# hulop/SfM

Measured on AMD Instinct MI355X. Metric: BA iterations/sec + residual-evals/sec (cams x pts x obs); 1/2/4/8 GPU, higher is better.
Workload: dtype f64; 1 GPU; C3 per GPU: full BA solve (LM + DENSE_SCHUR, Ceres default options); cams=500, points=200000, observations=2000000, points_per_gpu=200000, obs_per_gpu=2000000, views_per_point=10, parallelism=single GPU, reduced_camera_factor=single GPU

## Files before the change

### sfm_amd/csrc/ba_device.h

```cpp
#pragma once
#include <hip/hip_runtime.h>
#include <algorithm>
#include <cstdint>

#include "ba_lm.h"

namespace sfm {

constexpr int kJRec = 20;
constexpr int kJX = 0, kRes = 6, kJC = 8;
constexpr int kEU = 4;
constexpr int kCamR = 36;
constexpr int kUcam = 28;
constexpr int kCamPM = 37;
constexpr int kCamPMMax = 512;
constexpr int kPtV = 10;
constexpr int kPtL = 10;
constexpr int kPtS = 16;
constexpr int kPtG = 16;
constexpr int kCamSR = 32;
constexpr int kNB = 64;
constexpr int kThreads = 256;
constexpr uint32_t kYSentinelWord = 0x7FF4DEADu;
constexpr uint64_t kYSentinel = (uint64_t(kYSentinelWord) << 32) | kYSentinelWord;

struct ReduceJob {
  int slot, nb, op, dst;
};
struct ReduceBatch {
  ReduceJob job[8];
  int n = 0;
  void add(int slot, int nb, int op, int dst) { job[n++] = ReduceJob{slot, nb, op, dst}; }
};

struct DevProblem {
  int32_t C = 0, P = 0;
  int64_t N = 0;
  int32_t* pt_off = nullptr;
  int32_t* order = nullptr;
  int64_t N_pad = 0;
  int32_t* cam_obs = nullptr;
  int32_t* cam_rng = nullptr;
  int32_t* cm_p = nullptr;
  int4* jchunks = nullptr;
  int32_t n_jchunks = 0;
  int32_t xcd_slice_max = 0;
  int32_t* tile_cnt = nullptr;
  int32_t* tile_exp = nullptr;
  int32_t overlap = 0;
  int32_t* jgrp = nullptr;
  int32_t jac_blocks = 1;
  int32_t jac_blocks_rec = 1;
  double* uv_cm = nullptr;
  int32_t* pos = nullptr;
  double* Kc = nullptr;
  double* cam = nullptr;
  double* cam_new = nullptr;
  double* X = nullptr;
  double* X_new = nullptr;
  double* cam0 = nullptr;
  double* X0 = nullptr;
  double* scale_c = nullptr;
  double* scale_p = nullptr;
  double* diag_c = nullptr;
  double* diag_p = nullptr;
  double* camR = nullptr;
  double* camRn = nullptr;
  bool pm_backsub = false;
  double* jrec = nullptr;
  double* eu = nullptr;
  bool eu_cm = false;
  double* ypt = nullptr;
  int32_t* wcam = nullptr;
  double* ptV = nullptr;
  double* ptL = nullptr;
  double* Ucam = nullptr;
  int32_t n = 0, ld = 0, nblk = 0;
  double* S = nullptr;
  double* Spack = nullptr;
  double* invL = nullptr;
  double* ysol = nullptr;
  int32_t* fail = nullptr;
  int32_t* flags = nullptr;
  int32_t* cflags = nullptr;
  unsigned long long* cticket = nullptr;
  int32_t n_cu = 0;
  double min_diag = 1e-6, max_diag = 1e32;

  int64_t n_blk = 0, n_pairs = 0;
  int2* blk = nullptr;
  int32_t* seg = nullptr;
  int32_t* bpts = nullptr;
  int32_t* bperm = nullptr;
  int64_t n_bslots = 0;
  int4* srec = nullptr;
  int32_t schur_wgs = 0;
  double* camS = nullptr;
  double* ptS = nullptr;
  double* ptG = nullptr;
  int32_t schur_pts_sub = 8;
  bool schur_wg_blocks = false;
  double* dpart = nullptr;
  double* jpart = nullptr;
  double* uv_pm = nullptr;
  int32_t* cam_pm = nullptr;
  double* partials = nullptr;
  int32_t max_blocks = 0;
  double* scal = nullptr;
  double* scal_host = nullptr;
  const int32_t* gate = nullptr;
  const double* radius_dev = nullptr;
};

enum PartialSlot {
  kPCost = 0, kPXNormCam, kPXNormPt, kPGradCam, kPGradPt, kPModel, kPNewCost, kPStepPt, kPStepCam, kPBad,
  kPBadCam, kPBadBack, kPModelPt,
  kNumPartialSlots
};

void launch_cam_prep(const DevProblem& d, double* cam, bool count_norm, hipStream_t s);
void launch_cam_prep_accept(const DevProblem& d, bool count_norm, int grid, hipStream_t s);
void launch_jacobian(const DevProblem& d, bool scaled, hipStream_t s, bool write_records = false);
void launch_cam_reduce(const DevProblem& d, hipStream_t s);
void launch_cam_finalize(const DevProblem& d, int mode, bool reuse_diag, bool count_grad, hipStream_t s);
void launch_cam_sum_finalize(const DevProblem& d, int mode, bool count_grad, hipStream_t s);
void launch_point_eval(const DevProblem& d, int mode, bool reuse_diag, hipStream_t s, bool factor = false,
                       double radius = 0.0);
void launch_point_prep(const DevProblem& d, double radius, hipStream_t s);
void launch_obs_prep(const DevProblem& d, hipStream_t s);
void launch_point_factor(const DevProblem& d, double radius, hipStream_t s);
void launch_schur(const DevProblem& d, double radius, bool add_diag, hipStream_t s);
void launch_schur_diag(const DevProblem& d, double radius, bool add_diag, hipStream_t s);
void launch_schur_offdiag(const DevProblem& d, int* tile_cnt, hipStream_t s);
void launch_cam_sum_diag(const DevProblem& d, double radius, bool add_diag, hipStream_t s);
void launch_pad_init(const DevProblem& d, hipStream_t s);
void launch_pack_upper(const DevProblem& d, bool unpack, hipStream_t s);
void launch_gated_copy(const double* src, double* dst, int64_t n, double scale, const int32_t* gate, hipStream_t s);
void launch_cam_update(const DevProblem& d, bool count_norm, hipStream_t s);
inline bool backsub_pm(const DevProblem& d, bool cams_var, bool pts_var) {
  return d.pm_backsub && cams_var && pts_var && d.P > 0 && d.N_pad > 0;
}
bool launch_point_eval_with_cams(const DevProblem& d, int mode, bool count_grad, hipStream_t s);
void launch_point_backsub(const DevProblem& d, hipStream_t s, bool cams_var = true, bool pts_var = true,
                          bool count_norm = false);
inline int obs_xcd_blocks(const DevProblem& d) {
  const int64_t per = d.xcd_slice_max > 0 ? (int64_t(d.xcd_slice_max) + 3) / 4
                                          : ((d.N_pad / 64 + 3) / 4 + 7) / 8;
  return int(8 * std::max<int64_t>(1, per));
}
inline int pt_xcd_blocks(const DevProblem& d) {
  const int64_t per_slice = (int64_t(d.P) + 7) / 8;
  return int(8 * std::max<int64_t>(1, (per_slice + kThreads - 1) / kThreads));
}
void launch_cam_solve(const DevProblem& d, double radius, hipStream_t s);
void launch_reduce(const DevProblem& d, int slot, int nb, int op, int dst, hipStream_t s);
void launch_reduce_batch(const DevProblem& d, const ReduceBatch& b, bool copy_fail, hipStream_t s);
int blocks_for(int64_t n, int threads);

bool launch_cholesky(const DevProblem& d, int epoch, hipStream_t s, bool clear_fail = true, int cam_step = -1,
                     int overlap = 0);
void launch_backsolve(const DevProblem& d, int epoch, hipStream_t s, bool sentinel_set = false);

int launch_cholesky_panel(const DevProblem& d, int k, int pt, int epoch, hipStream_t s);
void launch_panel_update(const DevProblem& d, int k, int j0, int j1, int pt, int nranks, int rank, hipStream_t s);
int panel_update_tiles(int nblk, int pt, int j0, int j1, int nranks, int rank);
constexpr int kPanelPack = 0, kPanelUnpack = 1, kPanelAdd = 2;
void launch_panel_copy(const DevProblem& d, int mode, int pt, int col0, int col1, const int64_t* off, int64_t off1,
                       double* buf, hipStream_t s);
void launch_fail_slot(const DevProblem& d, bool put, double* slot, hipStream_t s);
void launch_spd_fill(double* A, int ld, int n, unsigned seed, hipStream_t s);

}
```

### sfm_amd/csrc/ba_host_layout.h

```cpp
#ifndef SFM_BA_HOST_LAYOUT_H_
#define SFM_BA_HOST_LAYOUT_H_

#include <algorithm>
#include <array>
#include <climits>
#include <cmath>
#include <cstddef>
#include <cstdint>
#include <cstdlib>
#include <vector>

namespace sfm {

constexpr size_t kStageMaxBytes = size_t(1) << 20;
constexpr int64_t kHostCheckMaxObs = 65536;
constexpr int64_t kDeferredUvMinObs = 262144;
constexpr int kSmallSetupMaxC = 256;
constexpr int kSmallSetupMaxChunks = 2048;
constexpr int kSmallSetupMaxPtObs = 64;
constexpr int64_t kSmallSetupMaxObs = 64 * 1024;
constexpr int64_t kSchurXcdMinBlocks = 8192;

namespace hostlayout {

struct StageLayout {
  size_t bytes = 0;
  size_t add(size_t n) {
    const size_t o = bytes;
    bytes += (n + 255) & ~size_t(255);
    return o;
  }
};

inline size_t runs_blob_bound(int C, int64_t N, int P) {
  return 64 * (size_t(C) + 1) + 2 * size_t(N) + 8 * (size_t(P) + 1) + 4 * size_t(C) + 2048;
}

enum class ParamRoute { None, Early, Side, Late };

struct SetupPlan {
  bool host_counts = false;
  bool stage_in = false;
  bool deferred_uv = false;
  size_t o_uv = 0, o_cam = 0, o_pt = 0, o_pc = 0, in_bytes = 0;
  size_t il_base = 0, il_bound = 0;
  size_t o_K = 0, o_c = 0, o_c0 = 0, o_X = 0, o_X0 = 0, pl_bytes = 0;
  size_t pl_base = 0;
  ParamRoute route = ParamRoute::None;
  size_t stage_bytes = 0;
};

inline SetupPlan plan_setup(int64_t N, int C, int P, bool sync_uv) {
  SetupPlan p;
  const bool host_check = N <= kHostCheckMaxObs;
  StageLayout up;
  p.o_uv = up.add(sizeof(double) * 2 * size_t(N));
  p.o_cam = up.add(sizeof(int32_t) * size_t(N));
  p.o_pt = up.add(sizeof(int32_t) * size_t(N));
  p.o_pc = host_check ? up.add(sizeof(int32_t) * (size_t(P) + 1)) : 0;
  p.in_bytes = up.bytes;
  p.stage_in = p.in_bytes <= kStageMaxBytes;
  p.host_counts = host_check && p.stage_in;
  p.deferred_uv = !p.stage_in && N >= kDeferredUvMinObs && !sync_uv;
  p.il_base = p.host_counts ? (p.in_bytes + 255) / 256 * 256 : 0;
  p.il_bound = p.host_counts ? runs_blob_bound(C, N, P) : 0;
  StageLayout pl;
  p.o_K = pl.add(sizeof(double) * 5 * size_t(C));
  p.o_c = pl.add(sizeof(double) * 6 * size_t(C));
  p.o_c0 = pl.add(sizeof(double) * 6 * size_t(C));
  p.o_X = pl.add(sizeof(double) * 3 * size_t(P));
  p.o_X0 = pl.add(sizeof(double) * 3 * size_t(P));
  p.pl_bytes = pl.bytes;
  p.pl_base = (p.il_base + p.il_bound + 255) / 256 * 256;
  if (!(C || P)) p.route = ParamRoute::None;
  else if (p.host_counts && p.pl_base + p.pl_bytes <= 4 * kStageMaxBytes) p.route = ParamRoute::Early;
  else if (p.pl_bytes > kStageMaxBytes) p.route = ParamRoute::Side;
  else p.route = ParamRoute::Late;
  p.stage_bytes = std::max({p.stage_in ? p.il_base + p.il_bound : 0,
                            p.route == ParamRoute::Early ? p.pl_base + p.pl_bytes : 0,
                            sizeof(int32_t) * (size_t(C) + 4)});
  return p;
}

inline bool small_setup_fits(int64_t N, int C, int P, const int32_t* n_obs_of_cam, const int32_t* n_obs_of_pt) {
  if (!(N > 0 && N <= kSmallSetupMaxObs && C > 0 && C <= kSmallSetupMaxC &&
        int64_t(C) * (C + 1) / 2 <= kSchurXcdMinBlocks))
    return false;
  int64_t nch = 0;
  for (int c = 0; c < C; ++c) nch += (n_obs_of_cam[c] + 63) / 64;
  if (nch > kSmallSetupMaxChunks) return false;
  for (int p = 0; p < P; ++p)
    if (n_obs_of_pt[p] > kSmallSetupMaxPtObs) return false;
  return true;
}

struct SchurShape {
  int pts_sub = 8;
  bool wg_blocks = false;
};
inline SchurShape schur_shape(int64_t n_pairs, int64_t n_blk, const char* pts_sub_env, const char* wg_env) {
  SchurShape sh;
  const double avg = n_blk ? double(n_pairs) / double(n_blk) : 0.0;
  if (pts_sub_env) {
    const int v = std::atoi(pts_sub_env);
    sh.pts_sub = v == 64 ? 64 : v == 32 ? 32 : v == 8 ? 8 : 16;
  } else {
    while (sh.pts_sub < 64 && sh.pts_sub < avg / 10.0) sh.pts_sub *= 2;
  }
  sh.wg_blocks = sh.pts_sub == 64 && n_blk <= 4 * 256 && avg >= 256.0;
  if (wg_env) sh.wg_blocks = wg_env[0] == '1' && sh.pts_sub == 64;
  return sh;
}

struct Chunk {
  int32_t cam, pos, cnt, first;
};
static_assert(sizeof(Chunk) == 16, "Chunk must match the device's int4");

inline void check_and_count(int64_t N, const double* obs_uv, const int32_t* cam_idx, const int32_t* pt_idx, int C,
                            int P, bool want_slices, int32_t* cam_cnt, int32_t* pc, std::vector<int32_t>* cam_slice,
                            int64_t* pairs_est) {
  int32_t first[3] = {INT32_MAX, INT32_MAX, INT32_MAX};
  std::fill(cam_cnt, cam_cnt + size_t(C) + 4, 0);
  std::fill(pc, pc + size_t(P) + 1, 0);
  cam_slice->clear();
  *pairs_est = 0;
  const uint64_t* uvb = reinterpret_cast<const uint64_t*>(obs_uv);
  auto nonfinite = [](uint64_t b) { return uint32_t(((b >> 52) & 0x7ff) == 0x7ff); };
  uint32_t bad = 0;
  {
    std::vector<int32_t> cc4(4 * (size_t(C) + 1), 0), pc4(4 * (size_t(P) + 1), 0);
    want_slices = want_slices && P > 0;
    uint32_t sb[8] = {0, 0, 0, 0, 0, 0, 0, 0};
    for (int k = 1; k < 8; ++k) sb[k] = uint32_t((int64_t(k) * P + 7) / 8);
    auto slice_of = [&](uint32_t p) {
      uint32_t v = 0;
      for (int k = 1; k < 8; ++k) v += uint32_t(p >= sb[k]);
      return v;
    };
    std::vector<int32_t> cs4(want_slices ? 4 * 8 * (size_t(C) + 1) : 0, 0);
    int64_t i = 0;
    for (; i + 4 <= N; i += 4) {
      for (int u = 0; u < 4; ++u) {
        const uint32_t c = uint32_t(cam_idx[i + u]), p = uint32_t(pt_idx[i + u]);
        const uint32_t b = uint32_t(c >= uint32_t(C)) | uint32_t(p >= uint32_t(P)) | nonfinite(uvb[2 * (i + u)]) |
                           nonfinite(uvb[2 * (i + u) + 1]);
        bad |= b;
        const uint32_t cc = c < uint32_t(C) ? c : uint32_t(C);
        ++cc4[u * (size_t(C) + 1) + cc];
        ++pc4[u * (size_t(P) + 1) + (p < uint32_t(P) ? p : uint32_t(P))];
        if (want_slices) ++cs4[(u * (size_t(C) + 1) + cc) * 8 + slice_of(p)];
      }
    }
    for (; i < N; ++i) {
      const uint32_t c = uint32_t(cam_idx[i]), p = uint32_t(pt_idx[i]);
      bad |= uint32_t(c >= uint32_t(C)) | uint32_t(p >= uint32_t(P)) | nonfinite(uvb[2 * i]) |
             nonfinite(uvb[2 * i + 1]);
      const uint32_t cc = c < uint32_t(C) ? c : uint32_t(C);
      ++cc4[cc];
      ++pc4[p < uint32_t(P) ? p : uint32_t(P)];
      if (want_slices) ++cs4[size_t(cc) * 8 + slice_of(p)];
    }
    if (want_slices) {
      cam_slice->assign(8 * size_t(C), 0);
      for (size_t e = 0; e < 8 * size_t(C); ++e)
        (*cam_slice)[e] = cs4[e] + cs4[8 * (size_t(C) + 1) + e] + cs4[16 * (size_t(C) + 1) + e] +
                          cs4[24 * (size_t(C) + 1) + e];
    }
    for (int c = 0; c < C; ++c)
      cam_cnt[4 + size_t(c)] =
          cc4[c] + cc4[(size_t(C) + 1) + c] + cc4[2 * (size_t(C) + 1) + c] + cc4[3 * (size_t(C) + 1) + c];
    for (int p = 0; p < P; ++p) {
      pc[p] = pc4[p] + pc4[(size_t(P) + 1) + p] + pc4[2 * (size_t(P) + 1) + p] + pc4[3 * (size_t(P) + 1) + p];
      *pairs_est += int64_t(pc[p]) * (pc[p] - 1) / 2;
    }
  }
  if (bad) {
    for (int64_t i = 0; i < N; ++i) {
      const int32_t c = cam_idx[i], p = pt_idx[i];
      const bool cok = c >= 0 && c < C, pok = p >= 0 && p < P;
      const bool uok = std::isfinite(obs_uv[2 * i]) && std::isfinite(obs_uv[2 * i + 1]);
      if (!cok && first[0] == INT32_MAX) first[0] = int32_t(i);
      if (!pok && first[1] == INT32_MAX) first[1] = int32_t(i);
      if (!uok && first[2] == INT32_MAX) first[2] = int32_t(i);
    }
  }
  cam_cnt[0] = first[0];
  cam_cnt[1] = first[1];
  cam_cnt[2] = first[2];
  cam_cnt[3] = INT32_MAX;
}

struct Runs {
  std::vector<int32_t> cam_off, cam_rng, wcam;
  std::vector<Chunk> chunks;
  int64_t npad = 0;
};
inline void camera_runs(int C, const int32_t* n_obs_of_cam, Runs* r) {
  r->cam_off.assign(size_t(C) + 1, 0);
  r->cam_rng.assign(2 * size_t(C), 0);
  int64_t npad = 0;
  for (int c = 0; c < C; ++c) {
    const int32_t n_c = n_obs_of_cam[c];
    r->cam_off[c + 1] = r->cam_off[c] + n_c;
    r->cam_rng[2 * c] = int32_t(npad);
    r->cam_rng[2 * c + 1] = int32_t(npad + n_c);
    npad += (n_c + 63) / 64 * 64;
  }
  r->npad = npad;
  r->wcam.assign(size_t(npad / 64) + 1, 0);
  for (int c = 0; c < C; ++c)
    for (int64_t w = r->cam_rng[2 * c] / 64;
         w < (int64_t(r->cam_rng[2 * c]) + r->cam_off[c + 1] - r->cam_off[c] + 63) / 64; ++w)
      r->wcam[size_t(w)] = c;
  r->chunks.clear();
  for (int c = 0; c < C; ++c) {
    const int32_t n_c = r->cam_off[c + 1] - r->cam_off[c];
    for (int32_t k = 0; 64 * k < n_c; ++k)
      r->chunks.push_back(Chunk{c, r->cam_rng[2 * c] + 64 * k, std::min<int32_t>(64, n_c - 64 * k),
                                r->cam_off[c] + 64 * k});
  }
}

inline int32_t small_slice_max(int C, const int32_t* n_obs_of_cam, const std::vector<int32_t>& cam_slice) {
  std::array<int32_t, 8> jcnt{};
  for (int c = 0; c < C; ++c) {
    const int32_t n_c = n_obs_of_cam[c];
    int32_t cum = 0;
    int sl = 0;
    for (int32_t k = 0; 64 * k < n_c; ++k) {
      while (sl < 7 && cum + cam_slice[8 * size_t(c) + sl] <= 64 * k) cum += cam_slice[8 * size_t(c) + sl++];
      ++jcnt[size_t(sl)];
    }
  }
  return *std::max_element(jcnt.begin(), jcnt.end());
}

}
}

#endif
```

### sfm_amd/csrc/ba_kernels.hip

```cpp
#include <hip/hip_runtime.h>
#include <cfloat>
#include <cmath>
#include <cstdlib>
#include "ba_device.h"
#include "ba_common.h"

namespace sfm {

namespace {

__global__ __launch_bounds__(kThreads) void k_cam_prep(int C, double* __restrict__ cam,
                                                       double* __restrict__ camR, double* __restrict__ part_xn, const int* __restrict__ gate,
                                                       const double* __restrict__ cam_src, const double* __restrict__ X_src,
                                                       double* __restrict__ X_dst, int64_t n_x) {
  if (gate && *gate == 0) return;
  __shared__ double sh[4];
  const int c = blockIdx.x * blockDim.x + threadIdx.x;
  for (int64_t i = int64_t(blockIdx.x) * blockDim.x + threadIdx.x; i < n_x; i += int64_t(gridDim.x) * blockDim.x)
    X_dst[i] = X_src[i];
  if (int64_t(blockIdx.x) * blockDim.x >= C) return;
  double xn = 0.0;
  if (c < C) {
    const double* cs = cam_src ? cam_src : cam;
    double x6[6];
// ... 14 lines not shown

__device__ __forceinline__ int wave_uniform(int v) { return __builtin_amdgcn_readfirstlane(v); }

__device__ __forceinline__ void jac_flush(const double* wst, double* __restrict__ jrec, int64_t ib, int l) {
  double* dst = jrec + ib * kJRec;
  double2 v[kJRec / 2];
#pragma unroll
  for (int kq = 0; kq < kJRec / 2; ++kq) v[kq] = ld2(wst + 2 * (64 * kq + l));
#pragma unroll
  for (int kq = 0; kq < kJRec / 2; ++kq) st2_nt(dst + 2 * (64 * kq + l), v[kq].x, v[kq].y);
}

__device__ __forceinline__ void wave_lds_sync() {
  __builtin_amdgcn_fence(__ATOMIC_RELEASE, "wavefront");
  __builtin_amdgcn_wave_barrier();
  __builtin_amdgcn_fence(__ATOMIC_ACQUIRE, "wavefront");
}

__device__ __forceinline__ double jac_record(const double* cr, double tc0, double tc1, double tc2, double fx, double sk,
                                             double cx, double fy, double cy, const double* sc, const double* sp,
                                             const double Xp[3], double2 uvo, double rec[kJRec]) {
  const double pc0 = cr[0] * Xp[0] + cr[1] * Xp[1] + cr[2] * Xp[2] + tc0;
  const double pc1 = cr[3] * Xp[0] + cr[4] * Xp[1] + cr[5] * Xp[2] + tc1;
  const double pc2 = cr[6] * Xp[0] + cr[7] * Xp[1] + cr[8] * Xp[2] + tc2;
  const SharedDiv dz = shared_div(pc2);
  const double xp = sdiv(dz, pc0), yp = sdiv(dz, pc1);
  const double r0 = fx * xp + sk * yp + cx - uvo.x;
  const double r1 = fy * yp + cy - uvo.y;
  const double iz = srcp(dz);
  const double a0 = fx * iz, a1 = sk * iz, a2 = -(fx * xp + sk * yp) * iz;
  const double b1 = fy * iz, b2 = -fy * yp * iz;
#pragma unroll
  for (int j = 0; j < 3; ++j) {
    rec[kJX + j] = (a0 * cr[j] + a1 * cr[3 + j] + a2 * cr[6 + j]) * sp[j];
    rec[kJX + 3 + j] = (b1 * cr[3 + j] + b2 * cr[6 + j]) * sp[j];
  }
  rec[kRes] = r0;
  rec[kRes + 1] = r1;
#pragma unroll
  for (int kk = 0; kk < 3; ++kk) {
    const double* D = cr + 9 + 9 * kk;
    const double q0 = D[0] * Xp[0] + D[1] * Xp[1] + D[2] * Xp[2];
    const double q1 = D[3] * Xp[0] + D[4] * Xp[1] + D[5] * Xp[2];
    const double q2 = D[6] * Xp[0] + D[7] * Xp[1] + D[8] * Xp[2];
    rec[kJC + kk] = (a0 * q0 + a1 * q1 + a2 * q2) * sc[kk];
    rec[kJC + 6 + kk] = (b1 * q1 + b2 * q2) * sc[kk];
  }
  rec[kJC + 3] = a0 * sc[3]; rec[kJC + 4] = a1 * sc[4]; rec[kJC + 5] = a2 * sc[5];
  rec[kJC + 9] = 0.0;        rec[kJC + 10] = b1 * sc[4]; rec[kJC + 11] = b2 * sc[5];
  return 0.5 * (r0 * r0 + r1 * r1);
}

template <bool kRec>
__global__ __launch_bounds__(kThreads) void k_jacobian(const int32_t* __restrict__ grp_off,
                                                       const int4* __restrict__ chunks,
                                                       const int32_t* __restrict__ cm_p,
                                                       const double* __restrict__ uv_cm,
                                                       const double* __restrict__ Kc, const double* __restrict__ cam,
                                                       const double* __restrict__ camR, const double* __restrict__ X,
                                                       const double* __restrict__ scale_c,
                                                       const double* __restrict__ scale_p, int scaled,
                                                       double* __restrict__ jrec, double* __restrict__ part_cost,
                                                       double* __restrict__ jpart, const int* __restrict__ gate) {
  if (gate && *gate == 0) return;
  __shared__ double sh[4];
  __shared__ __attribute__((aligned(16))) double stage[kRec ? kThreads * kJRec : 2];
  const int l = threadIdx.x & 63;
  const int wv = wave_uniform(threadIdx.x >> 6);
  double* wst = stage + wv * 64 * kJRec;
  const int grp = blockIdx.x & 7;
  const int nbg = (int(gridDim.x) - 1 - grp) / 8 + 1;
  const int nw = nbg * (kThreads / 64);
  const int wi = (blockIdx.x >> 3) * (kThreads / 64) + wv;
  const int g0 = grp_off[grp], glen = grp_off[grp + 1] - g0;
  int t = g0 + int(int64_t(glen) * wi / nw);
  const int n_chunks = g0 + int(int64_t(glen) * (wi + 1) / nw);
  double cost = 0.0;
  auto chunk_at = [&](int tt) { return chunks[tt < n_chunks ? tt : t]; };
  int p_nxt = 0;
  double2 uv_cur = make_double2(0.0, 0.0);
  double Xc[3] = {0.0, 0.0, 1.0}, spc[3] = {1.0, 1.0, 1.0};
  if (t < n_chunks) {
    const int64_t i = int64_t(chunks[t].y) + l;
    const int p0 = cm_p[i];
    uv_cur = ld2(uv_cm + 2 * i);
    p_nxt = cm_p[int64_t(chunk_at(t + 1).y) + l];
#pragma unroll
    for (int j = 0; j < 3; ++j) Xc[j] = X[3 * size_t(p0) + j];
    if (scaled)
#pragma unroll
      for (int j = 0; j < 3; ++j) spc[j] = scale_p[3 * size_t(p0) + j];
  }
  asm volatile("" : "+v"(Xc[0]), "+v"(Xc[1]), "+v"(Xc[2]), "+v"(spc[0]), "+v"(spc[1]), "+v"(spc[2]), "+v"(uv_cur.x),
               "+v"(uv_cur.y), "+v"(p_nxt));
  double acc[32];
#pragma unroll
  for (int e = 0; e < 32; ++e) acc[e] = 0.0;
  for (; t < n_chunks; ++t) {
    const int4 ch = chunks[t];
    const int c = ch.x, cnt = ch.z;
    const int64_t ib = ch.y;
    double Xn[3], spn[3] = {1.0, 1.0, 1.0};
#pragma unroll
    for (int j = 0; j < 3; ++j) Xn[j] = X[3 * size_t(p_nxt) + j];
    if (scaled)
#pragma unroll
      for (int j = 0; j < 3; ++j) spn[j] = scale_p[3 * size_t(p_nxt) + j];
    const int4 ch_n = chunk_at(t + 1);
    const double2 uv_nxt = ld2(uv_cm + 2 * (int64_t(ch_n.y) + l));
    const int p_nn = cm_p[int64_t(chunk_at(t + 2).y) + l];
    const double* cr = camR + size_t(kCamR) * c;
    const double* k = Kc + 5 * size_t(c);
    double sc[6];
#pragma unroll
    for (int a = 0; a < 6; ++a) sc[a] = scaled ? scale_c[6 * size_t(c) + a] : 1.0;
    {
      double rec[kJRec];
      const double cl = jac_record(cr, cam[6 * c + 3], cam[6 * c + 4], cam[6 * c + 5], k[0], k[1], k[2], k[3], k[4],
                                   sc, spc, Xc, uv_cur, rec);
      cost += (l < cnt) ? cl : 0.0;
      if (kRec) {
        double* mine = wst + l * kJRec;
#pragma unroll
        for (int f = 0; f < kJRec; f += 2) st2(mine + f, rec[f], rec[f + 1]);
      }
      if (jpart) {
        double j0[6], j1[6], r0 = rec[kRes], r1 = rec[kRes + 1];
#pragma unroll
        for (int a = 0; a < 6; ++a) {
          j0[a] = rec[kJC + a];
          j1[a] = rec[kJC + 6 + a];
        }
        if (cnt < 64) {
          const bool real = l < cnt;
#pragma unroll
          for (int a = 0; a < 6; ++a) {
            j0[a] = real ? j0[a] : 0.0;
            j1[a] = real ? j1[a] : 0.0;
          }
          r0 = real ? r0 : 0.0;
          r1 = real ? r1 : 0.0;
        }
        int q = 0;
#pragma unroll
        for (int a = 0; a < 6; ++a)
#pragma unroll
          for (int b = a; b < 6; ++b, ++q) acc[q] += j0[a] * j0[b] + j1[a] * j1[b];
#pragma unroll
        for (int a = 0; a < 6; ++a) acc[21 + a] += j0[a] * r0 + j1[a] * r1;
        double tot = 0.0;
        if (t + 1 >= n_chunks || ch_n.x != c) {
          tot = wave_sum32(acc, l);
#pragma unroll
          for (int e = 0; e < 32; ++e) acc[e] = 0.0;
        }
        if (!(l & 1) && (l >> 1) < 27) jpart[size_t(ib / 64) * 27 + (l >> 1)] = tot;
      }
    }
    if (kRec) {
      wave_lds_sync();
      jac_flush(wst, jrec, ib, l);
      wave_lds_sync();
    }
#pragma unroll
    for (int j = 0; j < 3; ++j) { Xc[j] = Xn[j]; spc[j] = spn[j]; }
    uv_cur = uv_nxt;
    p_nxt = p_nn;
  }
  const double r = block_reduce(cost, sh, false);
  if (threadIdx.x == 0) part_cost[blockIdx.x] = r;
}

__global__ __launch_bounds__(64) void k_cam_sum(const int32_t* __restrict__ cam_rng,
                                                const double* __restrict__ jpart, double* __restrict__ Ucam, const int* __restrict__ gate) {
  if (gate && *gate == 0) return;
  const int c = blockIdx.x, t = threadIdx.x;
  const int w0 = cam_rng[2 * c] / 64, w1 = (cam_rng[2 * c + 1] + 63) / 64;
  double v[32];
#pragma unroll
  for (int e = 0; e < 32; ++e) v[e] = 0.0;
  for (int w = w0 + t; w < w1; w += 64) {
    const double* src = jpart + size_t(w) * 27;
#pragma unroll
    for (int e = 0; e < 27; ++e) v[e] += src[e];
  }
  const double sum = wave_sum32(v, t);
  if (!(t & 1) && (t >> 1) < 27) Ucam[size_t(kUcam) * c + (t >> 1)] = sum;
}

struct CamFold {
  const int32_t* cam_rng;
  const double* jpart;
  double* Ucam;
  double* scale_c;
  double* diag_c;
  double min_diag, max_diag;
  int mode, C;
  double* part_grad;
};
__device__ __forceinline__ double cam_sum_body(int c, int t, const CamFold& f) {
  const int w0 = f.cam_rng[2 * c] / 64, w1 = (f.cam_rng[2 * c + 1] + 63) / 64;
  double v[32];
#pragma unroll
  for (int e = 0; e < 32; ++e) v[e] = 0.0;
  for (int w = w0 + t; w < w1; w += 64) {
    const double* src = f.jpart + size_t(w) * 27;
#pragma unroll
    for (int e = 0; e < 27; ++e) v[e] += src[e];
  }
  const double sum = wave_sum32(v, t);
  if (!(t & 1) && (t >> 1) < 27) f.Ucam[size_t(kUcam) * c + (t >> 1)] = sum;
  const int a = t < 6 ? t : 0;
  const double cn = __shfl(sum, 2 * up6(a, a)), ga = __shfl(sum, 2 * (21 + a));
  double g = 0.0;
  if (t < 6) {
    if (f.mode == 0) {
      f.scale_c[6 * c + a] = 1.0 / (1.0 + sqrt(cn));
    } else {
      f.diag_c[6 * c + a] = fmin(fmax(cn, f.min_diag), f.max_diag);
      g = fabs(ga / f.scale_c[6 * c + a]);
    }
  }
#pragma unroll
  for (int off = 4; off > 0; off >>= 1) g = fmax(g, __shfl_xor(g, off));
  if (t == 0 && f.part_grad) f.part_grad[c] = g;
  return sum;
}

__global__ __launch_bounds__(64) void k_cam_sum_finalize(const CamFold f, const int* __restrict__ gate) {
  if (gate && *gate == 0) return;
  cam_sum_body(blockIdx.x, threadIdx.x, f);
}

__global__ __launch_bounds__(kThreads) void k_cam_finalize(int C, const double* __restrict__ Ucam,
                                                           double* __restrict__ scale_c, double* __restrict__ diag_c,
                                                           double min_diag, double max_diag, int mode, int reuse,
                                                           double* __restrict__ part_grad, const int* __restrict__ gate) {
  if (gate && *gate == 0) return;
  __shared__ double sh[4];
  const int c = blockIdx.x * blockDim.x + threadIdx.x;
  double g = 0.0;
  if (c < C) {
    const double* U = Ucam + size_t(kUcam) * c;
    for (int a = 0; a < 6; ++a) {
      const double cn = U[up6(a, a)];
      if (mode == 0) {
        scale_c[6 * c + a] = 1.0 / (1.0 + sqrt(cn));
      } else {
        if (!reuse) diag_c[6 * c + a] = fmin(fmax(cn, min_diag), max_diag);
        g = fmax(g, fabs(U[21 + a] / scale_c[6 * c + a]));
      }
    }
  }
  const double r = block_reduce(g, sh, true);
  if (threadIdx.x == 0 && part_grad) part_grad[blockIdx.x] = r;
}

struct CamView {
  const double* R; const double* t; const double* K;
  int sR, sT, sK;
};

__device__ __forceinline__ double point_factor_body(int p, const double v[9], const double dg[3], double radius,
                                                    const double x[3], const double sp[3], double* __restrict__ ptL,
                                                    double* __restrict__ ptS, double* __restrict__ ptG) {
  double bad = 0.0;
  double D[3];
  for (int k = 0; k < 3; ++k) { const double d = sqrt(dg[k] / radius); D[k] = d * d; }
  const double V00 = v[0] + D[0], V10 = v[1], V11 = v[2] + D[1], V20 = v[3], V21 = v[4], V22 = v[5] + D[2];
  const double l00 = sqrt(V00);
  const double l10 = V10 / l00, l20 = V20 / l00;
  const double l11 = sqrt(V11 - l10 * l10);
  const double l21 = (V21 - l20 * l10) / l11;
  const double l22 = sqrt(V22 - l20 * l20 - l21 * l21);
  if (!(l00 > 0.0) || !(l11 > 0.0) || !(l22 > 0.0)) bad = 1.0;
  const double z0 = v[6] / l00, z1 = (v[7] - l10 * z0) / l11, z2 = (v[8] - l20 * z0 - l21 * z1) / l22;
  double* L = ptL + size_t(kPtL) * p;
  st2(L, l00, l10); st2(L + 2, l11, l20); st2(L + 4, l21, l22); st2(L + 6, z0, z1); st2(L + 8, z2, 0.0);
  if (ptS) {
    double* o = ptS + size_t(kPtS) * p;
    st2(o, x[0], x[1]); st2(o + 2, x[2], sp[0]); st2(o + 4, sp[1], sp[2]);
    st2(o + 6, l10, l20); st2(o + 8, l21, 1.0 / l00); st2(o + 10, 1.0 / l11, 1.0 / l22);
    st2(o + 12, z0, z1); st2(o + 14, z2, 0.0);
  }
  if (ptG) {
    const double i00 = 1.0 / l00, i11 = 1.0 / l11, i22 = 1.0 / l22;
    const double li10 = -l10 * i00 * i11, li21 = -l21 * i11 * i22, li20 = -(l20 * i00 + l21 * li10) * i22;
    double* o = ptG + size_t(kPtG) * p;
    st2(o, x[0], x[1]); st2(o + 2, x[2], sp[0] * i00); st2(o + 4, sp[0] * li10, sp[0] * li20);
    st2(o + 6, sp[1] * i11, sp[1] * li21); st2(o + 8, sp[2] * i22, 0.0);
  }
  return bad;
}

struct PointFold {
  double radius;
  const double* radius_dev;
  double* ptL;
  double* ptS;
  double* ptG;
  double* part_bad;
};

__device__ __forceinline__ void point_eval_body(int p, const int32_t* __restrict__ pt_off,
                                                const int32_t* __restrict__ cam_pm,
                                                const double* __restrict__ uv_pm, const CamView cv,
                                                const double* __restrict__ X, double* __restrict__ scale_p,
                                                double* __restrict__ diag_p, double* __restrict__ ptV,
                                                double min_diag, double max_diag, int mode, int reuse, double& g,
                                                double& xn, const PointFold& pf, double& bad) {
  double V[6] = {0, 0, 0, 0, 0, 0}, b[3] = {0, 0, 0};
  const double Xp[3] = {X[3 * size_t(p)], X[3 * size_t(p) + 1], X[3 * size_t(p) + 2]};
  double sp[3] = {1.0, 1.0, 1.0};
  if (mode == 1)
    for (int k = 0; k < 3; ++k) sp[k] = scale_p[3 * size_t(p) + k];
  const int q0 = pt_off[p], q1 = pt_off[p + 1];
  int c_n = q0 < q1 ? cam_pm[q0] : 0;
  double2 uv_n = q0 < q1 ? ld2(uv_pm + 2 * size_t(q0)) : make_double2(0.0, 0.0);
  for (int q = q0; q < q1; ++q) {
    const int c = c_n;
    const double2 uvo = uv_n;
    if (q + 1 < q1) {
      c_n = cam_pm[q + 1];
      uv_n = ld2(uv_pm + 2 * size_t(q + 1));
    }
    const double* cr = cv.R + size_t(cv.sR) * c;
    const double* k5 = cv.K + size_t(cv.sK) * c;
    const double* tc = cv.t + size_t(cv.sT) * c;
    const double fx = k5[0], sk = k5[1], cx = k5[2], fy = k5[3], cy = k5[4];
    const double pc0 = cr[0] * Xp[0] + cr[1] * Xp[1] + cr[2] * Xp[2] + tc[0];
    const double pc1 = cr[3] * Xp[0] + cr[4] * Xp[1] + cr[5] * Xp[2] + tc[1];
    const double pc2 = cr[6] * Xp[0] + cr[7] * Xp[1] + cr[8] * Xp[2] + tc[2];
    const SharedDiv dz = shared_div(pc2);
    const double xp = sdiv(dz, pc0), yp = sdiv(dz, pc1);
    const double r0 = fx * xp + sk * yp + cx - uvo.x;
    const double r1 = fy * yp + cy - uvo.y;
    const double iz = srcp(dz);
    const double a0 = fx * iz, a1 = sk * iz, a2 = -(fx * xp + sk * yp) * iz;
    const double b1 = fy * iz, b2 = -fy * yp * iz;
    double u[3], v[3];
#pragma unroll
    for (int j = 0; j < 3; ++j) {
      u[j] = (a0 * cr[j] + a1 * cr[3 + j] + a2 * cr[6 + j]) * sp[j];
      v[j] = (b1 * cr[3 + j] + b2 * cr[6 + j]) * sp[j];
    }
    V[0] += u[0] * u[0] + v[0] * v[0];
    V[1] += u[1] * u[0] + v[1] * v[0]; V[2] += u[1] * u[1] + v[1] * v[1];
    V[3] += u[2] * u[0] + v[2] * v[0]; V[4] += u[2] * u[1] + v[2] * v[1]; V[5] += u[2] * u[2] + v[2] * v[2];
    b[0] += u[0] * r0 + v[0] * r1; b[1] += u[1] * r0 + v[1] * r1; b[2] += u[2] * r0 + v[2] * r1;
  }
  const double cn[3] = {V[0], V[2], V[5]};
  if (mode == 0) {
    for (int k = 0; k < 3; ++k) scale_p[3 * size_t(p) + k] = 1.0 / (1.0 + sqrt(cn[k]));
  } else {
    for (int k = 0; k < 3; ++k) {
      if (!reuse) diag_p[3 * size_t(p) + k] = fmin(fmax(cn[k], min_diag), max_diag);
      g = fmax(g, fabs(b[k] / scale_p[3 * size_t(p) + k]));
      xn += X[3 * size_t(p) + k] * X[3 * size_t(p) + k];
    }
    double* o = ptV + size_t(kPtV) * p;
    st2(o, V[0], V[1]); st2(o + 2, V[2], V[3]); st2(o + 4, V[4], V[5]); st2(o + 6, b[0], b[1]); st2(o + 8, b[2], 0.0);
    if (pf.ptL) {
      double fv[9] = {V[0], V[1], V[2], V[3], V[4], V[5], b[0], b[1], b[2]};
      double fd[3], fx[3] = {Xp[0], Xp[1], Xp[2]}, fs[3] = {sp[0], sp[1], sp[2]};
      for (int k = 0; k < 3; ++k) fd[k] = reuse ? diag_p[3 * size_t(p) + k] : fmin(fmax(cn[k], min_diag), max_diag);
      double radius = pf.radius_dev ? *pf.radius_dev : pf.radius;
      asm volatile("" : "+v"(fv[0]), "+v"(fv[1]), "+v"(fv[2]), "+v"(fv[3]), "+v"(fv[4]), "+v"(fv[5]), "+v"(fv[6]),
                        "+v"(fv[7]), "+v"(fv[8]), "+v"(fd[0]), "+v"(fd[1]), "+v"(fd[2]), "+v"(radius));
      bad = point_factor_body(p, fv, fd, radius, fx, fs, pf.ptL, pf.ptS, pf.ptG);
    }
  }
}

__global__ __launch_bounds__(kThreads) void k_point_eval_rc(int P, const int32_t* __restrict__ pt_off,
                                                            const int32_t* __restrict__ cam_pm,
                                                            const double* __restrict__ uv_pm,
                                                            const double* __restrict__ camR,
                                                            const double* __restrict__ cam,
                                                            const double* __restrict__ Kc,
                                                            const double* __restrict__ X,
                                                            double* __restrict__ scale_p, double* __restrict__ diag_p,
                                                            double* __restrict__ ptV, double min_diag, double max_diag,
                                                            int mode, int reuse, double* __restrict__ part_grad,
                                                            double* __restrict__ part_xn, const int* __restrict__ gate,
                                                            const PointFold pf) {
  if (gate && *gate == 0) return;
  __shared__ double sh[4];
  const int p = blockIdx.x * blockDim.x + threadIdx.x;
  double g = 0.0, xn = 0.0, bad = 0.0;
  const CamView cv{camR, cam + 3, Kc, kCamR, 6, 5};
  if (p < P)
    point_eval_body(p, pt_off, cam_pm, uv_pm, cv, X, scale_p, diag_p, ptV, min_diag, max_diag, mode, reuse, g, xn, pf,
                    bad);
  if (mode == 1) {
    const double rg = block_reduce(g, sh, true);
    if (threadIdx.x == 0) part_grad[blockIdx.x] = rg;
    const double rx = block_reduce(xn, sh, false);
    if (threadIdx.x == 0) part_xn[blockIdx.x] = rx;
    if (pf.ptL) {
      const double rb = block_reduce(bad, sh, true);
      if (threadIdx.x == 0) pf.part_bad[blockIdx.x] = rb;
    }
  }
}

constexpr int kCamE = 17;
template <int kMaxC, int kGroups = 1>
__global__ __launch_bounds__(kThreads * kGroups) void k_point_eval_lds(int P, int C, const int32_t* __restrict__ pt_off,
                                                             const int32_t* __restrict__ cam_pm,
                                                             const double* __restrict__ uv_pm,
                                                             const double* __restrict__ camR,
                                                             const double* __restrict__ cam,
                                                             const double* __restrict__ Kc,
                                                             const double* __restrict__ X,
                                                             double* __restrict__ scale_p, double* __restrict__ diag_p,
                                                             double* __restrict__ ptV, double min_diag, double max_diag,
                                                             int mode, int reuse, double* __restrict__ part_grad,
                                                             double* __restrict__ part_xn, const int* __restrict__ gate,
                                                             const CamFold cf, const PointFold pf) {
  if (gate && *gate == 0) return;
  static_assert(kGroups == 1 || kMaxC > 64, "the camera fold runs with one group per workgroup");
  const int nbp = (P + kThreads - 1) / kThreads;
  if (kGroups == 1 && int(blockIdx.x) >= nbp) {
    const int c = (int(blockIdx.x) - nbp) * (kThreads / 64) + int(threadIdx.x >> 6);
    if (c < cf.C) cam_sum_body(c, threadIdx.x & 63, cf);
    return;
  }
  __shared__ double sh[4 * kGroups];
  __shared__ double cst[kMaxC * kCamE];
  for (int i = threadIdx.x; i < C * kCamE; i += blockDim.x) {
    const int c = i / kCamE, j = i - c * kCamE;
    cst[i] = j < 9 ? camR[size_t(kCamR) * c + j] : j < 12 ? cam[6 * size_t(c) + 3 + (j - 9)] : Kc[5 * size_t(c) + (j - 12)];
  }
  __syncthreads();
  const int grp = int(threadIdx.x) / kThreads, tg = int(threadIdx.x) % kThreads;
  const int vb = int(blockIdx.x) * kGroups + grp;
  const int p = vb * kThreads + tg;
  double g = 0.0, xn = 0.0, bad = 0.0;
  const CamView cv{cst, cst + 9, cst + 12, kCamE, kCamE, kCamE};
  if (p < P)
    point_eval_body(p, pt_off, cam_pm, uv_pm, cv, X, scale_p, diag_p, ptV, min_diag, max_diag, mode, reuse, g, xn, pf,
                    bad);
  if (mode == 1) {
    const int w = int(threadIdx.x) >> 6, l = int(threadIdx.x) & 63;
    __shared__ double shb[4 * kGroups];
    const double wg = wave_max(g), wx = wave_sum(xn);
    if (pf.ptL) {
      const double wb = wave_max(bad);
      if (l == 0) shb[w] = wb;
    }
    if (l == 0) sh[w] = wg;
    __syncthreads();
    double rg = 0.0;
    if (tg == 0) {
      rg = sh[4 * grp];
      for (int i = 1; i < 4; ++i) rg = fmax(rg, sh[4 * grp + i]);
    }
    __syncthreads();
    if (l == 0) sh[w] = wx;
    __syncthreads();
    if (tg == 0 && vb < nbp) {
      double rx = sh[4 * grp];
      for (int i = 1; i < 4; ++i) rx = rx + sh[4 * grp + i];
      part_grad[vb] = rg;
      part_xn[vb] = rx;
      if (pf.ptL) {
        double rb = shb[4 * grp];
        for (int i = 1; i < 4; ++i) rb = fmax(rb, shb[4 * grp + i]);
        pf.part_bad[vb] = rb;
      }
    }
  }
}

__global__ __launch_bounds__(kThreads) void k_point_factor(int P, const double* __restrict__ ptV,
                                                           const double* __restrict__ diag_p, double radius,
                                                           double* __restrict__ ptL, double* __restrict__ part_bad,
                                                           const double* __restrict__ X,
                                                           const double* __restrict__ scale_p,
                                                           double* __restrict__ ptS, const int* __restrict__ gate, const double* __restrict__ radius_dev,
                                                           double* __restrict__ ptG) {
  if (gate && *gate == 0) return;
  if (radius_dev) radius = *radius_dev;
  __shared__ double sh[4];
  const int p = blockIdx.x * blockDim.x + threadIdx.x;
  double bad = 0.0;
  if (p < P) {
    const double* vp = ptV + size_t(kPtV) * p;
    const double v[9] = {vp[0], vp[1], vp[2], vp[3], vp[4], vp[5], vp[6], vp[7], vp[8]};
    const double dg[3] = {diag_p[3 * size_t(p)], diag_p[3 * size_t(p) + 1], diag_p[3 * size_t(p) + 2]};
    double x[3] = {0.0, 0.0, 0.0}, sp[3] = {0.0, 0.0, 0.0};
    if (ptS || ptG)
      for (int k = 0; k < 3; ++k) { x[k] = X[3 * size_t(p) + k]; sp[k] = scale_p[3 * size_t(p) + k]; }
    bad = point_factor_body(p, v, dg, radius, x, sp, ptL, ptS, ptG);
  }
  const double r = block_reduce(bad, sh, true);
  if (threadIdx.x == 0) part_bad[blockIdx.x] = r;
}

struct ObsRC {
  double rec[kJRec];
  double M[6];
  double h0, h1;
};
__device__ __forceinline__ void obs_recompute(int c, int p, double2 uvo, const double* __restrict__ camR,
                                              const double* __restrict__ cam, const double* __restrict__ Kc,
                                              const double* __restrict__ scale_c, const double* __restrict__ ptS,
                                              ObsRC& o) {
  const double* cr = camR + size_t(kCamR) * c;
  const double* k = Kc + 5 * size_t(c);
  const double* tc = cam + 6 * size_t(c) + 3;
  const double* sc = scale_c + 6 * size_t(c);
  const double fx = k[0], sk = k[1], cx = k[2], fy = k[3], cy = k[4];
  const double* rp = ptS + size_t(kPtS) * p;
  double q[16];
#pragma unroll
  for (int f = 0; f < 16; f += 2) {
    const double2 x = ld2(rp + f);
    q[f] = x.x; q[f + 1] = x.y;
  }
  const double Xp[3] = {q[0], q[1], q[2]}, sp[3] = {q[3], q[4], q[5]};
  const double pc0 = cr[0] * Xp[0] + cr[1] * Xp[1] + cr[2] * Xp[2] + tc[0];
  const double pc1 = cr[3] * Xp[0] + cr[4] * Xp[1] + cr[5] * Xp[2] + tc[1];
  const double pc2 = cr[6] * Xp[0] + cr[7] * Xp[1] + cr[8] * Xp[2] + tc[2];
  const double iz = srcp(shared_div(pc2)), xp = pc0 * iz, yp = pc1 * iz;
  double* rec = o.rec;
  rec[kRes] = fx * xp + sk * yp + cx - uvo.x;
  rec[kRes + 1] = fy * yp + cy - uvo.y;
  const double a0 = fx * iz, a1 = sk * iz, a2 = -(fx * xp + sk * yp) * iz;
  const double b1 = fy * iz, b2 = -fy * yp * iz;
#pragma unroll
  for (int j = 0; j < 3; ++j) {
    rec[kJX + j] = (a0 * cr[j] + a1 * cr[3 + j] + a2 * cr[6 + j]) * sp[j];
    rec[kJX + 3 + j] = (b1 * cr[3 + j] + b2 * cr[6 + j]) * sp[j];
  }
#pragma unroll
  for (int kk = 0; kk < 3; ++kk) {
    const double* D = cr + 9 + 9 * kk;
    const double q0 = D[0] * Xp[0] + D[1] * Xp[1] + D[2] * Xp[2];
    const double q1 = D[3] * Xp[0] + D[4] * Xp[1] + D[5] * Xp[2];
    const double q2 = D[6] * Xp[0] + D[7] * Xp[1] + D[8] * Xp[2];
    rec[kJC + kk] = (a0 * q0 + a1 * q1 + a2 * q2) * sc[kk];
    rec[kJC + 6 + kk] = (b1 * q1 + b2 * q2) * sc[kk];
  }
  rec[kJC + 3] = a0 * sc[3]; rec[kJC + 4] = a1 * sc[4]; rec[kJC + 5] = a2 * sc[5];
  rec[kJC + 9] = 0.0;        rec[kJC + 10] = b1 * sc[4]; rec[kJC + 11] = b2 * sc[5];
  const double l10 = q[6], l20 = q[7], l21 = q[8], i00 = q[9], i11 = q[10], i22 = q[11];
  const double* e = rec + kJX;
  o.M[0] = e[0] * i00; o.M[1] = (e[1] - l10 * o.M[0]) * i11; o.M[2] = (e[2] - l20 * o.M[0] - l21 * o.M[1]) * i22;
  o.M[3] = e[3] * i00; o.M[4] = (e[4] - l10 * o.M[3]) * i11; o.M[5] = (e[5] - l20 * o.M[3] - l21 * o.M[4]) * i22;
  o.h0 = o.M[0] * q[12] + o.M[1] * q[13] + o.M[2] * q[14];
  o.h1 = o.M[3] * q[12] + o.M[4] * q[13] + o.M[5] * q[14];
}

struct XcdChunks {
  int t, end, stride;
};
__device__ __forceinline__ XcdChunks xcd_chunks(const int32_t* __restrict__ grp_off, int wv) {
  const int grp = blockIdx.x & 7;
  const int nbg = (int(gridDim.x) - 1 - grp) / 8 + 1;
  const int wi = (blockIdx.x >> 3) * (kThreads / 64) + wv;
  return XcdChunks{grp_off[grp] + wi, grp_off[grp + 1], nbg * (kThreads / 64)};
}

__global__ __launch_bounds__(kThreads) void k_obs_prep_rc(const int32_t* __restrict__ grp_off,
                                                          const int4* __restrict__ chunks,
                                                          const int32_t* __restrict__ cm_p,
                                                          const double* __restrict__ uv_cm,
                                                          const int32_t* __restrict__ cam_obs,
                                                          const double* __restrict__ camR,
                                                          const double* __restrict__ cam,
                                                          const double* __restrict__ Kc,
                                                          const double* __restrict__ scale_c,
                                                          const double* __restrict__ ptS,
                                                          double* __restrict__ dpart, const int* __restrict__ gate) {
  if (gate && *gate == 0) return;
  const int l = threadIdx.x & 63, wv = threadIdx.x >> 6;
  const XcdChunks xc = xcd_chunks(grp_off, wave_uniform(wv));
  if (xc.t >= xc.end) return;
  const int4 ch = chunks[xc.t];
  const int64_t i0 = __builtin_amdgcn_readfirstlane(ch.y);
  const int64_t i = i0 + l;
  const int c = __builtin_amdgcn_readfirstlane(ch.x);
  ObsRC o;
  obs_recompute(c, cm_p[i], ld2(uv_cm + 2 * i), camR, cam, Kc, scale_c, ptS, o);
  const double* jc = o.rec + kJC;
  double F[18];
#pragma unroll
  for (int u = 0; u < 6; ++u) {
    F[3 * u] = jc[u] * o.M[0] + jc[6 + u] * o.M[3];
    F[3 * u + 1] = jc[u] * o.M[1] + jc[6 + u] * o.M[4];
    F[3 * u + 2] = jc[u] * o.M[2] + jc[6 + u] * o.M[5];
  }
  double r0 = o.rec[kRes] - o.h0, r1 = o.rec[kRes + 1] - o.h1;
  if (__builtin_amdgcn_readfirstlane(ch.z) < 64) {
    const bool real = cam_obs[i] >= 0;
#pragma unroll
    for (int e = 0; e < 18; ++e) F[e] = real ? F[e] : 0.0;
    r0 = real ? r0 : 0.0;
    r1 = real ? r1 : 0.0;
  }
  double v[32];
  int q = 0;
#pragma unroll
  for (int u = 0; u < 6; ++u)
#pragma unroll
    for (int w = u; w < 6; ++w, ++q)
      v[q] = F[3 * u] * F[3 * w] + F[3 * u + 1] * F[3 * w + 1] + F[3 * u + 2] * F[3 * w + 2];
#pragma unroll
  for (int u = 0; u < 6; ++u) v[21 + u] = jc[u] * r0 + jc[6 + u] * r1;
#pragma unroll
  for (int e = 27; e < 32; ++e) v[e] = 0.0;
  const double tot = wave_sum32(v, l);
  if (!(l & 1) && (l >> 1) < 27) dpart[size_t(i0 / 64) * 27 + (l >> 1)] = tot;
}

__global__ __launch_bounds__(kThreads) void k_backsub_a_rc(const int32_t* __restrict__ grp_off,
                                                           const int4* __restrict__ chunks,
                                                           const int32_t* __restrict__ cm_p,
                                                           const double* __restrict__ uv_cm,
                                                           const int32_t* __restrict__ cam_obs,
                                                           const double* __restrict__ camR,
                                                           const double* __restrict__ cam,
                                                           const double* __restrict__ Kc,
                                                           const double* __restrict__ scale_c,
                                                           const double* __restrict__ ptS,
                                                           const double* __restrict__ ysol, double* __restrict__ eu,
                                                           int eu_cm, double* __restrict__ part_model, const int* __restrict__ gate) {
  if (gate && *gate == 0) return;
  __shared__ double sh[4];
  const int l = threadIdx.x & 63, wv = threadIdx.x >> 6;
  double model = 0.0;
  const XcdChunks xc = xcd_chunks(grp_off, wave_uniform(wv));
  for (int t = xc.t; t < xc.end; t += xc.stride) {
    const int4 ch = chunks[t];
    const int64_t i = int64_t(__builtin_amdgcn_readfirstlane(ch.y)) + l;
    const int c = __builtin_amdgcn_readfirstlane(ch.x);
    ObsRC o;
    obs_recompute(c, cm_p[i], ld2(uv_cm + 2 * i), camR, cam, Kc, scale_c, ptS, o);
    const double* y = ysol + 6 * size_t(c);
    const double* J = o.rec + kJC;
    double e0 = 0.0, e1 = 0.0;
#pragma unroll
    for (int k = 0; k < 6; ++k) { e0 += J[k] * y[k]; e1 += J[6 + k] * y[k]; }
    const int qo = cam_obs[i];
    if (qo >= 0) {
      model += e0 * o.rec[kRes] + e1 * o.rec[kRes + 1] - 0.5 * (e0 * e0 + e1 * e1);
      const double* M = o.M;
      double* dst = eu + 4 * (eu_cm ? size_t(i) : size_t(qo));
      st2(dst, M[0] * e0 + M[3] * e1, M[1] * e0 + M[4] * e1);
      st2(dst + 2, M[2] * e0 + M[5] * e1, 0.0);
    }
  }
  const double r = block_reduce(model, sh, false);
  if (threadIdx.x == 0) part_model[blockIdx.x] = r;
}

template <bool kRegs = false>
__device__ __forceinline__ void schur_diag_body(int c, int C, int t, const int32_t* __restrict__ cam_rng,
                                                const double* __restrict__ dpart, const double* __restrict__ Ucam,
                                                const double* __restrict__ diag_c, double radius, int add_diag,
                                                double* __restrict__ S, int ld, int n, int init,
                                                int* __restrict__ fail, unsigned long long* __restrict__ ysol,
                                                int n_y, double uq = 0.0, double dgu = 0.0) {
  for (int j = 6 * c; j < 6 * c + 6; ++j) {
    for (int i = n + 1 + t; i < ld; i += 64) S[size_t(j) * ld + i] = 0.0;
    if (t == 0 && j < n_y) ysol[j] = kYSentinel;
  }
  if (c == C - 1) {
    for (int j = n; j < ld; ++j) {
      for (int i = (j > n ? j : n + 1) + t; i < ld; i += 64) S[size_t(j) * ld + i] = (i == j) ? 1.0 : 0.0;
      if (t == 0 && j < n_y) ysol[j] = kYSentinel;
    }
    if (t == 0) {
      S[size_t(n) * ld + n] = 1.0;
      *fail = 0;
    }
  }
  const int w0 = cam_rng[2 * c] / 64, w1 = (cam_rng[2 * c + 1] + 63) / 64;
  double v[32];
#pragma unroll
  for (int e = 0; e < 32; ++e) v[e] = 0.0;
  for (int w = w0 + t; w < w1; w += 64) {
    const double* src = dpart + size_t(w) * 27;
#pragma unroll
    for (int e = 0; e < 27; ++e) v[e] += src[e];
  }
  const double sum = wave_sum32(v, t);
  const int tu = t < 36 ? t / 6 : 0, tv = t < 36 ? t % 6 : 0;
  const int src = t < 36 ? up6(tu, tv) : (t < 42 ? 21 + (t - 36) : 0);
  const double tot = __shfl(sum, 2 * src);
  if (t < 36) {
    const int u = tu, vv = tv, q = src;
    double* sp = S + size_t(6 * c + u) * ld + 6 * size_t(c) + vv;
    double val = (init ? 0.0 : *sp) - tot;
    if (add_diag) {
      val += kRegs ? uq : Ucam[size_t(kUcam) * c + q];
      if (u == vv) { const double dd = sqrt((kRegs ? dgu : diag_c[6 * size_t(c) + u]) / radius); val += dd * dd; }
    }
    *sp = val;
  } else if (t < 42) {
    S[size_t(6 * c + (t - 36)) * ld + n] = tot;
  }
}

struct DiagFold {
  const int32_t* cam_rng;
  const double* dpart;
  const double* Ucam;
  const double* diag_c;
  double radius;
  const double* radius_dev;
  int add_diag, C, n, n_y;
  int* fail;
  unsigned long long* ysol;
};

constexpr int kCamS = 50;

__device__ __forceinline__ void stage_cam(double* cs, int c, const double* __restrict__ camR,
                                          const double* __restrict__ cam, const double* __restrict__ Kc,
                                          const double* __restrict__ scale_c, int l) {
  if (l < 36) cs[l] = camR[size_t(kCamR) * c + l];
  else if (l < 39) cs[l] = cam[6 * size_t(c) + 3 + (l - 36)];
  else if (l < 44) cs[l] = Kc[5 * size_t(c) + (l - 39)];
  else if (l < 50) cs[l] = scale_c[6 * size_t(c) + (l - 44)];
}

__device__ __forceinline__ void pair_side_m(const double* cs, const double Xp[3], const double sp[3],
                                            const double Lp[6], double M[6], double ab[5]) {
  const double* cr = cs;
  const double fx = cs[39], sk = cs[40], fy = cs[42];
  const double pc0 = cr[0] * Xp[0] + cr[1] * Xp[1] + cr[2] * Xp[2] + cs[36];
  const double pc1 = cr[3] * Xp[0] + cr[4] * Xp[1] + cr[5] * Xp[2] + cs[37];
  const double pc2 = cr[6] * Xp[0] + cr[7] * Xp[1] + cr[8] * Xp[2] + cs[38];
  const double iz = srcp(shared_div(pc2)), xp = pc0 * iz, yp = pc1 * iz;
  const double a0 = fx * iz, a1 = sk * iz, a2 = -(fx * xp + sk * yp) * iz;
  const double b1 = fy * iz, b2 = -fy * yp * iz;
  ab[0] = a0; ab[1] = a1; ab[2] = a2; ab[3] = b1; ab[4] = b2;
  double e[6];
#pragma unroll
  for (int j = 0; j < 3; ++j) {
    e[j] = (a0 * cr[j] + a1 * cr[3 + j] + a2 * cr[6 + j]) * sp[j];
    e[3 + j] = (b1 * cr[3 + j] + b2 * cr[6 + j]) * sp[j];
  }
// ... 534 lines not shown
    p_nx = iB1;
    asm volatile("" ::: "memory");
    pairs_rot_finish<kSub>(cs1, cs2, acc, own, cc, S, ld, nullptr, l, sl);
    wave_lds_sync();
    tA = tB; tB = tC; tC += W;
    rA = rB; rB = rC;
    cur ^= 1;
  }
}

__global__ __launch_bounds__(64) void k_schur_diag_sum(const int32_t* __restrict__ cam_rng,
                                                       const double* __restrict__ dpart,
                                                       const double* __restrict__ Ucam,
                                                       const double* __restrict__ diag_c, double radius,
                                                       int add_diag, double* __restrict__ S, int ld, int n,
                                                       int init, const int* __restrict__ gate, const double* __restrict__ radius_dev,
                                                       int* __restrict__ fail, unsigned long long* __restrict__ ysol, int n_y) {
  if (gate && *gate == 0) return;
  if (radius_dev) radius = *radius_dev;
  schur_diag_body(blockIdx.x, gridDim.x, threadIdx.x, cam_rng, dpart, Ucam, diag_c, radius, add_diag, S, ld, n, init,
                  fail, ysol, n_y);
}

__global__ __launch_bounds__(64) void k_cam_sum_diag(const CamFold f, const DiagFold df, double* __restrict__ S, int ld,
                                                     const int* __restrict__ gate) {
  if (gate && *gate == 0) return;
  const int c = blockIdx.x, t = threadIdx.x;
  const double sum = cam_sum_body(c, t, f);
  const int tu = t < 36 ? t / 6 : 0, tv = t < 36 ? t % 6 : 0;
  double uq = __shfl(sum, 2 * up6(tu, tv));
  double dgu = fmin(fmax(__shfl(sum, 2 * up6(tu, tu)), f.min_diag), f.max_diag);
  double radius = df.radius_dev ? *df.radius_dev : df.radius;
  asm volatile("" : "+v"(uq), "+v"(dgu), "+v"(radius));
  schur_diag_body<true>(c, df.C, t, df.cam_rng, df.dpart, nullptr, nullptr, radius, df.add_diag, S, ld, df.n, 1,
                        df.fail, df.ysol, df.n_y, uq, dgu);
}

__device__ __forceinline__ size_t packed_row(int i, int n) { return size_t(i) * (n + 1) - size_t(i) * (i - 1) / 2; }

__global__ void k_pack_upper(const double* __restrict__ S, int ld, int n, double* __restrict__ P, const int* __restrict__ gate) {
  if (gate && *gate == 0) return;
  const int i = blockIdx.x;
  const double* row = S + size_t(i) * ld;
  double* dst = P + packed_row(i, n) - i;
  for (int j = i + threadIdx.x; j <= n; j += blockDim.x) dst[j] = row[j];
}

__global__ void k_unpack_upper(const double* __restrict__ P, int ld, int n, double* __restrict__ S, const int* __restrict__ gate) {
  if (gate && *gate == 0) return;
  const int i = blockIdx.x;
  double* row = S + size_t(i) * ld;
  const double* src = P + packed_row(i, n) - i;
  for (int j = i + threadIdx.x; j <= n; j += blockDim.x) row[j] = src[j];
}

__global__ void k_gated_copy(const double* src, double* dst, int64_t n, double scale, const int* __restrict__ gate) {
  if (gate && *gate == 0) return;
  for (int64_t i = blockIdx.x * int64_t(blockDim.x) + threadIdx.x; i < n; i += int64_t(gridDim.x) * blockDim.x)
    dst[i] = src[i] * scale;
}

__global__ void k_pad_init(double* __restrict__ S, int ld, int n, int* __restrict__ fail,
                           unsigned long long* __restrict__ ysol, int n_y, const int* __restrict__ gate) {
  if (gate && *gate == 0) return;
  const int j = blockIdx.x;
  if (j == 0 && threadIdx.x == 0) *fail = 0;
  if (threadIdx.x == 0 && j < n_y) ysol[j] = kYSentinel;
  for (int i = (j > n ? j : n + 1) + threadIdx.x; i < ld; i += blockDim.x) S[size_t(j) * ld + i] = (i == j) ? 1.0 : 0.0;
  if (j == n && threadIdx.x == 0) S[size_t(n) * ld + n] = 1.0;
}

__device__ __forceinline__ void cam_pm_pack(int c, const double* __restrict__ camR, const double* __restrict__ cam,
                                            const double* __restrict__ Kc, const double* __restrict__ ysol,
                                            const double* __restrict__ scale_c, double* __restrict__ o) {
  const double* cr = camR + size_t(kCamR) * c;
  double R[9], sy[6];
  for (int i = 0; i < 9; ++i) R[i] = cr[i];
  for (int k = 0; k < 6; ++k) sy[k] = scale_c[6 * c + k] * ysol[6 * c + k];
  bool first_order = true;
#pragma unroll 1
  for (int k = 0; k < 3; ++k)
#pragma unroll
    for (int i = 0; i < 9; ++i) first_order = first_order & (cr[9 + 9 * k + i] == skew_basis_entry(k, i));
  double om[3] = {sy[0], sy[1], sy[2]};
  if (!first_order) {
    om[0] = om[1] = om[2] = 0.0;
    for (int k = 0; k < 3; ++k) {
      const double* D = cr + 9 + 9 * k;
      double W[9];
      for (int i = 0; i < 3; ++i)
        for (int j = 0; j < 3; ++j) W[3 * i + j] = D[3 * i] * R[3 * j] + D[3 * i + 1] * R[3 * j + 1] + D[3 * i + 2] * R[3 * j + 2];
      om[0] += 0.5 * (W[7] - W[5]) * sy[k];
      om[1] += 0.5 * (W[2] - W[6]) * sy[k];
      om[2] += 0.5 * (W[3] - W[1]) * sy[k];
    }
  }
  for (int i = 0; i < 9; ++i) o[i] = R[i];
  for (int i = 0; i < 3; ++i) o[9 + i] = cam[6 * c + 3 + i];
  for (int i = 0; i < 5; ++i) o[12 + i] = Kc[5 * size_t(c) + i];
  for (int i = 0; i < 3; ++i) { o[17 + i] = om[i]; o[20 + i] = sy[3 + i]; }
  o[35] = first_order ? 1.0 : 0.0;
  o[36] = 0.0;
}

__global__ __launch_bounds__(kThreads) void k_cam_update(int C, const double* __restrict__ cam,
                                                         const double* __restrict__ ysol,
                                                         const double* __restrict__ scale_c,
                                                         double* __restrict__ cam_new, double* __restrict__ camRn,
                                                         double* __restrict__ part_step, double* __restrict__ part_bad, const int* __restrict__ gate) {
  if (gate && *gate == 0) return;
  __shared__ double sh[4];
  const int c = blockIdx.x * blockDim.x + threadIdx.x;
  double st = 0.0, bad = 0.0;
  if (c < C) cam_update_one(c, cam, ysol, scale_c, cam_new, camRn, st, bad);
  const double rs = block_reduce(st, sh, false);
  if (threadIdx.x == 0 && part_step) part_step[blockIdx.x] = rs;
  const double rb = block_reduce(bad, sh, true);
  if (threadIdx.x == 0) part_bad[blockIdx.x] = rb;
}

__global__ __launch_bounds__(kThreads) void k_cam_solve(int C, const double* __restrict__ Ucam,
                                                        const double* __restrict__ diag_c, double radius,
                                                        double* __restrict__ ysol, int* __restrict__ fail, const int* __restrict__ gate, const double* __restrict__ radius_dev) {
  if (gate && *gate == 0) return;
  if (radius_dev) radius = *radius_dev;
  const int c = blockIdx.x * blockDim.x + threadIdx.x;
  if (c >= C) return;
  const double* U = Ucam + size_t(kUcam) * c;
  double L[21], y[6];
  bool ok = true;
#pragma unroll
  for (int j = 0; j < 6; ++j) {
    double s = U[up6(j, j)] + diag_c[6 * c + j] / radius;
#pragma unroll
    for (int k = 0; k < j; ++k) s -= L[up6(k, j)] * L[up6(k, j)];
    ok = ok && s > 0.0 && isfinite(s);
    const double ljj = sqrt(s);
    L[up6(j, j)] = ljj;
#pragma unroll
    for (int i = j + 1; i < 6; ++i) {
      double a = U[up6(j, i)];
#pragma unroll
      for (int k = 0; k < j; ++k) a -= L[up6(k, i)] * L[up6(k, j)];
      L[up6(j, i)] = a / ljj;
    }
  }
#pragma unroll
  for (int i = 0; i < 6; ++i) {
    double s = U[21 + i];
#pragma unroll
    for (int k = 0; k < i; ++k) s -= L[up6(k, i)] * y[k];
    y[i] = s / L[up6(i, i)];
  }
#pragma unroll
  for (int i = 5; i >= 0; --i) {
    double s = y[i];
#pragma unroll
    for (int k = i + 1; k < 6; ++k) s -= L[up6(i, k)] * y[k];
    y[i] = s / L[up6(i, i)];
  }
#pragma unroll
  for (int i = 0; i < 6; ++i) ysol[6 * c + i] = y[i];
  if (!ok) atomicOr(fail, 1);
}


__global__ __launch_bounds__(kThreads) void k_backsub_b(int P, const int32_t* __restrict__ pt_off,
                                                        const double* __restrict__ eu,
                                                        const int32_t* __restrict__ eu_pos,
                                                        const double* __restrict__ ptL,
                                                        const double* __restrict__ ptV,
                                                        const double* __restrict__ scale_p,
                                                        const double* __restrict__ X, double* __restrict__ X_new,
                                                        double* __restrict__ ypt, double* __restrict__ part_step,
                                                        double* __restrict__ part_bad,
                                                        double* __restrict__ part_model, const int* __restrict__ gate) {
  if (gate && *gate == 0) return;
  __shared__ double sh[4];
  const int x = blockIdx.x & 7;
  const int pb = int((int64_t(x) * P + 7) / 8), pe = int((int64_t(x + 1) * P + 7) / 8);
  const int p = pb + (blockIdx.x >> 3) * blockDim.x + threadIdx.x;
  double st = 0.0, bad = 0.0, model = 0.0;
  if (p < pe) {
    const double* L = ptL + size_t(kPtL) * p;
    const double l00 = L[0], l10 = L[1], l11 = L[2], l20 = L[3], l21 = L[4], l22 = L[5];
    double w0 = L[6], w1 = L[7], w2 = L[8];
    double s0 = 0.0, s1 = 0.0, s2 = 0.0;
    const int q0 = pt_off[p], q1 = pt_off[p + 1];
    int q = q0;
    for (; q + 4 <= q1; q += 4) {
      int ps[4];
#pragma unroll
      for (int j = 0; j < 4; ++j) ps[j] = eu_pos ? eu_pos[q + j] : q + j;
      double2 a[4];
      double b[4];
#pragma unroll
      for (int j = 0; j < 4; ++j) {
        const double* u = eu + 4 * size_t(ps[j]);
        a[j] = ld2(u);
        b[j] = u[2];
      }
#pragma unroll
      for (int j = 0; j < 4; ++j) {
        w0 -= a[j].x;
        w1 -= a[j].y;
        w2 -= b[j];
        s0 += a[j].x; s1 += a[j].y; s2 += b[j];
      }
    }
    for (; q < q1; ++q) {
      const double* u = eu + 4 * (eu_pos ? size_t(eu_pos[q]) : size_t(q));
      const double2 u01 = ld2(u);
      const double u2 = u[2];
      w0 -= u01.x;
      w1 -= u01.y;
      w2 -= u2;
      s0 += u01.x; s1 += u01.y; s2 += u2;
    }
    const double y2 = w2 / l22;
    const double y1 = (w1 - l21 * y2) / l11;
    const double y0 = (w0 - l10 * y1 - l20 * y2) / l00;
    if (!isfinite(y0) || !isfinite(y1) || !isfinite(y2)) bad = 1.0;
    {
      const double* v = ptV + size_t(kPtV) * p;
      const double h0 = l00 * s0, h1 = l10 * s0 + l11 * s1, h2 = l20 * s0 + l21 * s1 + l22 * s2;
      const double yVy = v[0] * y0 * y0 + v[2] * y1 * y1 + v[5] * y2 * y2 +
                         2.0 * (v[1] * y0 * y1 + v[3] * y0 * y2 + v[4] * y1 * y2);
      model = y0 * (v[6] - h0) + y1 * (v[7] - h1) + y2 * (v[8] - h2) - 0.5 * yVy;
    }
    const double yp[3] = {y0, y1, y2};
    for (int k = 0; k < 3; ++k) {
      const double x = X[3 * size_t(p) + k];
      const double xn = x + scale_p[3 * size_t(p) + k] * (-yp[k]);
      const double d = x - xn;
      st += d * d;
      X_new[3 * size_t(p) + k] = xn;
      ypt[3 * size_t(p) + k] = yp[k];
    }
  }
  double r = block_reduce(st, sh, false);
  if (threadIdx.x == 0) part_step[blockIdx.x] = r;
  r = block_reduce(bad, sh, true);
  if (threadIdx.x == 0) part_bad[blockIdx.x] = r;
  r = block_reduce(model, sh, false);
  if (threadIdx.x == 0) part_model[blockIdx.x] = r;
}

__global__ __launch_bounds__(kThreads) void k_backsub_c(const int32_t* __restrict__ grp_off,
                                                        const int4* __restrict__ chunks,
                                                        const int32_t* __restrict__ cam_obs,
                                                        const int32_t* __restrict__ cm_p,
                                                        const double* __restrict__ uv_cm,
                                                        const double* __restrict__ Kc,
                                                        const double* __restrict__ X_new,
                                                        const double* __restrict__ camRn,
                                                        double* __restrict__ part_cost, const int* __restrict__ gate) {
  if (gate && *gate == 0) return;
  __shared__ double sh[4];
  const int l = threadIdx.x & 63, wv = threadIdx.x >> 6;
  const XcdChunks xc = xcd_chunks(grp_off, wave_uniform(wv));
  double ncost = 0.0;
  if (xc.t < xc.end) {
    const int4 ch = chunks[xc.t];
    const int64_t i = int64_t(__builtin_amdgcn_readfirstlane(ch.y)) + l;
    const int c = __builtin_amdgcn_readfirstlane(ch.x);
    const bool real = cam_obs[i] >= 0;
    const int p = cm_p[i];
    const double* Rn = camRn + 12 * size_t(c);
    const double Xn0 = X_new[3 * size_t(p)], Xn1 = X_new[3 * size_t(p) + 1], Xn2 = X_new[3 * size_t(p) + 2];
    double pc[3];
#pragma unroll
    for (int k = 0; k < 3; ++k) pc[k] = Rn[3 * k] * Xn0 + Rn[3 * k + 1] * Xn1 + Rn[3 * k + 2] * Xn2 + Rn[9 + k];
    const SharedDiv dz = shared_div(pc[2]);
    const double xp = sdiv(dz, pc[0]), ypj = sdiv(dz, pc[1]);
    const double* k5 = Kc + 5 * size_t(c);
    const double2 uvo = ld2(uv_cm + 2 * i);
    const double rn0 = k5[0] * xp + k5[1] * ypj + k5[2] - uvo.x;
    const double rn1 = k5[3] * ypj + k5[4] - uvo.y;
    if (real) ncost = 0.5 * (rn0 * rn0 + rn1 * rn1);
  }
  const double r = block_reduce(ncost, sh, false);
  if (threadIdx.x == 0) part_cost[blockIdx.x] = r;
}

struct CamStepFold {
  const double* cam; const double* ysol; const double* scale_c; const double* camR; const double* Kc;
  double* cam_new; double* camRn; double* part_step; double* part_bad;
};

__device__ __forceinline__ void cam_step_record(int c, const CamStepFold& cu, double* o, bool store, double& st,
                                                double& bad) {
  double xn[6], rn[12];
  cam_update_vals(c, cu.cam, cu.ysol, cu.scale_c, xn, rn, st, bad);
  if (store) {
    for (int k = 0; k < 6; ++k) cu.cam_new[6 * c + k] = xn[k];
    for (int i = 0; i < 12; ++i) cu.camRn[12 * size_t(c) + i] = rn[i];
  }
  for (int i = 0; i < 12; ++i) o[23 + i] = rn[i];
  cam_pm_pack(c, cu.camR, cu.cam, cu.Kc, cu.ysol, cu.scale_c, o);
}

template <int kGroups>
__global__ __launch_bounds__(kThreads * kGroups) void k_backsub_pm(
    int P, int C, const int32_t* __restrict__ pt_off, const int32_t* __restrict__ cam_pm,
    const double* __restrict__ uv_pm, const double* __restrict__ ptL,
    const double* __restrict__ ptV, const double* __restrict__ scale_p, const double* __restrict__ X,
    double* __restrict__ X_new, double* __restrict__ ypt, double* __restrict__ part_model,
    double* __restrict__ part_model_pt, double* __restrict__ part_step, double* __restrict__ part_bad,
    double* __restrict__ part_cost, const int* __restrict__ gate, const CamStepFold cu) {
  if (gate && *gate == 0) return;
  static_assert(kThreads * kGroups >= kCamPMMax, "one thread per camera record");
  __shared__ double sh[4 * kGroups];
  __shared__ double cst[kCamPMMax * kCamPM];
  const int nbp = (P + kThreads - 1) / kThreads;
  const int grp = int(threadIdx.x) / kThreads, tg = int(threadIdx.x) % kThreads;
  const int vb = int(blockIdx.x) * kGroups + grp;
  const int p = vb * kThreads + tg;
  {
    const int c = int(threadIdx.x);
    double cst_ = 0.0, cbad = 0.0;
    if (c < C) cam_step_record(c, cu, cst + kCamPM * c, blockIdx.x == 0, cst_, cbad);
    if (blockIdx.x == 0) {
      const int w = int(threadIdx.x) >> 6, l = int(threadIdx.x) & 63;
      const int nbc = (C + kThreads - 1) / kThreads;
      const double ws = wave_sum(cst_), wb = wave_max(cbad);
      if (l == 0) sh[w] = ws;
      __syncthreads();
      if (tg == 0 && grp < nbc && cu.part_step) {
        double r = sh[4 * grp];
        for (int i = 1; i < 4; ++i) r = r + sh[4 * grp + i];
        cu.part_step[grp] = r;
      }
      __syncthreads();
      if (l == 0) sh[w] = wb;
      __syncthreads();
      if (tg == 0 && grp < nbc) {
        double r = sh[4 * grp];
        for (int i = 1; i < 4; ++i) r = fmax(r, sh[4 * grp + i]);
        cu.part_bad[grp] = r;
      }
    }
  }
  __syncthreads();
  double model = 0.0, model_pt = 0.0, st = 0.0, bad = 0.0, ncost = 0.0;
  if (p < P) {
    const double Xp[3] = {X[3 * size_t(p)], X[3 * size_t(p) + 1], X[3 * size_t(p) + 2]};
    const double sp[3] = {scale_p[3 * size_t(p)], scale_p[3 * size_t(p) + 1], scale_p[3 * size_t(p) + 2]};
    const int q0 = pt_off[p], q1 = pt_off[p + 1];
    int c_n = q0 < q1 ? cam_pm[q0] : 0;
    double2 uv_n = q0 < q1 ? ld2(uv_pm + 2 * size_t(q0)) : make_double2(0.0, 0.0);
    double h0 = 0.0, h1 = 0.0, h2 = 0.0;
    for (int q = q0; q < q1; ++q) {
      const double* k = cst + kCamPM * c_n;
      const double2 uvo = uv_n;
      if (q + 1 < q1) {
        c_n = cam_pm[q + 1];
        uv_n = ld2(uv_pm + 2 * size_t(q + 1));
      }
      const double y0 = k[0] * Xp[0] + k[1] * Xp[1] + k[2] * Xp[2];
      const double y1 = k[3] * Xp[0] + k[4] * Xp[1] + k[5] * Xp[2];
      const double y2 = k[6] * Xp[0] + k[7] * Xp[1] + k[8] * Xp[2];
      const double pc0 = y0 + k[9], pc1 = y1 + k[10], pc2 = y2 + k[11];
      const double fx = k[12], sk = k[13], cx = k[14], fy = k[15], cy = k[16];
      const double iz = srcp(shared_div(pc2)), xp = pc0 * iz, yp = pc1 * iz;
      const double r0 = fx * xp + sk * yp + cx - uvo.x;
      const double r1 = fy * yp + cy - uvo.y;
      const double a0 = fx * iz, a1 = sk * iz, a2 = -(fx * xp + sk * yp) * iz;
      const double b1 = fy * iz, b2 = -fy * yp * iz;
      const bool fo = k[35] != 0.0;
      const double t0 = fo ? Xp[0] : y0, t1 = fo ? Xp[1] : y1, t2 = fo ? Xp[2] : y2;
      const double d0 = k[18] * t2 - k[19] * t1 + k[20];
      const double d1 = k[19] * t0 - k[17] * t2 + k[21];
      const double d2 = k[17] * t1 - k[18] * t0 + k[22];
      const double e0 = a0 * d0 + a1 * d1 + a2 * d2, e1 = b1 * d1 + b2 * d2;
      model += e0 * r0 + e1 * r1 - 0.5 * (e0 * e0 + e1 * e1);
      h0 += ((a0 * k[0] + a1 * k[3] + a2 * k[6]) * e0 + (b1 * k[3] + b2 * k[6]) * e1) * sp[0];
      h1 += ((a0 * k[1] + a1 * k[4] + a2 * k[7]) * e0 + (b1 * k[4] + b2 * k[7]) * e1) * sp[1];
      h2 += ((a0 * k[2] + a1 * k[5] + a2 * k[8]) * e0 + (b1 * k[5] + b2 * k[8]) * e1) * sp[2];
    }
    const double* L = ptL + size_t(kPtL) * p;
    const double l00 = L[0], l10 = L[1], l11 = L[2], l20 = L[3], l21 = L[4], l22 = L[5];
    const double s0 = h0 / l00, s1 = (h1 - l10 * s0) / l11, s2 = (h2 - l20 * s0 - l21 * s1) / l22;
    const double w0 = L[6] - s0, w1 = L[7] - s1, w2 = L[8] - s2;
    const double yp2 = w2 / l22;
    const double yp1 = (w1 - l21 * yp2) / l11;
    const double yp0 = (w0 - l10 * yp1 - l20 * yp2) / l00;
    if (!isfinite(yp0) || !isfinite(yp1) || !isfinite(yp2)) bad = 1.0;
    {
      const double* v = ptV + size_t(kPtV) * p;
      const double yVy = v[0] * yp0 * yp0 + v[2] * yp1 * yp1 + v[5] * yp2 * yp2 +
                         2.0 * (v[1] * yp0 * yp1 + v[3] * yp0 * yp2 + v[4] * yp1 * yp2);
      model_pt = yp0 * (v[6] - h0) + yp1 * (v[7] - h1) + yp2 * (v[8] - h2) - 0.5 * yVy;
    }
    const double ys[3] = {yp0, yp1, yp2};
    double Xn[3];
#pragma unroll
    for (int j = 0; j < 3; ++j) {
      Xn[j] = Xp[j] + sp[j] * (-ys[j]);
      const double dd = Xp[j] - Xn[j];
      st += dd * dd;
      X_new[3 * size_t(p) + j] = Xn[j];
      ypt[3 * size_t(p) + j] = ys[j];
    }
    c_n = q0 < q1 ? cam_pm[q0] : 0;
    uv_n = q0 < q1 ? ld2(uv_pm + 2 * size_t(q0)) : make_double2(0.0, 0.0);
    for (int q = q0; q < q1; ++q) {
      const double* k = cst + kCamPM * c_n;
      const double2 uvo = uv_n;
      if (q + 1 < q1) {
        c_n = cam_pm[q + 1];
        uv_n = ld2(uv_pm + 2 * size_t(q + 1));
      }
      const double* Rn = k + 23;
      double pc[3];
#pragma unroll
      for (int j = 0; j < 3; ++j) pc[j] = Rn[3 * j] * Xn[0] + Rn[3 * j + 1] * Xn[1] + Rn[3 * j + 2] * Xn[2] + Rn[9 + j];
      const SharedDiv dz = shared_div(pc[2]);
      const double xp = sdiv(dz, pc[0]), ypj = sdiv(dz, pc[1]);
      const double rn0 = k[12] * xp + k[13] * ypj + k[14] - uvo.x;
      const double rn1 = k[15] * ypj + k[16] - uvo.y;
      ncost += 0.5 * (rn0 * rn0 + rn1 * rn1);
    }
  }
  const int w = int(threadIdx.x) >> 6, l = int(threadIdx.x) & 63;
  auto group_reduce = [&](double v, bool is_max, double* __restrict__ part) {
    v = is_max ? wave_max(v) : wave_sum(v);
    __syncthreads();
    if (l == 0) sh[w] = v;
    __syncthreads();
    if (tg == 0 && vb < nbp) {
      double r = sh[4 * grp];
      for (int i = 1; i < 4; ++i) r = is_max ? fmax(r, sh[4 * grp + i]) : r + sh[4 * grp + i];
      part[vb] = r;
    }
  };
  group_reduce(model, false, part_model);
  group_reduce(model_pt, false, part_model_pt);
  group_reduce(st, false, part_step);
  group_reduce(bad, true, part_bad);
  group_reduce(ncost, false, part_cost);
}

__global__ __launch_bounds__(1024) void k_reduce_batch(const double* __restrict__ partials, int64_t max_blocks,
                                                       ReduceBatch b, double* __restrict__ scal,
                                                       const int* __restrict__ fail, const int* __restrict__ gate) {
  if (gate && *gate == 0) return;
  __shared__ double sh[16];
  reduce_batch_job(partials, max_blocks, b.job[blockIdx.x], scal, blockIdx.x == 0 ? fail : nullptr, sh);
}

__global__ __launch_bounds__(1024) void k_reduce(const double* __restrict__ src, int nb, int op,
                                                 double* __restrict__ dst) {
  __shared__ double sh[16];
  double v = 0.0;
  for (int i = threadIdx.x; i < nb; i += 1024) v = op ? fmax(v, src[i]) : v + src[i];
  v = op ? wave_max(v) : wave_sum(v);
  const int w = threadIdx.x >> 6, l = threadIdx.x & 63;
  if (l == 0) sh[w] = v;
  __syncthreads();
  if (threadIdx.x == 0) {
    double r = sh[0];
    for (int i = 1; i < 16; ++i) r = op ? fmax(r, sh[i]) : r + sh[i];
    *dst = r;
  }
}

}

int blocks_for(int64_t n, int threads) { return int((n + threads - 1) / threads); }

static inline double* slot(const DevProblem& d, int s) { return d.partials + size_t(s) * d.max_blocks; }

void launch_cam_prep(const DevProblem& d, double* cam, bool count_norm, hipStream_t s) {
  k_cam_prep<<<blocks_for(d.C, kThreads), kThreads, 0, s>>>(d.C, cam, d.camR, count_norm ? slot(d, kPXNormCam) : nullptr, d.gate,
                                                            nullptr, nullptr, nullptr, 0);
}
void launch_cam_prep_accept(const DevProblem& d, bool count_norm, int grid, hipStream_t s) {
  k_cam_prep<<<std::max(grid, blocks_for(d.C, kThreads)), kThreads, 0, s>>>(
      d.C, d.cam, d.camR, count_norm ? slot(d, kPXNormCam) : nullptr, d.gate, d.cam_new, d.X_new, d.X, 3 * int64_t(d.P));
}
void launch_jacobian(const DevProblem& d, bool scaled, hipStream_t s, bool write_records) {
  if (write_records)
    k_jacobian<true><<<d.jac_blocks_rec, kThreads, 0, s>>>(d.jgrp, d.jchunks, d.cm_p, d.uv_cm, d.Kc, d.cam, d.camR,
                                                           d.X, d.scale_c, d.scale_p, scaled ? 1 : 0, d.jrec,
                                                           slot(d, kPCost), d.jpart, d.gate);
  else
    k_jacobian<false><<<d.jac_blocks, kThreads, 0, s>>>(d.jgrp, d.jchunks, d.cm_p, d.uv_cm, d.Kc, d.cam, d.camR, d.X,
                                                        d.scale_c, d.scale_p, scaled ? 1 : 0, d.jrec, slot(d, kPCost),
                                                        d.jpart, d.gate);
}
void launch_cam_reduce(const DevProblem& d, hipStream_t s) {
  if (d.C) k_cam_sum<<<d.C, 64, 0, s>>>(d.cam_rng, d.jpart, d.Ucam, d.gate);
}
static CamFold cam_fold(const DevProblem& d, int mode, bool count_grad) {
  return CamFold{d.cam_rng, d.jpart, d.Ucam, d.scale_c, d.diag_c, d.min_diag, d.max_diag, mode, d.C,
                 count_grad ? slot(d, kPGradCam) : nullptr};
}
void launch_cam_sum_finalize(const DevProblem& d, int mode, bool count_grad, hipStream_t s) {
  if (d.C) k_cam_sum_finalize<<<d.C, 64, 0, s>>>(cam_fold(d, mode, count_grad), d.gate);
}
bool launch_point_eval_with_cams(const DevProblem& d, int mode, bool count_grad, hipStream_t s) {
  if (d.P == 0 || d.C == 0 || d.C > 64) return false;
  const int nb = blocks_for(d.P, kThreads) + (d.C + kThreads / 64 - 1) / (kThreads / 64);
  k_point_eval_lds<64><<<nb, kThreads, 0, s>>>(d.P, d.C, d.pt_off, d.cam_pm, d.uv_pm, d.camR, d.cam, d.Kc, d.X,
                                               d.scale_p, d.diag_p, d.ptV, d.min_diag, d.max_diag, mode, 0,
                                               slot(d, kPGradPt), slot(d, kPXNormPt), d.gate,
                                               cam_fold(d, mode, count_grad), PointFold{});
  return true;
}
void launch_cam_finalize(const DevProblem& d, int mode, bool reuse_diag, bool count_grad, hipStream_t s) {
  k_cam_finalize<<<blocks_for(d.C, kThreads), kThreads, 0, s>>>(d.C, d.Ucam, d.scale_c, d.diag_c, d.min_diag, d.max_diag, mode,
                                                               reuse_diag ? 1 : 0,
                                                               count_grad ? slot(d, kPGradCam) : nullptr, d.gate);
}
static bool env_flag_k(const char* name) {
  const char* v = std::getenv(name);
  return v && v[0] == '1';
}
void launch_point_eval(const DevProblem& d, int mode, bool reuse_diag, hipStream_t s, bool factor, double radius) {
  if (d.P == 0) return;
  const int nb = blocks_for(d.P, kThreads);
  const PointFold pf = factor && mode == 1 ? PointFold{radius, d.radius_dev, d.ptL, d.ptS, d.ptG, slot(d, kPBad)}
                                           : PointFold{};
#define SFM_PE_LDS(M_)                                                                                              \
  k_point_eval_lds<M_><<<nb, kThreads, 0, s>>>(d.P, d.C, d.pt_off, d.cam_pm, d.uv_pm, d.camR, d.cam, d.Kc, d.X,      \
                                               d.scale_p, d.diag_p, d.ptV, d.min_diag, d.max_diag, mode,           \
                                               reuse_diag ? 1 : 0, slot(d, kPGradPt), slot(d, kPXNormPt), d.gate,    \
                                               CamFold{}, pf)
  if (d.C <= 64) SFM_PE_LDS(64);
  else if (d.C <= 512 && !env_flag_k("SFM_PE_GROUPS1"))
    k_point_eval_lds<512, 2><<<blocks_for(d.P, 2 * kThreads), 2 * kThreads, 0, s>>>(
        d.P, d.C, d.pt_off, d.cam_pm, d.uv_pm, d.camR, d.cam, d.Kc, d.X, d.scale_p, d.diag_p, d.ptV, d.min_diag,
        d.max_diag, mode, reuse_diag ? 1 : 0, slot(d, kPGradPt), slot(d, kPXNormPt), d.gate, CamFold{}, pf);
  else if (d.C <= 512) SFM_PE_LDS(512);
  else
    k_point_eval_rc<<<nb, kThreads, 0, s>>>(d.P, d.pt_off, d.cam_pm, d.uv_pm, d.camR, d.cam, d.Kc, d.X, d.scale_p,
                                            d.diag_p, d.ptV, d.min_diag, d.max_diag, mode, reuse_diag ? 1 : 0,
                                            slot(d, kPGradPt), slot(d, kPXNormPt), d.gate, pf);
#undef SFM_PE_LDS
}
void launch_point_factor(const DevProblem& d, double radius, hipStream_t s) {
  if (d.P) k_point_factor<<<blocks_for(d.P, kThreads), kThreads, 0, s>>>(d.P, d.ptV, d.diag_p, radius, d.ptL,
                                                                         slot(d, kPBad), d.X, d.scale_p, d.ptS, d.gate, d.radius_dev,
                                                                         d.ptG);
}
void launch_point_prep(const DevProblem& d, double radius, hipStream_t s) {
  launch_point_factor(d, radius, s);
  launch_obs_prep(d, s);
}
void launch_obs_prep(const DevProblem& d, hipStream_t s) {
  if (d.N_pad)
    k_obs_prep_rc<<<obs_xcd_blocks(d), kThreads, 0, s>>>(d.jgrp, d.jchunks, d.cm_p, d.uv_cm, d.cam_obs, d.camR, d.cam,
                                                         d.Kc, d.scale_c, d.ptS, d.dpart, d.gate);
}
void launch_schur(const DevProblem& d, double radius, bool add_diag, hipStream_t s) {
  if (d.schur_wg_blocks && d.n_blk && d.C) {
    const DiagFold f{d.cam_rng, d.dpart, d.Ucam, d.diag_c, radius, d.radius_dev, add_diag ? 1 : 0, d.C, d.n,
                     (d.n + kNB - 1) / kNB * kNB, d.fail, reinterpret_cast<unsigned long long*>(d.ysol)};
    k_schur_pts<64, kThreads / 64><<<int(d.n_bslots), kThreads, 0, s>>>(d.n_bslots, d.blk, d.seg, d.bpts, d.ptS,
                                                                       d.camR, d.cam, d.Kc, d.scale_c, d.S, d.ld,
                                                                       d.bperm, d.gate, nullptr, d.nblk, f);
    return;
  }
  launch_schur_diag(d, radius, add_diag, s);
  launch_schur_offdiag(d, nullptr, s);
}
void launch_cam_sum_diag(const DevProblem& d, double radius, bool add_diag, hipStream_t s) {
  if (!d.C) return;
  const DiagFold f{d.cam_rng, d.dpart, d.Ucam, d.diag_c, radius, d.radius_dev, add_diag ? 1 : 0, d.C, d.n,
                   (d.n + kNB - 1) / kNB * kNB, d.fail, reinterpret_cast<unsigned long long*>(d.ysol)};
  k_cam_sum_diag<<<d.C, 64, 0, s>>>(cam_fold(d, 1, true), f, d.S, d.ld, d.gate);
}
void launch_schur_diag(const DevProblem& d, double radius, bool add_diag, hipStream_t s) {
  if (d.C)
    k_schur_diag_sum<<<d.C, 64, 0, s>>>(d.cam_rng, d.dpart, d.Ucam, d.diag_c, radius, add_diag ? 1 : 0, d.S, d.ld,
                                        d.n, 1, d.gate, d.radius_dev, d.fail,
                                        reinterpret_cast<unsigned long long*>(d.ysol), (d.n + kNB - 1) / kNB * kNB);
}
void launch_schur_offdiag(const DevProblem& d, int* tile_cnt, hipStream_t s) {
  if (!d.n_blk) return;
  const int64_t n_slots = tile_cnt ? d.n_blk : d.n_bslots;
  const int32_t* bperm = tile_cnt ? nullptr : d.bperm;
  const int sub = d.schur_pts_sub, per = 64 / sub * (kThreads / 64);
  const int nb = int((n_slots + per - 1) / per);
#define SFM_PTS(S_)                                                                                           \
  k_schur_pts<S_><<<nb, kThreads, 0, s>>>(n_slots, d.blk, d.seg, d.bpts, d.ptS, d.camR, d.cam, d.Kc, d.scale_c, \
                                          d.S, d.ld, bperm, d.gate, tile_cnt, d.nblk, DiagFold{})
  if (d.schur_wg_blocks) {
    k_schur_pts<64, kThreads / 64><<<int(n_slots), kThreads, 0, s>>>(n_slots, d.blk, d.seg, d.bpts, d.ptS,
                                                                    d.camR, d.cam, d.Kc, d.scale_c, d.S, d.ld,
                                                                    bperm, d.gate, tile_cnt, d.nblk, DiagFold{});
    return;
  }
  if (d.ptG && d.srec && !tile_cnt) {
    const int64_t wg_groups = n_slots / per;
    const int grid = d.schur_wgs > 0 ? d.schur_wgs
                                     : int(std::max<int64_t>(8, std::min<int64_t>(8 * std::max(1, d.n_cu), wg_groups)));
    const int n_tick = int(n_slots / (8 * per)) * (kThreads / 64);
    const int nbc = (d.C + per - 1) / per;
#define SFM_ROTP(S_)                                                                                               \
  k_cam_stage_rot<S_><<<nbc, kThreads, 0, s>>>(d.C, d.camR, d.cam, d.Kc, d.scale_c, d.camS, d.gate);               \
  k_schur_pairs_rot_pw<S_><<<grid, kThreads, 0, s>>>(d.srec, n_tick, d.bpts, d.ptG, d.camS, d.S, d.ld, d.gate)
    if (sub == 8) { SFM_ROTP(8); }
    else if (sub == 16) { SFM_ROTP(16); }
    else if (sub == 32) { SFM_ROTP(32); }
    else { SFM_ROTP(64); }
#undef SFM_ROTP
    return;
  }
  if (d.ptG) {
#define SFM_ROT(S_)                                                                                           \
  k_schur_pairs_rot<S_><<<nb, kThreads, 0, s>>>(n_slots, d.blk, d.seg, d.bpts, d.ptG, d.camR, d.cam, d.Kc, d.scale_c, \
                                                d.S, d.ld, bperm, d.gate, tile_cnt, d.nblk)
    if (sub == 8) SFM_ROT(8);
    else if (sub == 16) SFM_ROT(16);
    else if (sub == 32) SFM_ROT(32);
    else SFM_ROT(64);
#undef SFM_ROT
    return;
  }
  if (sub == 8) SFM_PTS(8);
  else if (sub == 16) SFM_PTS(16);
  else if (sub == 32) SFM_PTS(32);
  else SFM_PTS(64);
#undef SFM_PTS
}
void launch_pack_upper(const DevProblem& d, bool unpack, hipStream_t s) {
  if (d.n == 0) return;
  if (unpack) k_unpack_upper<<<d.n, 256, 0, s>>>(d.Spack, d.ld, d.n, d.S, d.gate);
  else k_pack_upper<<<d.n, 256, 0, s>>>(d.S, d.ld, d.n, d.Spack, d.gate);
}
void launch_gated_copy(const double* src, double* dst, int64_t n, double scale, const int32_t* gate, hipStream_t s) {
  if (n <= 0) return;
  const int grid = int(std::min<int64_t>(1024, (n + 255) / 256));
  k_gated_copy<<<grid, 256, 0, s>>>(src, dst, n, scale, gate);
}
void launch_pad_init(const DevProblem& d, hipStream_t s) {
  const int n_y = (d.n + kNB - 1) / kNB * kNB;
  k_pad_init<<<d.ld, 64, 0, s>>>(d.S, d.ld, d.n, d.fail, reinterpret_cast<unsigned long long*>(d.ysol), n_y, d.gate);
}
void launch_cam_update(const DevProblem& d, bool count_norm, hipStream_t s) {
  k_cam_update<<<blocks_for(d.C, kThreads), kThreads, 0, s>>>(d.C, d.cam, d.ysol, d.scale_c, d.cam_new, d.camRn,
                                                             count_norm ? slot(d, kPStepCam) : nullptr,
                                                             slot(d, kPBadCam), d.gate);
}
void launch_cam_solve(const DevProblem& d, double radius, hipStream_t s) {
  (void)hipMemsetAsync(d.fail, 0, sizeof(int), s);
  if (d.C) k_cam_solve<<<blocks_for(d.C, kThreads), kThreads, 0, s>>>(d.C, d.Ucam, d.diag_c, radius, d.ysol, d.fail, d.gate, d.radius_dev);
}
void launch_point_backsub(const DevProblem& d, hipStream_t s, bool cams_var, bool pts_var, bool count_norm) {
  if (backsub_pm(d, cams_var, pts_var)) {
    constexpr int kG = 4;
    k_backsub_pm<kG><<<blocks_for(d.P, kG * kThreads), kG * kThreads, 0, s>>>(
        d.P, d.C, d.pt_off, d.cam_pm, d.uv_pm, d.ptL, d.ptV, d.scale_p, d.X, d.X_new, d.ypt,
        slot(d, kPModel), slot(d, kPModelPt), slot(d, kPStepPt), slot(d, kPBadBack), slot(d, kPNewCost), d.gate,
        CamStepFold{d.cam, d.ysol, d.scale_c, d.camR, d.Kc, d.cam_new, d.camRn,
                    count_norm ? slot(d, kPStepCam) : nullptr, slot(d, kPBadCam)});
    return;
  }
  if (d.N_pad && cams_var)
    k_backsub_a_rc<<<obs_xcd_blocks(d), kThreads, 0, s>>>(d.jgrp, d.jchunks, d.cm_p, d.uv_cm, d.cam_obs, d.camR,
                                                          d.cam, d.Kc, d.scale_c, d.ptS, d.ysol, d.eu, d.eu_cm ? 1 : 0,
                                                          slot(d, kPModel), d.gate);
  else if (d.N_pad) {
    (void)hipMemsetAsync(d.eu, 0, sizeof(double) * 4 * size_t(d.eu_cm ? d.N_pad : d.N), s);
    (void)hipMemsetAsync(slot(d, kPModel), 0, sizeof(double) * size_t(obs_xcd_blocks(d)), s);
  }
  if (d.P && pts_var) {
    k_backsub_b<<<pt_xcd_blocks(d), kThreads, 0, s>>>(d.P, d.pt_off, d.eu, d.eu_cm ? d.pos : nullptr,
                                                               d.ptL, d.ptV, d.scale_p,
                                                               d.X, d.X_new, d.ypt, slot(d, kPStepPt),
                                                               slot(d, kPBadBack), slot(d, kPModelPt), d.gate);
  } else if (d.P) {
    const size_t nbP = size_t(pt_xcd_blocks(d));
    (void)hipMemsetAsync(d.ypt, 0, sizeof(double) * 3 * size_t(d.P), s);
    (void)hipMemcpyAsync(d.X_new, d.X, sizeof(double) * 3 * size_t(d.P), hipMemcpyDeviceToDevice, s);
    (void)hipMemsetAsync(slot(d, kPStepPt), 0, sizeof(double) * nbP, s);
    (void)hipMemsetAsync(slot(d, kPBadBack), 0, sizeof(double) * nbP, s);
    (void)hipMemsetAsync(slot(d, kPModelPt), 0, sizeof(double) * nbP, s);
  }
  if (d.N_pad)
    k_backsub_c<<<obs_xcd_blocks(d), kThreads, 0, s>>>(d.jgrp, d.jchunks, d.cam_obs, d.cm_p, d.uv_cm, d.Kc, d.X_new,
                                                       d.camRn, slot(d, kPNewCost), d.gate);
}
void launch_reduce(const DevProblem& d, int sl, int nb, int op, int dst, hipStream_t s) {
  k_reduce<<<1, 1024, 0, s>>>(slot(d, sl), nb, op, d.scal + dst);
}
void launch_reduce_batch(const DevProblem& d, const ReduceBatch& b, bool copy_fail, hipStream_t s) {
  if (b.n > 0)
    k_reduce_batch<<<b.n, 1024, 0, s>>>(d.partials, d.max_blocks, b, d.scal, copy_fail ? d.fail : nullptr, d.gate);
}

}
```

### sfm_amd/csrc/ba_problem.hip

```cpp
#include <hip/hip_runtime.h>

#include <algorithm>
#include <atomic>
#include <climits>
#include <cstdlib>
#include <cstring>
#include <string>
#include <thread>
#include <vector>

#include "sfm_trace.h"
#include "ba_device.h"
#include "ba_setup.h"
#include "ba_common.h"
#include "ba_host_layout.h"
#include "ba_handle.h"
#include "../../include/sfm_amd.h"

using namespace sfm;
using hostlayout::ParamRoute;

namespace {

struct Setup {
  sfm_ba_handle* const h;
  DevProblem& d;
  const hipStream_t s;
  const int64_t N;
  const int C, P;
  const double* const obs_uv;
  const int32_t *const cam_idx, *const pt_idx;
  const double* const X;
  const hostlayout::SetupPlan plan;
  HostTimer timer;
  int rc = 0;

  std::vector<double> Kc, cam;
  std::vector<int32_t> cam_cnt;
  std::vector<int32_t> cam_slice;
  int64_t pairs_est = 0;
  hostlayout::Runs runs;
  bool small = false;

  uint8_t* in_blob = nullptr;
  double* in_uv = nullptr;
  int32_t *in_cam = nullptr, *in_pt = nullptr, *cnt_p = nullptr, *cnt_c = nullptr;
  int32_t* err = nullptr;
  uint64_t *k64a = nullptr, *k64b = nullptr;
  uint32_t *k32a = nullptr, *k32b = nullptr;
  int32_t *iota = nullptr, *pt_s = nullptr, *cm_order = nullptr, *perm = nullptr, *d_cam_off = nullptr;
  int4* ch_in = nullptr;
  void* sort_tmp = nullptr;
  size_t sort_bytes = 0;
  int32_t* small_fill = nullptr;
  int64_t* poff = nullptr;
  const int32_t* pair_order = nullptr;
  int64_t n_pairs = 0;
  int bperm_per = 0;
  int64_t* grp_host = nullptr;
  int32_t* uv_err_host = nullptr;

  std::atomic<int> uv_state{0};
  std::atomic<int> param_state{0};
  struct Joiner {
    std::thread t;
    void join() {
      if (t.joinable()) t.join();
    }
    ~Joiner() { join(); }
  } worker;

  Setup(sfm_ba_handle* h_, int64_t n_obs, const double* uv, const int32_t* ci, const int32_t* pi, int n_cams,
        int n_pts, const double* X_)
      : h(h_), d(h_->d), s(h_->stream), N(n_obs), C(n_cams), P(n_pts), obs_uv(uv), cam_idx(ci), pt_idx(pi), X(X_),
        plan(hostlayout::plan_setup(n_obs, n_cams, n_pts, n_obs >= kDeferredUvMinObs && env_flag("SFM_SYNC_UV"))),
        cam_cnt(size_t(n_cams) + 4) {}

  template <typename T>
  bool alloc(T*& p, size_t count) { return (rc = dalloc(h, &p, count)) == 0; }
  template <typename T>
  bool tmp(T*& p, size_t count) { return (rc = dalloc_tmp(h, &p, count)) == 0; }
};

struct ProblemGuard {
  Setup& c;
  bool committed = false;
  ~ProblemGuard() {
    if (committed) return;
    c.worker.join();
    free_problem(c.h);
  }
};

void bind_params(Setup& c, uint8_t* blob) {
  c.d.Kc = reinterpret_cast<double*>(blob + c.plan.o_K);
  c.d.cam = reinterpret_cast<double*>(blob + c.plan.o_c);
  c.d.cam0 = reinterpret_cast<double*>(blob + c.plan.o_c0);
  c.d.X = reinterpret_cast<double*>(blob + c.plan.o_X);
  c.d.X0 = reinterpret_cast<double*>(blob + c.plan.o_X0);
}
int alloc_params(Setup& c) {
  uint8_t* pb = nullptr;
  if (!c.alloc(pb, c.plan.pl_bytes)) return c.rc;
  bind_params(c, pb);
  return 0;
}
void fill_param_stage(const Setup& c, uint8_t* ps) {
  std::memcpy(ps + c.plan.o_K, c.Kc.data(), sizeof(double) * c.Kc.size());
  std::memcpy(ps + c.plan.o_c, c.cam.data(), sizeof(double) * c.cam.size());
  std::memcpy(ps + c.plan.o_c0, c.cam.data(), sizeof(double) * c.cam.size());
  if (c.P) {
    std::memcpy(ps + c.plan.o_X, c.X, sizeof(double) * 3 * size_t(c.P));
    std::memcpy(ps + c.plan.o_X0, c.X, sizeof(double) * 3 * size_t(c.P));
  }
}
int ensure_side_stream(sfm_ba_handle* h) {
  if (h->ustream) return 0;
  HIPCHK(hipStreamCreateWithFlags(&h->ustream, hipStreamNonBlocking));
  HIPCHK(hipEventCreateWithFlags(&h->uev, hipEventDisableTiming));
  return 0;
}
bool side_params_copies(Setup& c) {
  const DevProblem& d = c.d;
  hipStream_t u = c.h->ustream;
  const size_t cam_b = sizeof(double) * c.cam.size(), X_b = sizeof(double) * 3 * size_t(c.P);
  return hipMemcpyAsync(d.Kc, c.Kc.data(), sizeof(double) * c.Kc.size(), hipMemcpyHostToDevice, u) == hipSuccess &&
         hipMemcpyAsync(d.cam, c.cam.data(), cam_b, hipMemcpyHostToDevice, u) == hipSuccess &&
         hipMemcpyAsync(d.cam0, d.cam, cam_b, hipMemcpyDeviceToDevice, u) == hipSuccess &&
         (!c.P || (hipMemcpyAsync(d.X, c.X, X_b, hipMemcpyHostToDevice, u) == hipSuccess &&
                   hipMemcpyAsync(d.X0, d.X, X_b, hipMemcpyDeviceToDevice, u) == hipSuccess)) &&
         hipEventRecord(c.h->uev, u) == hipSuccess;
}
int enqueue_side_params(Setup& c) { return side_params_copies(c) ? 0 : fail(SFM_EIO, "parameter upload failed"); }


int open_uploads(Setup& c, const double* K9, const double* rot, const double* t) {
  if (int rc = stage_reserve(c.h, c.plan.stage_bytes)) return rc;
  if (!c.tmp(c.in_blob, c.plan.in_bytes)) return c.rc;
  c.in_uv = reinterpret_cast<double*>(c.in_blob + c.plan.o_uv);
  c.in_cam = reinterpret_cast<int32_t*>(c.in_blob + c.plan.o_cam);
  c.in_pt = reinterpret_cast<int32_t*>(c.in_blob + c.plan.o_pt);
  c.Kc.resize(5 * size_t(c.C));
  c.cam.resize(6 * size_t(c.C));
  for (int i = 0; i < c.C; ++i) {
    const double* k = K9 + 9 * size_t(i);
    double* o = &c.Kc[5 * size_t(i)];
    o[0] = k[0]; o[1] = k[1]; o[2] = k[2]; o[3] = k[4]; o[4] = k[5];
    for (int j = 0; j < 3; ++j) { c.cam[6 * i + j] = rot[3 * i + j]; c.cam[6 * i + 3 + j] = t[3 * i + j]; }
  }
  if (c.plan.route == ParamRoute::Side) {
    if (int rc = alloc_params(c)) return rc;
    return ensure_side_stream(c.h);
  }
  return 0;
}

int start_uv_worker(Setup& c) {
  sfm_ba_handle* h = c.h;
  if (int rc = ensure_side_stream(h)) return rc;
  if (!h->uev_uv) HIPCHK(hipEventCreateWithFlags(&h->uev_uv, hipEventDisableTiming));
  Setup* cp = &c;
  auto uv_job = [cp]() {
    Setup& c = *cp;
    bool ok = hipSetDevice(c.h->device) == hipSuccess;
    if (c.plan.route == ParamRoute::Side)
      c.param_state.store(ok && side_params_copies(c) ? 1 : 2, std::memory_order_release);
    ok = ok && hipMemcpyAsync(c.in_uv, c.obs_uv, sizeof(double) * 2 * size_t(c.N), hipMemcpyHostToDevice,
                              c.h->ustream) == hipSuccess &&
         hipEventRecord(c.h->uev_uv, c.h->ustream) == hipSuccess;
    c.uv_state.store(ok ? 1 : 2, std::memory_order_release);
  };
  try {
    c.worker.t = std::thread(uv_job);
  } catch (...) {
    uv_job();
  }
  return 0;
}
int wait_uv(Setup& c) {
  c.worker.join();
  if (c.uv_state.load(std::memory_order_acquire) != 1) return fail(SFM_EIO, "observation upload failed");
  if (hipStreamWaitEvent(c.s, c.h->uev_uv, 0) != hipSuccess) return fail(SFM_EIO, "observation upload wait failed");
  return 0;
}

int upload_inputs(Setup& c) {
  const hostlayout::SetupPlan& pl = c.plan;
  uint8_t* stg = c.h->stage;
  hipStream_t s = c.s;
  const int64_t N = c.N;
  if (pl.host_counts) {
    hostlayout::check_and_count(N, c.obs_uv, c.cam_idx, c.pt_idx, c.C, c.P, c.C <= kSmallSetupMaxC, c.cam_cnt.data(),
                                reinterpret_cast<int32_t*>(stg + pl.o_pc), &c.cam_slice, &c.pairs_est);
    c.cnt_p = reinterpret_cast<int32_t*>(c.in_blob + pl.o_pc);
    c.timer.mark("host checks + counts");
  } else {
    if (!(c.tmp(c.err, 4 + size_t(c.C) + 1) && c.tmp(c.cnt_p, size_t(c.P) + 1))) return c.rc;
    c.cnt_c = c.err + 4;
  }
  if (pl.stage_in && (N || pl.host_counts)) {
    if (N) {
      std::memcpy(stg + pl.o_uv, c.obs_uv, sizeof(double) * 2 * size_t(N));
      std::memcpy(stg + pl.o_cam, c.cam_idx, sizeof(int32_t) * size_t(N));
      std::memcpy(stg + pl.o_pt, c.pt_idx, sizeof(int32_t) * size_t(N));
    }
    HIPCHK(hipMemcpyAsync(c.in_blob, stg, pl.in_bytes, hipMemcpyHostToDevice, s));
    c.timer.mark("stage copy + upload");
  } else if (N) {
    HIPCHK(hipMemcpyAsync(c.in_cam, c.cam_idx, sizeof(int32_t) * size_t(N), hipMemcpyHostToDevice, s));
    HIPCHK(hipMemcpyAsync(c.in_pt, c.pt_idx, sizeof(int32_t) * size_t(N), hipMemcpyHostToDevice, s));
    if (pl.deferred_uv) return start_uv_worker(c);
    HIPCHK(hipMemcpyAsync(c.in_uv, c.obs_uv, sizeof(double) * 2 * size_t(N), hipMemcpyHostToDevice, s));
  }
  return 0;
}

int validate_on_device(Setup& c) {
  const bool deferred_uv = c.plan.deferred_uv;
  uint8_t* stg = c.h->stage;
  hipStream_t s = c.s;
  Fill32Set fs;
  fs.add(c.err, 4 * sizeof(int32_t), uint32_t(INT32_MAX));
  fs.add(c.cnt_c, sizeof(int32_t) * (size_t(c.C) + 1), 0);
  fs.add(c.cnt_p, sizeof(int32_t) * (size_t(c.P) + 1), 0);
  launch_fill32(fs, s);
  launch_validate(c.N, deferred_uv ? nullptr : c.in_uv, c.in_cam, c.in_pt, c.C, c.P, c.err, c.cnt_c,
                  deferred_uv ? nullptr : c.cnt_p, s);
  HIPCHK(hipMemcpyAsync(stg, c.err, sizeof(int32_t) * (size_t(c.C) + 4), hipMemcpyDeviceToHost, s));
  HIPCHK(hipStreamSynchronize(s));
  std::memcpy(c.cam_cnt.data(), stg, sizeof(int32_t) * (size_t(c.C) + 4));
  if (deferred_uv && std::min(c.cam_cnt[0], c.cam_cnt[1]) != INT32_MAX) {
    if (int rc = wait_uv(c)) return rc;
    launch_validate(c.N, c.in_uv, c.in_cam, c.in_pt, c.C, c.P, c.err, c.cnt_c, c.cnt_p, s);
    HIPCHK(hipMemcpyAsync(stg, c.err, sizeof(int32_t) * 4, hipMemcpyDeviceToHost, s));
    HIPCHK(hipStreamSynchronize(s));
    std::memcpy(c.cam_cnt.data(), stg, sizeof(int32_t) * 4);
  }
  return 0;
}
int report_first_bad_observation(const Setup& c) {
  const int32_t e0 = c.cam_cnt[0], e1 = c.cam_cnt[1], e2 = c.cam_cnt[2];
  const int32_t first = std::min({e0, e1, e2});
  if (first == INT32_MAX) return 0;
  const char* what = first == e0 ? "cam_idx out of range at " : first == e1 ? "pt_idx out of range at "
                                                                               : "non-finite observation at ";
  return fail(SFM_EINVAL, what + std::to_string(first));
}

void camera_runs(Setup& c) {
  DevProblem& d = c.d;
  hostlayout::camera_runs(c.C, c.cam_cnt.data() + 4, &c.runs);
  d.N_pad = c.runs.npad;
  d.n_jchunks = int32_t(c.runs.chunks.size());
  d.jac_blocks_rec = 8 * std::max(1, std::min((d.n_jchunks / 8 + 3) / 4, 128));
  d.jac_blocks = 8 * std::max(1, std::min((d.n_jchunks / 8 + 3) / 4, 256));
  if (const char* jw = std::getenv("SFM_JAC_WG_PER_XCD")) {
    const int v = std::atoi(jw);
    if (v > 0) d.jac_blocks = 8 * std::max(1, std::min((d.n_jchunks / 8 + 3) / 4, v));
  }
  const char* ss = std::getenv("SFM_SMALL_SETUP");
  c.small = c.plan.host_counts && !(ss && ss[0] == '0') &&
            hostlayout::small_setup_fits(c.N, c.C, c.P, c.cam_cnt.data() + 4,
                                         reinterpret_cast<const int32_t*>(c.h->stage + c.plan.o_pc));
  c.timer.mark("camera runs (host)");
}

int alloc_layouts(Setup& c) {
  DevProblem& d = c.d;
  const size_t N = size_t(c.N), npad = size_t(d.N_pad);
  const int64_t nch = d.n_jchunks;
  const int64_t nmax = std::max<int64_t>({c.N, nch, 1});
  c.sort_bytes = std::max({setup_sort_bytes(c.N, 64), setup_sort_bytes(nmax, 32), setup_sort_bytes(c.P + 1, 1),
                           setup_sort_bytes(c.N + 1, 2), size_t(256)});
  uint8_t* tb = nullptr;
  const bool ok = (c.small || c.alloc(d.pt_off, size_t(c.P) + 1)) &&
                  c.alloc(d.order, N) && c.alloc(d.uv_pm, 2 * N) && c.alloc(d.cam_pm, N) && c.alloc(d.cam_obs, npad) &&
                  c.alloc(d.cm_p, npad) && c.alloc(d.jchunks, size_t(std::max(1, d.n_jchunks))) &&
                  c.alloc(d.jgrp, size_t(9)) && c.alloc(d.uv_cm, 2 * npad) && c.alloc(d.pos, N) &&
                  c.tmp(c.k64a, N) && c.tmp(c.k64b, N) && c.tmp(c.k32a, size_t(nmax)) && c.tmp(c.k32b, size_t(nmax)) &&
                  c.tmp(c.iota, size_t(nmax)) && c.tmp(c.pt_s, N) && c.tmp(c.cm_order, N) &&
                  c.tmp(c.perm, size_t(std::max<int64_t>(1, nch))) && c.tmp(tb, c.sort_bytes);
  c.sort_tmp = tb;
  return ok ? 0 : c.rc;
}

int upload_runs_blob(Setup& c) {
  DevProblem& d = c.d;
  const hostlayout::SetupPlan& pl = c.plan;
  const hostlayout::Runs& r = c.runs;
  const bool small = c.small;
  StageLayout il;
  const size_t o_rng = il.add(sizeof(int32_t) * r.cam_rng.size()), o_w = il.add(sizeof(int32_t) * r.wcam.size()),
               o_off = il.add(sizeof(int32_t) * r.cam_off.size()),
               o_ch = il.add(sizeof(hostlayout::Chunk) * r.chunks.size());
  const size_t o_poff = small ? il.add(sizeof(int32_t) * (size_t(c.P) + 1)) : 0,
               o_fill = small ? il.add(sizeof(int32_t) * (size_t(c.P) + size_t(c.C))) : 0;
  if (pl.il_base && il.bytes > pl.il_bound) return fail(SFM_EIO, "internal: camera-run blob above its bound");
  if (int rc = stage_reserve(c.h, pl.il_base + il.bytes)) return rc;
  if (pl.route == ParamRoute::Early && pl.il_base + il.bytes > pl.pl_base)
    return fail(SFM_EIO, "internal: stage layout overlap");
  uint8_t* stg = c.h->stage;
  uint8_t* ib = nullptr;
  if (!c.alloc(ib, il.bytes)) return c.rc;
  uint8_t* sb = stg + pl.il_base;
  std::memcpy(sb + o_rng, r.cam_rng.data(), sizeof(int32_t) * r.cam_rng.size());
  std::memcpy(sb + o_w, r.wcam.data(), sizeof(int32_t) * r.wcam.size());
  std::memcpy(sb + o_off, r.cam_off.data(), sizeof(int32_t) * r.cam_off.size());
  if (!r.chunks.empty()) std::memcpy(sb + o_ch, r.chunks.data(), sizeof(hostlayout::Chunk) * r.chunks.size());
  if (small) {
    const int32_t* pc = reinterpret_cast<const int32_t*>(stg + pl.o_pc);
    int32_t* po = reinterpret_cast<int32_t*>(sb + o_poff);
    po[0] = 0;
    for (int p = 0; p < c.P; ++p) po[p + 1] = po[p] + pc[p];
    std::memset(sb + o_fill, 0, sizeof(int32_t) * (size_t(c.P) + size_t(c.C)));
  }
  if (pl.deferred_uv) {
    void* sbd = nullptr;
    HIPCHK(hipHostGetDevicePointer(&sbd, sb, 0));
    launch_copy_from_host(ib, sbd, (il.bytes + 15) / 16 * 16, c.s);
  } else {
    HIPCHK(hipMemcpyAsync(ib, sb, il.bytes, hipMemcpyHostToDevice, c.s));
  }
  if (small) {
    d.pt_off = reinterpret_cast<int32_t*>(ib + o_poff);
    c.small_fill = reinterpret_cast<int32_t*>(ib + o_fill);
  }
  d.cam_rng = reinterpret_cast<int32_t*>(ib + o_rng);
  d.wcam = reinterpret_cast<int32_t*>(ib + o_w);
  c.d_cam_off = reinterpret_cast<int32_t*>(ib + o_off);
  c.ch_in = reinterpret_cast<int4*>(ib + o_ch);
  return 0;
}

int upload_params_early(Setup& c) {
  if (int rc = alloc_params(c)) return rc;
  uint8_t* ps = c.h->stage + c.plan.pl_base;
  fill_param_stage(c, ps);
  HIPCHK(hipMemcpyAsync(c.d.Kc, ps, c.plan.pl_bytes, hipMemcpyHostToDevice, c.s));
  return 0;
}

int layout_small(Setup& c) {
  DevProblem& d = c.d;
  hipStream_t s = c.s;
  int32_t* small_cnt = nullptr;
  d.n_blk = int64_t(c.C) * (c.C + 1) / 2;
  if (!(c.alloc(d.seg, size_t(d.n_blk) + 1) && c.tmp(small_cnt, std::max<size_t>(1, size_t(d.n_blk))))) return c.rc;
  c.timer.mark("allocs + camera-run blob");
  launch_small_pm(c.N, c.in_pt, c.in_cam, c.in_uv, d.pt_off, c.small_fill, reinterpret_cast<int32_t*>(c.k32a), d.order,
                  d.uv_pm, d.cam_pm, c.pt_s, s);
  launch_small_cm(c.N, c.C, d.cam_pm, c.d_cam_off, c.cm_order, s);
  launch_fill_cm(d.N_pad, d.wcam, d.cam_rng, c.d_cam_off, c.cm_order, c.pt_s, d.uv_pm, d.cm_p, d.uv_cm, d.cam_obs,
                 d.pos, s);
  launch_small_chunks(d.n_jchunks, c.ch_in, c.cm_order, c.pt_s, c.P, d.jchunks, d.jgrp, s);
  launch_small_pairs_count(c.C, d.n_blk, c.d_cam_off, c.cm_order, d.cam_pm, c.pt_s, d.pt_off, small_cnt, d.seg, s);
  c.n_pairs = std::max<int64_t>(1, 2 * c.pairs_est);
  d.xcd_slice_max = hostlayout::small_slice_max(c.C, c.cam_cnt.data() + 4, c.cam_slice);
  c.timer.mark("layout launches");
  return 0;
}

int layout_sorted(Setup& c) {
  DevProblem& d = c.d;
  hipStream_t s = c.s;
  const int64_t N = c.N;
  const int C = c.C, P = c.P, nch = d.n_jchunks;
  const bool deferred_uv = c.plan.deferred_uv;
  c.timer.mark("allocs + camera-run blob");
  launch_pm_keys(N, c.in_cam, c.in_pt, C, c.k64a, c.iota, s);
  HIPCHK(sort_pairs64(c.sort_tmp, c.sort_bytes, c.k64a, c.k64b, c.iota, d.order, N,
                      uint64_t(std::max(1, P)) * uint64_t(std::max(1, C)) - 1, s));
  launch_gather_pm(N, d.order, deferred_uv ? nullptr : c.in_uv, c.in_cam, c.in_pt, d.uv_pm, d.cam_pm, c.pt_s, c.k32a,
                   c.iota, s);
  if (deferred_uv) launch_pt_off(P, c.k64b, N, C, d.pt_off, s);
  else HIPCHK(exclusive_sum32(c.sort_tmp, c.sort_bytes, c.cnt_p, d.pt_off, int64_t(P) + 1, s));
  HIPCHK(sort_pairs32(c.sort_tmp, c.sort_bytes, c.k32a, c.k32b, c.iota, c.cm_order, N, uint64_t(std::max(1, C)) - 1,
                      s));
  launch_fill_cm(d.N_pad, d.wcam, d.cam_rng, c.d_cam_off, c.cm_order, c.pt_s, deferred_uv ? nullptr : d.uv_pm, d.cm_p,
                 d.uv_cm, d.cam_obs, d.pos, s);
  launch_chunk_keys(nch, c.ch_in, c.cm_order, c.pt_s, P, c.k32a, c.iota, s);
  HIPCHK(sort_pairs32(c.sort_tmp, c.sort_bytes, c.k32a, c.k32b, c.iota, c.perm, nch, 7, s));
  launch_chunk_gather(nch, c.perm, c.ch_in, c.k32b, d.jchunks, d.jgrp, s);
  int64_t* pcnt = nullptr;
  if (!(c.tmp(pcnt, size_t(N) + 1) && c.tmp(c.poff, size_t(N) + 1))) return c.rc;
  c.pair_order = env_flag("SFM_PAIRS_CM") ? c.cm_order : nullptr;
  launch_pair_count(N, c.pair_order, d.cam_pm, c.pt_s, d.pt_off, pcnt, s);
  HIPCHK(exclusive_sum64(c.sort_tmp, c.sort_bytes, pcnt, c.poff, N + 1, s));
  return 0;
}

int enqueue_total_readback(Setup& c) {
  uint8_t* stg = c.h->stage;
  if (!c.plan.deferred_uv) {
    HIPCHK(hipMemcpyAsync(stg, c.poff + c.N, sizeof(int64_t), hipMemcpyDeviceToHost, c.s));
    HIPCHK(hipMemcpyAsync(stg + 8, c.d.jgrp, 9 * sizeof(int32_t), hipMemcpyDeviceToHost, c.s));
    c.timer.mark("layout launches");
    return 0;
  }
  c.timer.mark("layout launches");
  void* stg_d = nullptr;
  HIPCHK(hipHostGetDevicePointer(&stg_d, stg, 0));
  uint8_t* sd = static_cast<uint8_t*>(stg_d);
  HostCopySet cs;
  cs.add(sd, c.poff + c.N, sizeof(int64_t));
  cs.add(sd + 8, c.d.jgrp, 9 * sizeof(int32_t));
  launch_copy_to_host(cs, c.s);
  return 0;
}
int read_pair_total(Setup& c) {
  const uint8_t* stg = c.h->stage;
  HIPCHK(hipStreamSynchronize(c.s));
  std::memcpy(&c.n_pairs, stg, sizeof(int64_t));
  int32_t g[9];
  std::memcpy(g, stg + 8, sizeof(g));
  c.d.xcd_slice_max = 0;
  for (int i = 0; i < 8; ++i) c.d.xcd_slice_max = std::max(c.d.xcd_slice_max, g[i + 1] - g[i]);
  c.timer.mark("layouts (device)");
  return 0;
}

int alloc_pair_lists(Setup& c) {
  DevProblem& d = c.d;
  if (c.n_pairs >= int64_t(INT32_MAX)) return fail(SFM_EINVAL, "too many Schur pairs for 32-bit offsets");
  d.n_blk = int64_t(c.C) * (c.C + 1) / 2;
  d.n_pairs = c.plan.host_counts && !c.cam_slice.empty() ? c.pairs_est : c.n_pairs;
  const hostlayout::SchurShape sh =
      hostlayout::schur_shape(d.n_pairs, d.n_blk, std::getenv("SFM_SCHUR_PTS_SUB"), std::getenv("SFM_SCHUR_WG"));
  d.schur_pts_sub = sh.pts_sub;
  d.schur_wg_blocks = sh.wg_blocks;
  if (!d.scal_host && hipHostMalloc(&d.scal_host, sizeof(double) * (kNumScalars + 1 + 17)) != hipSuccess) {
    d.scal_host = nullptr;
    return fail(SFM_ENOMEM, "hipHostMalloc failed");
  }
  c.grp_host = reinterpret_cast<int64_t*>(d.scal_host + kNumScalars + 1);
  c.uv_err_host = reinterpret_cast<int32_t*>(c.grp_host + 16);
  const bool ok = c.alloc(d.blk, std::max<size_t>(1, size_t(d.n_blk))) &&
                  (c.small || c.alloc(d.seg, size_t(d.n_blk) + 1)) &&
                  c.alloc(d.bpts, std::max<size_t>(1, size_t(c.n_pairs)));
  return ok ? 0 : c.rc;
}

void pair_lists_small(Setup& c) {
  DevProblem& d = c.d;
  launch_small_pairs_fill(c.C, d.n_blk, c.d_cam_off, c.cm_order, d.cam_pm, c.pt_s, d.pt_off, d.seg, d.bpts, c.s);
  launch_blk(c.C, d.blk, c.s);
  d.bperm = nullptr;
  d.srec = nullptr;
  d.n_bslots = d.n_blk;
}

int pair_lists_sorted(Setup& c) {
  DevProblem& d = c.d;
  hipStream_t s = c.s;
  const int64_t n_pairs = c.n_pairs;
  uint32_t *bk_a = nullptr, *bk_b = nullptr;
  int32_t* bv = nullptr;
  const int64_t nk = std::max<int64_t>({n_pairs, d.n_blk, 1});
  if (!(c.tmp(bk_a, size_t(nk)) && c.tmp(bk_b, size_t(nk)) && c.tmp(bv, size_t(nk)))) return c.rc;
  const size_t need = std::max(setup_sort_bytes(n_pairs, 32), setup_sort_bytes(d.n_blk, 32));
  if (need > c.sort_bytes) {
    uint8_t* tb = nullptr;
    if (!c.tmp(tb, need)) return c.rc;
    c.sort_tmp = tb;
    c.sort_bytes = need;
  }
  launch_pair_fill(c.N, c.pair_order, d.cam_pm, c.pt_s, d.pt_off, c.poff, c.C, bk_a, bv, s);
  HIPCHK(sort_pairs32(c.sort_tmp, c.sort_bytes, bk_a, bk_b, bv, d.bpts, n_pairs,
                      uint64_t(std::max<int64_t>(1, d.n_blk)) - 1, s));
  launch_seg(d.n_blk, bk_b, n_pairs, d.seg, s);
  launch_blk(c.C, d.blk, s);
  d.bperm = nullptr;
  d.srec = nullptr;
  d.n_bslots = d.n_blk;
  if (d.n_blk > kSchurXcdMinBlocks) {
    const int per = 64 / d.schur_pts_sub * (kThreads / 64);
    int32_t *sorted = nullptr, *row_x = nullptr;
    int64_t* grp = nullptr;
    if (!(c.tmp(sorted, size_t(d.n_blk)) && c.tmp(row_x, size_t(c.C)) && c.tmp(grp, 16) &&
          c.alloc(d.bperm, size_t(bperm_slots_bound(d.n_blk, per))) &&
          c.alloc(d.srec, size_t(bperm_slots_bound(d.n_blk, per)))))
      return c.rc;
    HIPCHK(launch_bperm(c.C, d.n_blk, n_pairs, d.seg, d.blk, per, bk_a, bk_b, bv, sorted, row_x, grp, c.sort_tmp,
                        c.sort_bytes, d.bperm, d.srec, s));
    HIPCHK(hipMemcpyAsync(c.grp_host, grp, sizeof(int64_t) * 16, hipMemcpyDeviceToHost, s));
    c.bperm_per = per;
  }
  return 0;
}

int alloc_solver_arrays(Setup& c) {
  sfm_ba_handle* h = c.h;
  DevProblem& d = c.d;
  const size_t C = size_t(c.C), P = size_t(c.P), N = size_t(c.N), npad = size_t(d.N_pad);
  d.n = 6 * c.C;
  d.ld = ((d.n + 1 + kNB - 1) / kNB) * kNB;
  d.nblk = d.ld / kNB;
  d.max_blocks = std::max({1, c.C, blocks_for(c.N, 256), blocks_for(c.P, 256), d.jac_blocks, d.jac_blocks_rec,
                           blocks_for(d.N_pad, 256), obs_xcd_blocks(d), pt_xcd_blocks(d)});
  if (c.plan.route == ParamRoute::Late || c.plan.route == ParamRoute::None)
    if (int rc = alloc_params(c)) return rc;
  d.pm_backsub = d.n_blk > kSchurXcdMinBlocks && c.C <= kCamPMMax;
  const char* ec = std::getenv("SFM_EU_CM");
  d.eu_cm = !(ec && ec[0] == '0');
  d.ptG = nullptr;
  d.camS = nullptr;
  h->force_pack = env_flag("SFM_FORCE_PACK");
  const char* ov = std::getenv("SFM_OVERLAP");
  d.overlap = (ov ? std::atoi(ov) : 0) > 0 && d.nblk > 2 && !sharded(h) ? 1 : 0;
  const size_t tiles = size_t(d.nblk) * d.nblk;
  bool ok = c.alloc(d.cam_new, 6 * C) && c.alloc(d.X_new, 3 * P) && c.alloc(d.scale_c, 6 * C) &&
            c.alloc(d.scale_p, 3 * P) && c.alloc(d.diag_c, 6 * C) && c.alloc(d.diag_p, 3 * P) &&
            c.alloc(d.camR, size_t(kCamR) * C) && c.alloc(d.camRn, 12 * C) &&
            c.alloc(d.eu, size_t(kEU) * (d.eu_cm ? npad : N)) && c.alloc(d.ypt, 3 * P) &&
            c.alloc(d.ptV, size_t(kPtV) * P) && c.alloc(d.ptL, size_t(kPtL) * P) &&
            c.alloc(d.ptS, size_t(kPtS) * std::max<size_t>(1, P)) &&
            (d.n_blk <= kSchurXcdMinBlocks || c.alloc(d.ptG, size_t(kPtG) * std::max<size_t>(1, P))) &&
            (d.n_blk <= kSchurXcdMinBlocks || c.alloc(d.camS, size_t(kCamSR) * std::max<size_t>(1, C))) &&
            c.alloc(d.Ucam, size_t(kUcam) * C) && c.alloc(d.jpart, 27 * std::max<size_t>(1, npad / 64)) &&
            c.alloc(d.dpart, 27 * std::max<size_t>(1, npad / 64)) && c.alloc(d.S, size_t(d.ld) * d.ld) &&
            (!(sharded(h) || h->force_pack) || c.alloc(d.Spack, packed_size(d.n))) &&
            c.alloc(d.invL, size_t(d.nblk) * kNB * kNB) && c.alloc(d.flags, size_t(d.nblk)) &&
            c.alloc(d.cflags, 2 * tiles) &&
            c.alloc(d.cticket, 5);
  if (!ok) return c.rc;
  const char* sw = std::getenv("SFM_SCHUR_WGS");
  d.schur_wgs = sw ? std::min(1 << 16, std::max(0, std::atoi(sw)) + 7) / 8 * 8 : 0;
  if (d.overlap) {
    if (!(c.alloc(d.tile_cnt, tiles) && c.alloc(d.tile_exp, tiles))) return c.rc;
    std::vector<int32_t> te(tiles, 0);
    for (int c1 = 0; c1 < c.C; ++c1)
      for (int c2 = c1; c2 < c.C; ++c2)
        for (int I = 6 * c2 / kNB; I <= (6 * c2 + 5) / kNB; ++I)
          for (int J = 6 * c1 / kNB; J <= (6 * c1 + 5) / kNB; ++J) ++te[size_t(I) * d.nblk + J];
    HIPCHK(hipMemcpy(d.tile_exp, te.data(), sizeof(int32_t) * te.size(), hipMemcpyHostToDevice));
  }
  ok = c.alloc(d.ysol, size_t(d.ld)) && c.alloc(d.fail, size_t(1)) &&
       c.alloc(d.partials, size_t(kNumPartialSlots) * d.max_blocks) &&
       c.alloc(d.scal, size_t(kNumScalars) + 1);
  return ok ? 0 : c.rc;
}

int layout_deferred_uv(Setup& c) {
  sfm_ba_handle* h = c.h;
  DevProblem& d = c.d;
  c.worker.join();
  if (c.uv_state.load(std::memory_order_acquire) != 1) return fail(SFM_EIO, "observation upload failed");
  c.timer.mark("uv upload (worker)");
  hipStream_t u = h->ustream;
  launch_uv_layout(c.N, d.N_pad, d.order, d.wcam, d.cam_rng, c.d_cam_off, c.cm_order, c.in_uv, d.uv_pm, d.uv_cm, c.err,
                   u);
  void* ue_d = nullptr;
  HIPCHK(hipHostGetDevicePointer(&ue_d, c.uv_err_host, 0));
  HostCopySet cs;
  cs.add(ue_d, c.err + 2, sizeof(int32_t));
  launch_copy_to_host(cs, u);
  HIPCHK(hipEventRecord(h->uev_uv, u));
  return 0;
}

int finish_params(Setup& c) {
  switch (c.plan.route) {
    case ParamRoute::None:
    case ParamRoute::Early:
      return 0;
    case ParamRoute::Side:
      if (c.plan.deferred_uv && c.param_state.load(std::memory_order_acquire) != 1)
        return fail(SFM_EIO, "parameter upload failed");
      HIPCHK(hipStreamWaitEvent(c.s, c.h->uev, 0));
      return 0;
    case ParamRoute::Late: {
      if (int rc = stage_reserve(c.h, c.plan.pl_bytes)) return rc;
      fill_param_stage(c, c.h->stage);
      HIPCHK(hipMemcpyAsync(c.d.Kc, c.h->stage, c.plan.pl_bytes, hipMemcpyHostToDevice, c.s));
      return 0;
    }
  }
  return 0;
}

int finish(Setup& c) {
  sfm_ba_handle* h = c.h;
  DevProblem& d = c.d;
  hipStream_t s = c.s;
  {
    Fill32Set fs;
    fs.add(d.S, sizeof(double) * size_t(d.ld) * d.ld, 0);
    fs.add(d.invL, sizeof(double) * size_t(d.nblk) * kNB * kNB, 0);
    fs.add(d.flags, sizeof(int32_t) * size_t(d.nblk), 0);
    fs.add(d.cflags, sizeof(int32_t) * 2 * size_t(d.nblk) * d.nblk, 0);
    fs.add(d.cticket, 5 * sizeof(unsigned long long), 0);
    fs.add(d.partials, sizeof(double) * size_t(kNumPartialSlots) * d.max_blocks, 0);
    launch_fill32(fs, s);
  }
  h->chol_epoch = 0;
  h->bs_epoch = 0;
  d.n_cu = h->n_cu;
  c.timer.mark("pairs + params launches");
  static const bool sync_setup = env_flag("SFM_SYNC_SETUP");
  const bool deferred_uv = c.plan.deferred_uv;
  if (deferred_uv) HIPCHK(hipStreamWaitEvent(s, h->uev_uv, 0));
  if (c.small && c.plan.route == ParamRoute::Early && !c.bperm_per && !sync_setup) return 0;
  HIPCHK(hipStreamSynchronize(s));
  if (deferred_uv && *c.uv_err_host != INT32_MAX)
    return fail(SFM_EINVAL, "non-finite observation at " + std::to_string(*c.uv_err_host));
  if (c.bperm_per) {
    int64_t m_max = 1;
    for (int x = 0; x < 8; ++x) m_max = std::max<int64_t>(m_max, (c.grp_host[8 + x] + c.bperm_per - 1) / c.bperm_per);
    d.n_bslots = m_max * 8 * c.bperm_per;
  }
  retire_tmps(h);
  c.timer.mark("pair lists + uploads (device)");
  return 0;
}

int run_setup(Setup& c, const double* K9, const double* rot, const double* t) {
  const hostlayout::SetupPlan& plan = c.plan;
  const bool side = plan.route == ParamRoute::Side;
  int rc = 0;
  if ((rc = open_uploads(c, K9, rot, t))) return rc;
  if ((rc = upload_inputs(c))) return rc;
  if (!plan.host_counts && (rc = validate_on_device(c))) return rc;
  c.timer.mark("upload + validate");
  if ((rc = report_first_bad_observation(c))) return rc;
  camera_runs(c);
  if ((rc = alloc_layouts(c))) return rc;
  if ((rc = upload_runs_blob(c))) return rc;
  if (plan.route == ParamRoute::Early && (rc = upload_params_early(c))) return rc;
  if (c.small) {
    if ((rc = layout_small(c))) return rc;
  } else {
    if ((rc = layout_sorted(c))) return rc;
    if ((rc = enqueue_total_readback(c))) return rc;
    if (side && !plan.deferred_uv) {
      if ((rc = enqueue_side_params(c))) return rc;
      c.timer.mark("parameter upload (side stream)");
    }
    if ((rc = read_pair_total(c))) return rc;
  }
  if ((rc = alloc_pair_lists(c))) return rc;
  if (c.small) pair_lists_small(c);
  else if ((rc = pair_lists_sorted(c))) return rc;
  if ((rc = alloc_solver_arrays(c))) return rc;
  release_pool(c.h);
  if (plan.deferred_uv && (rc = layout_deferred_uv(c))) return rc;
  if (side && c.small && (rc = enqueue_side_params(c))) return rc;
  if ((rc = finish_params(c))) return rc;
  return finish(c);
}

}

int sfm_ba_set_problem(sfm_ba_handle* h, int64_t n_obs, const double* obs_uv, const int32_t* cam_idx,
                       const int32_t* pt_idx, int32_t n_cams, const double* K9, const double* rot, const double* t,
                       int32_t n_pts, const double* X) {
  SFM_TRACE("sfm_ba_set_problem");
  if (!h) return fail(SFM_EINVAL, "handle is NULL");
  if (n_obs < 0 || n_cams < 0 || n_pts < 0) return fail(SFM_EINVAL, "negative size");
  if (n_obs > 0 && (!obs_uv || !cam_idx || !pt_idx)) return fail(SFM_EINVAL, "observation arrays are NULL");
  if (n_cams > 0 && (!K9 || !rot || !t)) return fail(SFM_EINVAL, "camera arrays are NULL");
  if (n_pts > 0 && !X) return fail(SFM_EINVAL, "point array is NULL");
  if (n_obs > int64_t(INT32_MAX) - 64 * int64_t(n_cams))
    return fail(SFM_EINVAL, "more than 2^31-1 observations per shard");
  Setup c(h, n_obs, obs_uv, cam_idx, pt_idx, n_cams, n_pts, X);
  HIPCHK(hipSetDevice(h->device));
  HIPCHK(hipStreamSynchronize(h->stream));
  free_problem(h);
  c.timer.mark("sync + free");
  h->d.C = n_cams;
  h->d.P = n_pts;
  h->d.N = n_obs;
  ProblemGuard guard{c};
  if (int rc = run_setup(c, K9, rot, t)) return rc;
  guard.committed = true;
  h->has_problem = true;
  return 0;
}
```

### sfm_amd/csrc/ba_setup.h

```cpp
#pragma once
#include <hip/hip_runtime.h>
#include <cstddef>
#include <cstdint>

#include "ba_host_layout.h"

namespace sfm {

size_t setup_sort_bytes(int64_t n, int which);
hipError_t sort_pairs64(void* tmp, size_t bytes, const uint64_t* kin, uint64_t* kout, const int32_t* vin,
                        int32_t* vout, int64_t n, uint64_t max_key, hipStream_t s);
hipError_t sort_pairs32(void* tmp, size_t bytes, const uint32_t* kin, uint32_t* kout, const int32_t* vin,
                        int32_t* vout, int64_t n, uint64_t max_key, hipStream_t s);
hipError_t exclusive_sum32(void* tmp, size_t bytes, const int32_t* in, int32_t* out, int64_t n, hipStream_t s);
hipError_t exclusive_sum64(void* tmp, size_t bytes, const int64_t* in, int64_t* out, int64_t n, hipStream_t s);

struct Fill32Set {
  struct Job { uint32_t* p; int64_t n; uint32_t v; } job[8];
  int n = 0;
  void add(void* p, size_t bytes, uint32_t v) { job[n++] = Job{static_cast<uint32_t*>(p), int64_t(bytes / 4), v}; }
};
void launch_fill32(const Fill32Set& fs, hipStream_t s);
struct HostCopySet {
  int n = 0;
  int32_t* dst[4];
  const int32_t* src[4];
  int words[4];
  void add(void* d, const void* s, size_t bytes) {
    dst[n] = static_cast<int32_t*>(d);
    src[n] = static_cast<const int32_t*>(s);
    words[n] = int(bytes / 4);
    ++n;
  }
};
void launch_copy_to_host(const HostCopySet& cs, hipStream_t s);
void launch_copy_from_host(void* dst, const void* src_host_mapped, size_t bytes, hipStream_t s);

void launch_validate(int64_t N, const double* uv, const int32_t* cam, const int32_t* pt, int C, int P, int32_t* err,
                     int32_t* cam_cnt, int32_t* pt_cnt, hipStream_t s);
void launch_pm_keys(int64_t N, const int32_t* cam, const int32_t* pt, int C, uint64_t* keys, int32_t* iota,
                    hipStream_t s);
void launch_gather_pm(int64_t N, const int32_t* order, const double* uv, const int32_t* cam, const int32_t* pt,
                      double* uv_pm, int32_t* cam_pm, int32_t* pt_s, uint32_t* cam_key, int32_t* iota, hipStream_t s);
void launch_fill_cm(int64_t N_pad, const int32_t* wcam, const int32_t* cam_rng, const int32_t* cam_off,
                    const int32_t* cm_order, const int32_t* pt_s, const double* uv_pm, int32_t* cm_p, double* uv_cm,
                    int32_t* cam_obs, int32_t* pos, hipStream_t s);
void launch_uv_layout(int64_t N, int64_t N_pad, const int32_t* order, const int32_t* wcam, const int32_t* cam_rng,
                      const int32_t* cam_off, const int32_t* cm_order, const double* uv, double* uv_pm, double* uv_cm,
                      int32_t* err, hipStream_t s);
void launch_pt_off(int P, const uint64_t* sorted_keys, int64_t N, int C, int32_t* pt_off, hipStream_t s);
void launch_chunk_keys(int n, const int4* ch, const int32_t* cm_order, const int32_t* pt_s, int P, uint32_t* key,
                       int32_t* iota, hipStream_t s);
void launch_chunk_gather(int n, const int32_t* perm, const int4* ch, const uint32_t* key, int4* out, int32_t* grp,
                         hipStream_t s);
void launch_pair_count(int64_t N, const int32_t* cm_order, const int32_t* cam_pm, const int32_t* pt_s,
                       const int32_t* pt_off, int64_t* cnt, hipStream_t s);
void launch_pair_fill(int64_t N, const int32_t* cm_order, const int32_t* cam_pm, const int32_t* pt_s,
                      const int32_t* pt_off, const int64_t* off, int C, uint32_t* key, int32_t* val, hipStream_t s);
void launch_seg(int64_t n_blk, const uint32_t* key, int64_t n_pairs, int32_t* seg, hipStream_t s);
void launch_blk(int C, int2* blk, hipStream_t s);
void launch_small_pm(int64_t N, const int32_t* pt, const int32_t* cam, const double* uv, const int32_t* pt_off,
                     int32_t* fill, int32_t* tmp, int32_t* order, double* uv_pm, int32_t* cam_pm, int32_t* pt_s,
                     hipStream_t s);
void launch_small_cm(int64_t N, int C, const int32_t* cam_pm, const int32_t* cam_off, int32_t* cm_order,
                     hipStream_t s);
void launch_small_chunks(int n, const int4* ch, const int32_t* cm_order, const int32_t* pt_s, int P, int4* out,
                         int32_t* grp, hipStream_t s);
void launch_small_pairs_count(int C, int64_t n_blk, const int32_t* cam_off, const int32_t* cm_order,
                              const int32_t* cam_pm, const int32_t* pt_s, const int32_t* pt_off, int32_t* cnt,
                              int32_t* seg, hipStream_t s);
void launch_small_pairs_fill(int C, int64_t n_blk, const int32_t* cam_off, const int32_t* cm_order,
                             const int32_t* cam_pm, const int32_t* pt_s, const int32_t* pt_off, const int32_t* seg,
                             int32_t* bpts, hipStream_t s);
int64_t bperm_slots_bound(int64_t n_blk, int per);
hipError_t launch_bperm(int C, int64_t n_blk, int64_t n_pairs, const int32_t* seg, const int2* blk, int per,
                        uint32_t* key_a, uint32_t* key_b, int32_t* iota, int32_t* sorted, int32_t* row_x,
                        int64_t* grp, void* sort_tmp, size_t sort_bytes, int32_t* bperm, int4* srec, hipStream_t s);

}
```

### sfm_amd/csrc/ba_setup.hip

```cpp
#include <hip/hip_runtime.h>
#include <algorithm>
#include <hipcub/hipcub.hpp>
#include <climits>
#include <cmath>
#include "ba_setup.h"

namespace sfm {
namespace {

constexpr int kT = 256;
inline int nblocks(int64_t n) { return int(std::max<int64_t>(1, (n + kT - 1) / kT)); }

constexpr int kLdsCams = 8192;
__global__ __launch_bounds__(kT) void k_validate(int64_t N, const double* __restrict__ uv,
                                                 const int32_t* __restrict__ cam, const int32_t* __restrict__ pt, int C,
                                                 int P, int32_t* __restrict__ err, int32_t* __restrict__ cam_cnt,
                                                 int32_t* __restrict__ pt_cnt) {
  __shared__ int32_t hist[kLdsCams];
  const bool lds = C <= kLdsCams;
  if (lds)
    for (int c = threadIdx.x; c < C; c += kT) hist[c] = 0;
  __syncthreads();
  for (int64_t i = int64_t(blockIdx.x) * kT + threadIdx.x; i < N; i += int64_t(gridDim.x) * kT) {
    const int c = cam[i], p = pt[i];
    const bool cok = c >= 0 && c < C, pok = p >= 0 && p < P;
    if (!cok) atomicMin(err + 0, int32_t(i));
    if (!pok) atomicMin(err + 1, int32_t(i));
    if (uv) {
      const double2 u = reinterpret_cast<const double2*>(uv)[i];
      if (!(isfinite(u.x) && isfinite(u.y))) atomicMin(err + 2, int32_t(i));
    }
    if (cok && pok) {
      if (lds) atomicAdd(hist + c, 1);
      else atomicAdd(cam_cnt + c, 1);
      if (pt_cnt) atomicAdd(pt_cnt + p, 1);
    }
  }
  __syncthreads();
  if (lds)
    for (int c = threadIdx.x; c < C; c += kT)
      if (hist[c]) atomicAdd(cam_cnt + c, hist[c]);
}

__global__ __launch_bounds__(kT) void k_pm_keys(int64_t N, const int32_t* __restrict__ cam,
                                                const int32_t* __restrict__ pt, int C, uint64_t* __restrict__ keys,
                                                int32_t* __restrict__ iota) {
  const int64_t i = int64_t(blockIdx.x) * kT + threadIdx.x;
  if (i >= N) return;
  keys[i] = uint64_t(pt[i]) * uint64_t(C) + uint64_t(cam[i]);
  iota[i] = int32_t(i);
}

__global__ __launch_bounds__(kT) void k_gather_pm(int64_t N, const int32_t* __restrict__ order,
                                                  const double* __restrict__ uv, const int32_t* __restrict__ cam,
                                                  const int32_t* __restrict__ pt, double* __restrict__ uv_pm,
                                                  int32_t* __restrict__ cam_pm, int32_t* __restrict__ pt_s,
                                                  uint32_t* __restrict__ cam_key, int32_t* __restrict__ iota) {
  const int64_t q = int64_t(blockIdx.x) * kT + threadIdx.x;
  if (q >= N) return;
  const int64_t i = order[q];
  if (uv) reinterpret_cast<double2*>(uv_pm)[q] = reinterpret_cast<const double2*>(uv)[i];
  const int c = cam[i];
  cam_pm[q] = c;
  pt_s[q] = pt[i];
  cam_key[q] = uint32_t(c);
  iota[q] = int32_t(q);
}

__global__ __launch_bounds__(kT) void k_fill_cm(int64_t N_pad, const int32_t* __restrict__ wcam,
                                                const int32_t* __restrict__ cam_rng,
                                                const int32_t* __restrict__ cam_off,
                                                const int32_t* __restrict__ cm_order,
                                                const int32_t* __restrict__ pt_s, const double* __restrict__ uv_pm,
                                                int32_t* __restrict__ cm_p, double* __restrict__ uv_cm,
                                                int32_t* __restrict__ cam_obs, int32_t* __restrict__ pos) {
  const int64_t i = int64_t(blockIdx.x) * kT + threadIdx.x;
  if (i >= N_pad) return;
  const int c = wcam[i >> 6];
  const int32_t j = int32_t(i - cam_rng[2 * c]);
  const int32_t n_c = cam_off[c + 1] - cam_off[c];
  const int32_t q = cm_order[cam_off[c] + min(j, n_c - 1)];
  cm_p[i] = pt_s[q];
  if (uv_pm) reinterpret_cast<double2*>(uv_cm)[i] = reinterpret_cast<const double2*>(uv_pm)[q];
  cam_obs[i] = j < n_c ? q : -1;
  if (j < n_c) pos[q] = int32_t(i);
}

__global__ __launch_bounds__(kT) void k_uv_layout(int64_t N, int64_t N_pad, const int32_t* __restrict__ order,
                                                  const int32_t* __restrict__ wcam,
                                                  const int32_t* __restrict__ cam_rng,
                                                  const int32_t* __restrict__ cam_off,
                                                  const int32_t* __restrict__ cm_order, const double* __restrict__ uv,
                                                  double* __restrict__ uv_pm, double* __restrict__ uv_cm,
                                                  int32_t* __restrict__ err) {
  const int64_t i = int64_t(blockIdx.x) * kT + threadIdx.x;
  if (i < N) {
    const int32_t o = order[i];
    const double2 u = reinterpret_cast<const double2*>(uv)[o];
    reinterpret_cast<double2*>(uv_pm)[i] = u;
    if (!(isfinite(u.x) && isfinite(u.y))) atomicMin(err + 2, o);
  }
  if (i < N_pad) {
    const int c = wcam[i >> 6];
    const int32_t j = int32_t(i - cam_rng[2 * c]);
    const int32_t n_c = cam_off[c + 1] - cam_off[c];
    const int32_t q = cm_order[cam_off[c] + min(j, n_c - 1)];
    reinterpret_cast<double2*>(uv_cm)[i] = reinterpret_cast<const double2*>(uv)[order[q]];
  }
}

__global__ __launch_bounds__(kT) void k_chunk_keys(int n, const int4* __restrict__ ch,
                                                   const int32_t* __restrict__ cm_order,
                                                   const int32_t* __restrict__ pt_s, int P, uint32_t* __restrict__ key,
                                                   int32_t* __restrict__ iota) {
  const int t = blockIdx.x * kT + threadIdx.x;
  if (t >= n) return;
  const int p0 = pt_s[cm_order[ch[t].w]];
  key[t] = uint32_t(int64_t(p0) * 8 / max(1, P));
  iota[t] = t;
}

__global__ __launch_bounds__(kT) void k_chunk_gather(int n, const int32_t* __restrict__ perm,
                                                     const int4* __restrict__ ch, const uint32_t* __restrict__ key,
                                                     int4* __restrict__ out, int32_t* __restrict__ grp) {
  const int t = blockIdx.x * kT + threadIdx.x;
  if (t < n) {
    const int4 v = ch[perm[t]];
    out[t] = make_int4(v.x, v.y, v.z, 0);
  }
  if (t <= 8) {
    int lo = 0, hi = n;
    while (lo < hi) {
      const int mid = (lo + hi) >> 1;
      if (int(key[mid]) < t) lo = mid + 1; else hi = mid;
    }
    grp[t] = lo;
  }
}

__global__ __launch_bounds__(kT) void k_pair_count(int64_t N, const int32_t* __restrict__ cm_order,
                                                   const int32_t* __restrict__ cam_pm,
                                                   const int32_t* __restrict__ pt_s,
                                                   const int32_t* __restrict__ pt_off, int64_t* __restrict__ cnt) {
  const int64_t i = int64_t(blockIdx.x) * kT + threadIdx.x;
  if (i > N) return;
  if (i == N) { cnt[N] = 0; return; }
  const int32_t o1 = cm_order ? cm_order[i] : int32_t(i);
  const int c1 = cam_pm[o1], p = pt_s[o1];
  int64_t k = 0;
  for (int32_t o2 = pt_off[p]; o2 < pt_off[p + 1]; ++o2) k += (cam_pm[o2] >= c1 && o2 != o1) ? 1 : 0;
  cnt[i] = k;
}

__device__ __forceinline__ int64_t row_start(int c1, int C) { return int64_t(c1) * C - int64_t(c1) * (c1 - 1) / 2; }

__global__ __launch_bounds__(kT) void k_pair_fill(int64_t N, const int32_t* __restrict__ cm_order,
                                                  const int32_t* __restrict__ cam_pm, const int32_t* __restrict__ pt_s,
                                                  const int32_t* __restrict__ pt_off, const int64_t* __restrict__ off,
                                                  int C, uint32_t* __restrict__ key, int32_t* __restrict__ val) {
  const int64_t i = int64_t(blockIdx.x) * kT + threadIdx.x;
  if (i >= N) return;
  const int32_t o1 = cm_order ? cm_order[i] : int32_t(i);
  const int c1 = cam_pm[o1], p = pt_s[o1];
  const int64_t rs = row_start(c1, C) - c1;
  int64_t k = off[i];
  for (int32_t o2 = pt_off[p]; o2 < pt_off[p + 1]; ++o2) {
    const int c2 = cam_pm[o2];
    if (c2 >= c1 && o2 != o1) {
      key[k] = uint32_t(rs + c2);
      val[k] = p;
      ++k;
    }
  }
}

__global__ __launch_bounds__(kT) void k_pt_off(int P, const uint64_t* __restrict__ key, int64_t N, int C,
                                               int32_t* __restrict__ pt_off) {
  const int64_t p = int64_t(blockIdx.x) * kT + threadIdx.x;
  if (p > P) return;
  const uint64_t t = uint64_t(p) * uint64_t(C);
  int64_t lo = 0, hi = N;
  while (lo < hi) {
    const int64_t mid = (lo + hi) >> 1;
    if (key[mid] < t) lo = mid + 1; else hi = mid;
  }
  pt_off[p] = int32_t(lo);
}

__global__ __launch_bounds__(kT) void k_seg(int64_t n_blk, const uint32_t* __restrict__ key, int64_t n_pairs,
                                            int32_t* __restrict__ seg) {
  const int64_t b = int64_t(blockIdx.x) * kT + threadIdx.x;
  if (b > n_blk) return;
  int64_t lo = 0, hi = n_pairs;
  while (lo < hi) {
    const int64_t mid = (lo + hi) >> 1;
    if (int64_t(key[mid]) < b) lo = mid + 1; else hi = mid;
  }
  seg[b] = int32_t(lo);
}

__global__ __launch_bounds__(kT) void k_blk(int C, int2* __restrict__ blk) {
  const int c1 = blockIdx.y;
  const int64_t rs = row_start(c1, C) - c1;
  for (int c2 = c1 + int(blockIdx.x) * kT + int(threadIdx.x); c2 < C; c2 += int(gridDim.x) * kT)
    blk[rs + c2] = make_int2(c1, c2);
}

__global__ __launch_bounds__(kT) void k_bperm_rows(int C, const int32_t* __restrict__ seg, int64_t n_pairs,
                                                   int64_t n_blk, int32_t* __restrict__ row_x,
                                                   int64_t* __restrict__ grp) {
  __shared__ int64_t sc[kT];
  __shared__ int64_t carry;
  __shared__ unsigned long long gfirst[8], gsize[8];
  const int t = threadIdx.x;
  if (t < 8) {
    gfirst[t] = ~0ull;
    gsize[t] = 0;
  }
  if (t == 0) carry = 0;
  __syncthreads();
  const int64_t total = n_pairs > 0 ? n_pairs : n_blk;
  for (int base = 0; base < C; base += kT) {
    const int c1 = base + t;
    int64_t first = 0, nb = 0, w = 0;
    if (c1 < C) {
      first = row_start(c1, C);
      nb = C - c1;
      w = n_pairs > 0 ? int64_t(seg[first + nb]) - seg[first] : nb;
    }
    sc[t] = w;
    __syncthreads();
    for (int o = 1; o < kT; o <<= 1) {
      const int64_t v = t >= o ? sc[t - o] : 0;
      __syncthreads();
      sc[t] += v;
      __syncthreads();
    }
    const int64_t before = carry + sc[t] - w;
    if (c1 < C) {
      const int x = int(min<int64_t>(7, (8 * (before + w / 2)) / max<int64_t>(1, total)));
      row_x[c1] = x;
      atomicMin(&gfirst[x], (unsigned long long)first);
      atomicAdd(&gsize[x], (unsigned long long)nb);
    }
    __syncthreads();
    if (t == kT - 1) carry += sc[kT - 1];
    __syncthreads();
  }
  if (t < 8) {
    grp[t] = gsize[t] ? int64_t(gfirst[t]) : 0;
    grp[8 + t] = int64_t(gsize[t]);
  }
}

__global__ __launch_bounds__(kT) void k_bperm_keys(int64_t n_blk, const int2* __restrict__ blk,
                                                   const int32_t* __restrict__ seg, int cbits,
                                                   uint32_t* __restrict__ key, int32_t* __restrict__ iota) {
  const int64_t b = int64_t(blockIdx.x) * kT + threadIdx.x;
  if (b >= n_blk) return;
  const uint32_t cmax = (1u << cbits) - 1u;
  const uint32_t cnt = min(uint32_t(seg[b + 1] - seg[b]), cmax);
  key[b] = (uint32_t(blk[b].x) << cbits) | (cmax - cnt);
  iota[b] = int32_t(b);
}

__global__ __launch_bounds__(kT) void k_bperm_fill(int64_t n_blk, const int32_t* __restrict__ sorted,
                                                   const int2* __restrict__ blk, const int32_t* __restrict__ row_x,
                                                   const int64_t* __restrict__ grp, int per,
                                                   const int32_t* __restrict__ seg, int32_t* __restrict__ bperm,
                                                   int4* __restrict__ srec) {
  const int64_t p = int64_t(blockIdx.x) * kT + threadIdx.x;
  if (p >= n_blk) return;
  const int32_t b = sorted[p];
  const int2 cc = blk[b];
  const int x = row_x[cc.x];
  const int64_t i = p - grp[x];
  const int64_t k = ((i / per) * 8 + x) * per + i % per;
  bperm[k] = b;
  srec[k] = make_int4(cc.x, cc.y, seg[b], seg[b + 1]);
}

__global__ __launch_bounds__(kT) void k_copy_from_host(uint4* __restrict__ dst, const uint4* __restrict__ src,
                                                       int64_t n16) {
  for (int64_t i = int64_t(blockIdx.x) * kT + threadIdx.x; i < n16; i += int64_t(gridDim.x) * kT) dst[i] = src[i];
}

__global__ __launch_bounds__(kT) void k_fill32(Fill32Set fs) {
  const Fill32Set::Job f = fs.job[blockIdx.y];
  const int64_t n4 = (reinterpret_cast<uintptr_t>(f.p) & 15) ? 0 : f.n / 4;
  const uint4 v4 = make_uint4(f.v, f.v, f.v, f.v);
  const int64_t t0 = int64_t(blockIdx.x) * kT + threadIdx.x, st = int64_t(gridDim.x) * kT;
  for (int64_t i = t0; i < n4; i += st) reinterpret_cast<uint4*>(f.p)[i] = v4;
  for (int64_t i = 4 * n4 + t0; i < f.n; i += st) f.p[i] = f.v;
}


__global__ __launch_bounds__(kT) void k_small_pm_scatter(int64_t N, const int32_t* __restrict__ pt,
                                                         const int32_t* __restrict__ pt_off,
                                                         int32_t* __restrict__ fill, int32_t* __restrict__ tmp) {
  const int64_t i = int64_t(blockIdx.x) * kT + threadIdx.x;
  if (i >= N) return;
  const int p = pt[i];
  tmp[pt_off[p] + atomicAdd(fill + p, 1)] = int32_t(i);
}
__global__ __launch_bounds__(kT) void k_small_pm_rank(int64_t N, const int32_t* __restrict__ pt_off,
                                                      const int32_t* __restrict__ tmp,
                                                      const int32_t* __restrict__ cam, const int32_t* __restrict__ pt,
                                                      const double* __restrict__ uv, int32_t* __restrict__ order,
                                                      double* __restrict__ uv_pm, int32_t* __restrict__ cam_pm,
                                                      int32_t* __restrict__ pt_s) {
  const int64_t s = int64_t(blockIdx.x) * kT + threadIdx.x;
  if (s >= N) return;
  const int32_t i = tmp[s];
  const int p = pt[i], c = cam[i];
  const int q0 = pt_off[p], q1 = pt_off[p + 1];
  int rank = 0;
  for (int q = q0; q < q1; ++q) {
    const int32_t j = tmp[q];
    const int cj = cam[j];
    rank += (cj < c || (cj == c && j < i)) ? 1 : 0;
  }
  const int dst = q0 + rank;
  order[dst] = i;
  reinterpret_cast<double2*>(uv_pm)[dst] = reinterpret_cast<const double2*>(uv)[i];
  cam_pm[dst] = c;
  pt_s[dst] = p;
}
constexpr int kSmallCmMaxSteps = int(kSmallSetupMaxObs / 1024);
__global__ __launch_bounds__(1024) void k_small_cm_compact(int64_t N, const int32_t* __restrict__ cam_pm,
                                                           const int32_t* __restrict__ cam_off,
                                                           int32_t* __restrict__ cm_order) {
  __shared__ int cnt[kSmallCmMaxSteps * 16];
  const int c = blockIdx.x, t = threadIdx.x, l = t & 63, w = t >> 6;
  const uint64_t lt = (l == 0) ? 0ull : (~0ull >> (64 - l));
  const int K = int((N + 1023) / 1024);
  uint64_t hits = 0;
#pragma unroll 8
  for (int k = 0; k < K; ++k) {
    const int64_t q = int64_t(k) * 1024 + t;
    if (q < N && cam_pm[q] == c) hits |= 1ull << k;
  }
  for (int k = 0; k < K; ++k) {
    const uint64_t m = __builtin_amdgcn_ballot_w64((hits >> k) & 1);
    if (l == 0) cnt[16 * k + w] = __popcll(m);
  }
  __syncthreads();
  __shared__ int wsum[16];
  const int ne = 16 * K;
  const int v = t < ne ? cnt[t] : 0;
  int incl = v;
#pragma unroll
  for (int off = 1; off < 64; off <<= 1) {
    const int o = __shfl_up(incl, off);
    if (l >= off) incl += o;
  }
  if (l == 63) wsum[w] = incl;
  __syncthreads();
  int wbase = 0;
  for (int u = 0; u < w; ++u) wbase += wsum[u];
  if (t < ne) cnt[t] = wbase + incl - v;
  __syncthreads();
  const int base = cam_off[c];
  for (int k = 0; k < K; ++k) {
    const uint64_t m = __builtin_amdgcn_ballot_w64((hits >> k) & 1);
    if ((hits >> k) & 1) cm_order[base + cnt[16 * k + w] + __popcll(m & lt)] = int32_t(int64_t(k) * 1024 + t);
  }
}
constexpr int kSmallChunks = 2048;
__global__ __launch_bounds__(1024) void k_small_chunks(int n, const int4* __restrict__ ch,
                                                       const int32_t* __restrict__ cm_order,
                                                       const int32_t* __restrict__ pt_s, int P, int4* __restrict__ out,
                                                       int32_t* __restrict__ grp) {
  __shared__ unsigned char key[kSmallChunks];
  for (int t = threadIdx.x; t < n; t += 1024)
    key[t] = (unsigned char)(int64_t(pt_s[cm_order[ch[t].w]]) * 8 / max(1, P));
  __syncthreads();
  if (threadIdx.x >= 64) return;
  const int l = threadIdx.x;
  const uint64_t lt = (l == 0) ? 0ull : (~0ull >> (64 - l));
  int cnt[8] = {0, 0, 0, 0, 0, 0, 0, 0};
  for (int b = 0; b < n; b += 64) {
    const int t = b + l, k = t < n ? int(key[t]) : -1;
#pragma unroll
    for (int g = 0; g < 8; ++g) cnt[g] += __popcll(__builtin_amdgcn_ballot_w64(k == g));
  }
  int start[9];
  start[0] = 0;
#pragma unroll
  for (int g = 0; g < 8; ++g) start[g + 1] = start[g] + cnt[g];
  if (l <= 8) {
    int v = 0;
#pragma unroll
    for (int g = 0; g <= 8; ++g) v = l == g ? start[g] : v;
    grp[l] = v;
  }
  for (int b = 0; b < n; b += 64) {
    const int t = b + l, k = t < n ? int(key[t]) : -1;
    int dst = 0;
#pragma unroll
    for (int g = 0; g < 8; ++g) {
      const uint64_t m = __builtin_amdgcn_ballot_w64(k == g);
      if (k == g) dst = start[g] + __popcll(m & lt);
      start[g] += __popcll(m);
    }
    if (t < n) {
      const int4 v = ch[t];
      out[dst] = make_int4(v.x, v.y, v.z, 0);
    }
  }
}
__device__ __forceinline__ int2 small_block(int64_t b, int C) {
  int c1 = 0;
  while (c1 + 1 < C && int64_t(c1 + 1) * C - int64_t(c1 + 1) * c1 / 2 <= b) ++c1;
  const int64_t rs = int64_t(c1) * C - int64_t(c1) * (c1 - 1) / 2 - c1;
  return make_int2(c1, int(b - rs));
}
__device__ __forceinline__ int small_pairs_of(int i, int c1, int c2, const int32_t* __restrict__ cm_order,
                                              const int32_t* __restrict__ cam_pm, const int32_t* __restrict__ pt_s,
                                              const int32_t* __restrict__ pt_off, int& p) {
  const int32_t o1 = cm_order[i];
  p = pt_s[o1];
  const int q0 = pt_off[p], q1 = pt_off[p + 1];
  int k = 0;
  for (int q = q0; q < q1; q += 4) {
    int cj[4];
#pragma unroll
    for (int j = 0; j < 4; ++j) cj[j] = cam_pm[min(q + j, q1 - 1)];
#pragma unroll
    for (int j = 0; j < 4; ++j) k += (q + j < q1 && cj[j] == c2) ? 1 : 0;
  }
  return k - (c2 == c1 ? 1 : 0);
}
__global__ __launch_bounds__(kT) void k_small_pair_count(int C, const int32_t* __restrict__ cam_off,
                                                         const int32_t* __restrict__ cm_order,
                                                         const int32_t* __restrict__ cam_pm,
                                                         const int32_t* __restrict__ pt_s,
                                                         const int32_t* __restrict__ pt_off, int32_t* __restrict__ cnt) {
  __shared__ int sh[kT / 64];
  const int2 cc = small_block(blockIdx.x, C);
  int k = 0, p;
  for (int i = cam_off[cc.x] + threadIdx.x; i < cam_off[cc.x + 1]; i += kT)
    k += small_pairs_of(i, cc.x, cc.y, cm_order, cam_pm, pt_s, pt_off, p);
  for (int off = 32; off > 0; off >>= 1) k += __shfl_xor(k, off);
  if ((threadIdx.x & 63) == 0) sh[threadIdx.x >> 6] = k;
  __syncthreads();
  if (threadIdx.x == 0) cnt[blockIdx.x] = sh[0] + sh[1] + sh[2] + sh[3];
}
__global__ __launch_bounds__(1024) void k_small_scan(int64_t n, const int32_t* __restrict__ cnt,
                                                     int32_t* __restrict__ seg) {
  __shared__ int32_t part[1024];
  const int t = threadIdx.x;
  const int64_t per = (n + 1023) / 1024, a = std::min<int64_t>(n, t * per), e = std::min<int64_t>(n, a + per);
  int32_t sum = 0;
  for (int64_t i = a; i < e; ++i) sum += cnt[i];
  part[t] = sum;
  __syncthreads();
  for (int off = 1; off < 1024; off <<= 1) {
    const int32_t v = t >= off ? part[t - off] : 0;
    __syncthreads();
    part[t] += v;
    __syncthreads();
  }
  int32_t run = part[t] - sum;
  for (int64_t i = a; i < e; ++i) {
    seg[i] = run;
    run += cnt[i];
  }
  if (t == 1023) seg[n] = part[t];
}
__global__ __launch_bounds__(kT) void k_small_pair_fill(int C, const int32_t* __restrict__ cam_off,
                                                        const int32_t* __restrict__ cm_order,
                                                        const int32_t* __restrict__ cam_pm,
                                                        const int32_t* __restrict__ pt_s,
                                                        const int32_t* __restrict__ pt_off,
                                                        const int32_t* __restrict__ seg, int32_t* __restrict__ bpts) {
  __shared__ int sc[kT];
  const int2 cc = small_block(blockIdx.x, C);
  const int t = threadIdx.x, i0 = cam_off[cc.x], i1 = cam_off[cc.x + 1];
  int run = seg[blockIdx.x];
  for (int b = i0; b < i1; b += kT) {
    const int i = b + t;
    int p = 0;
    const int k = i < i1 ? small_pairs_of(i, cc.x, cc.y, cm_order, cam_pm, pt_s, pt_off, p) : 0;
    sc[t] = k;
    __syncthreads();
    for (int off = 1; off < kT; off <<= 1) {
      const int v = t >= off ? sc[t - off] : 0;
      __syncthreads();
      sc[t] += v;
      __syncthreads();
    }
    for (int j = 0; j < k; ++j) bpts[run + sc[t] - k + j] = p;
    run += sc[kT - 1];
    __syncthreads();
  }
}

int bits_for(uint64_t max_key) {
  int b = 1;
  while (b < 64 && (max_key >> b) != 0) ++b;
  return b;
}

}

size_t setup_sort_bytes(int64_t n, int which) {
  size_t bytes = 0;
  if (n <= 0) return 0;
  if (which == 64)
    (void)hipcub::DeviceRadixSort::SortPairs(nullptr, bytes, (const uint64_t*)nullptr, (uint64_t*)nullptr,
                                             (const int32_t*)nullptr, (int32_t*)nullptr, int(n));
  else if (which == 32)
    (void)hipcub::DeviceRadixSort::SortPairs(nullptr, bytes, (const uint32_t*)nullptr, (uint32_t*)nullptr,
                                             (const int32_t*)nullptr, (int32_t*)nullptr, int(n));
  else if (which == 1)
    (void)hipcub::DeviceScan::ExclusiveSum(nullptr, bytes, (const int32_t*)nullptr, (int32_t*)nullptr, int(n));
  else
    (void)hipcub::DeviceScan::ExclusiveSum(nullptr, bytes, (const int64_t*)nullptr, (int64_t*)nullptr, int(n));
  return bytes;
}

hipError_t sort_pairs64(void* tmp, size_t bytes, const uint64_t* kin, uint64_t* kout, const int32_t* vin,
                        int32_t* vout, int64_t n, uint64_t max_key, hipStream_t s) {
  if (n <= 0) return hipSuccess;
  return hipcub::DeviceRadixSort::SortPairs(tmp, bytes, kin, kout, vin, vout, int(n), 0, bits_for(max_key), s);
}
hipError_t sort_pairs32(void* tmp, size_t bytes, const uint32_t* kin, uint32_t* kout, const int32_t* vin,
                        int32_t* vout, int64_t n, uint64_t max_key, hipStream_t s) {
  if (n <= 0) return hipSuccess;
  return hipcub::DeviceRadixSort::SortPairs(tmp, bytes, kin, kout, vin, vout, int(n), 0, bits_for(max_key), s);
}
hipError_t exclusive_sum32(void* tmp, size_t bytes, const int32_t* in, int32_t* out, int64_t n, hipStream_t s) {
  if (n <= 0) return hipSuccess;
  return hipcub::DeviceScan::ExclusiveSum(tmp, bytes, in, out, int(n), s);
}
hipError_t exclusive_sum64(void* tmp, size_t bytes, const int64_t* in, int64_t* out, int64_t n, hipStream_t s) {
  if (n <= 0) return hipSuccess;
  return hipcub::DeviceScan::ExclusiveSum(tmp, bytes, in, out, int(n), s);
}

void launch_validate(int64_t N, const double* uv, const int32_t* cam, const int32_t* pt, int C, int P, int32_t* err,
                     int32_t* cam_cnt, int32_t* pt_cnt, hipStream_t s) {
  if (N <= 0) return;
  k_validate<<<std::min(nblocks(N), 1024), kT, 0, s>>>(N, uv, cam, pt, C, P, err, cam_cnt, pt_cnt);
}
void launch_pm_keys(int64_t N, const int32_t* cam, const int32_t* pt, int C, uint64_t* keys, int32_t* iota,
                    hipStream_t s) {
  if (N > 0) k_pm_keys<<<nblocks(N), kT, 0, s>>>(N, cam, pt, C, keys, iota);
}
void launch_gather_pm(int64_t N, const int32_t* order, const double* uv, const int32_t* cam, const int32_t* pt,
                      double* uv_pm, int32_t* cam_pm, int32_t* pt_s, uint32_t* cam_key, int32_t* iota,
                      hipStream_t s) {
  if (N > 0) k_gather_pm<<<nblocks(N), kT, 0, s>>>(N, order, uv, cam, pt, uv_pm, cam_pm, pt_s, cam_key, iota);
}
void launch_fill_cm(int64_t N_pad, const int32_t* wcam, const int32_t* cam_rng, const int32_t* cam_off,
                    const int32_t* cm_order, const int32_t* pt_s, const double* uv_pm, int32_t* cm_p, double* uv_cm,
                    int32_t* cam_obs, int32_t* pos, hipStream_t s) {
  if (N_pad > 0)
    k_fill_cm<<<nblocks(N_pad), kT, 0, s>>>(N_pad, wcam, cam_rng, cam_off, cm_order, pt_s, uv_pm, cm_p, uv_cm, cam_obs,
                                            pos);
}
void launch_uv_layout(int64_t N, int64_t N_pad, const int32_t* order, const int32_t* wcam, const int32_t* cam_rng,
                      const int32_t* cam_off, const int32_t* cm_order, const double* uv, double* uv_pm, double* uv_cm,
                      int32_t* err, hipStream_t s) {
  const int64_t n = std::max(N, N_pad);
  if (n > 0)
    k_uv_layout<<<nblocks(n), kT, 0, s>>>(N, N_pad, order, wcam, cam_rng, cam_off, cm_order, uv, uv_pm, uv_cm, err);
}
void launch_chunk_keys(int n, const int4* ch, const int32_t* cm_order, const int32_t* pt_s, int P, uint32_t* key,
                       int32_t* iota, hipStream_t s) {
  if (n > 0) k_chunk_keys<<<nblocks(n), kT, 0, s>>>(n, ch, cm_order, pt_s, P, key, iota);
}
void launch_chunk_gather(int n, const int32_t* perm, const int4* ch, const uint32_t* key, int4* out, int32_t* grp,
                         hipStream_t s) {
  k_chunk_gather<<<nblocks(std::max(n, 9)), kT, 0, s>>>(n, perm, ch, key, out, grp);
}
void launch_pair_count(int64_t N, const int32_t* cm_order, const int32_t* cam_pm, const int32_t* pt_s,
                       const int32_t* pt_off, int64_t* cnt, hipStream_t s) {
  k_pair_count<<<nblocks(N + 1), kT, 0, s>>>(N, cm_order, cam_pm, pt_s, pt_off, cnt);
}
void launch_pair_fill(int64_t N, const int32_t* cm_order, const int32_t* cam_pm, const int32_t* pt_s,
                      const int32_t* pt_off, const int64_t* off, int C, uint32_t* key, int32_t* val, hipStream_t s) {
  if (N > 0) k_pair_fill<<<nblocks(N), kT, 0, s>>>(N, cm_order, cam_pm, pt_s, pt_off, off, C, key, val);
}
void launch_pt_off(int P, const uint64_t* sorted_keys, int64_t N, int C, int32_t* pt_off, hipStream_t s) {
  k_pt_off<<<nblocks(int64_t(P) + 1), kT, 0, s>>>(P, sorted_keys, N, C, pt_off);
}
void launch_seg(int64_t n_blk, const uint32_t* key, int64_t n_pairs, int32_t* seg, hipStream_t s) {
  k_seg<<<nblocks(n_blk + 1), kT, 0, s>>>(n_blk, key, n_pairs, seg);
}
void launch_copy_from_host(void* dst, const void* src_host_mapped, size_t bytes, hipStream_t s) {
  const int64_t n16 = int64_t(bytes / 16);
  if (n16 > 0)
    k_copy_from_host<<<int(std::min<int64_t>(nblocks(n16), 256)), kT, 0, s>>>(
        static_cast<uint4*>(dst), static_cast<const uint4*>(src_host_mapped), n16);
}
__global__ __launch_bounds__(kT) void k_copy_to_host(HostCopySet cs) {
  for (int k = 0; k < cs.n; ++k)
    for (int i = threadIdx.x; i < cs.words[k]; i += kT) cs.dst[k][i] = cs.src[k][i];
}
void launch_copy_to_host(const HostCopySet& cs, hipStream_t s) {
  if (cs.n > 0) k_copy_to_host<<<1, kT, 0, s>>>(cs);
}
void launch_fill32(const Fill32Set& fs, hipStream_t s) {
  if (fs.n == 0) return;
  int64_t mx = 1;
  for (int i = 0; i < fs.n; ++i) mx = std::max(mx, fs.job[i].n);
  const unsigned gx = unsigned(std::min<int64_t>(1024, (mx + kT - 1) / kT));
  k_fill32<<<dim3(gx, unsigned(fs.n)), kT, 0, s>>>(fs);
}
void launch_blk(int C, int2* blk, hipStream_t s) {
  if (C > 0) k_blk<<<dim3(unsigned((C + kT - 1) / kT), unsigned(C)), kT, 0, s>>>(C, blk);
}
void launch_small_pm(int64_t N, const int32_t* pt, const int32_t* cam, const double* uv, const int32_t* pt_off,
                     int32_t* fill, int32_t* tmp, int32_t* order, double* uv_pm, int32_t* cam_pm, int32_t* pt_s,
                     hipStream_t s) {
  if (N <= 0) return;
  k_small_pm_scatter<<<nblocks(N), kT, 0, s>>>(N, pt, pt_off, fill, tmp);
  k_small_pm_rank<<<nblocks(N), kT, 0, s>>>(N, pt_off, tmp, cam, pt, uv, order, uv_pm, cam_pm, pt_s);
}
void launch_small_cm(int64_t N, int C, const int32_t* cam_pm, const int32_t* cam_off, int32_t* cm_order,
                     hipStream_t s) {
  if (N <= 0 || C <= 0 || N > kSmallSetupMaxObs) return;
  k_small_cm_compact<<<C, 1024, 0, s>>>(N, cam_pm, cam_off, cm_order);
}
void launch_small_chunks(int n, const int4* ch, const int32_t* cm_order, const int32_t* pt_s, int P, int4* out,
                         int32_t* grp, hipStream_t s) {
  k_small_chunks<<<1, 1024, 0, s>>>(n, ch, cm_order, pt_s, P, out, grp);
}
void launch_small_pairs_count(int C, int64_t n_blk, const int32_t* cam_off, const int32_t* cm_order,
                              const int32_t* cam_pm, const int32_t* pt_s, const int32_t* pt_off, int32_t* cnt,
                              int32_t* seg, hipStream_t s) {
  if (n_blk <= 0) return;
  k_small_pair_count<<<unsigned(n_blk), kT, 0, s>>>(C, cam_off, cm_order, cam_pm, pt_s, pt_off, cnt);
  k_small_scan<<<1, 1024, 0, s>>>(n_blk, cnt, seg);
}
void launch_small_pairs_fill(int C, int64_t n_blk, const int32_t* cam_off, const int32_t* cm_order,
                             const int32_t* cam_pm, const int32_t* pt_s, const int32_t* pt_off, const int32_t* seg,
                             int32_t* bpts, hipStream_t s) {
  if (n_blk > 0) k_small_pair_fill<<<unsigned(n_blk), kT, 0, s>>>(C, cam_off, cm_order, cam_pm, pt_s, pt_off, seg, bpts);
}
int64_t bperm_slots_bound(int64_t n_blk, int per) { return std::max<int64_t>(1, (n_blk + per - 1) / per) * 8 * per; }
hipError_t launch_bperm(int C, int64_t n_blk, int64_t n_pairs, const int32_t* seg, const int2* blk, int per,
                        uint32_t* key_a, uint32_t* key_b, int32_t* iota, int32_t* sorted, int32_t* row_x,
                        int64_t* grp, void* sort_tmp, size_t sort_bytes, int32_t* bperm, int4* srec, hipStream_t s) {
  hipError_t e = hipMemsetAsync(bperm, 0xFF, sizeof(int32_t) * size_t(bperm_slots_bound(n_blk, per)), s);
  if (e == hipSuccess) e = hipMemsetAsync(srec, 0xFF, sizeof(int4) * size_t(bperm_slots_bound(n_blk, per)), s);
  if (e != hipSuccess || n_blk <= 0) return e;
  k_bperm_rows<<<1, kT, 0, s>>>(C, seg, n_pairs, n_blk, row_x, grp);
  const int cbits = 32 - bits_for(uint64_t(std::max(1, C)) - 1);
  k_bperm_keys<<<nblocks(n_blk), kT, 0, s>>>(n_blk, blk, seg, cbits, key_a, iota);
  e = sort_pairs32(sort_tmp, sort_bytes, key_a, key_b, iota, sorted, n_blk, ~uint64_t(0) >> 32, s);
  if (e != hipSuccess) return e;
  k_bperm_fill<<<nblocks(n_blk), kT, 0, s>>>(n_blk, sorted, blk, row_x, grp, per, seg, bperm, srec);
  return hipGetLastError();
}

}
```

Measured before the change: 1.880 billion residual-evals/s (obs x evaluations).

## Add wave-major interleaved layout for per-point observation streams

Builds a wave-major copy of the per-point camera index and uv arrays, so that each wavefront of 64 points reads its k-th observations from consecutive addresses, padded to the longest point in the wave. Point evaluation and point back-substitution kernels walk this layout with a stride of 64 instead of each lane reading its own contiguous run, which is meant to make those loads coalesced. It costs extra setup kernels, a device-to-host read of the slot count, and extra memory for padding. A fit check falls back to the old layout when padding would be excessive.

```diff
diff --git a/sfm_amd/csrc/ba_device.h b/sfm_amd/csrc/ba_device.h
--- a/sfm_amd/csrc/ba_device.h
+++ b/sfm_amd/csrc/ba_device.h
@@ -104,6 +104,9 @@
   double* jpart = nullptr;
   double* uv_pm = nullptr;
   int32_t* cam_pm = nullptr;
+  int32_t* woff = nullptr;
+  double* uv_wm = nullptr;
+  int32_t* cam_wm = nullptr;
   double* partials = nullptr;
   int32_t max_blocks = 0;
   double* scal = nullptr;
diff --git a/sfm_amd/csrc/ba_host_layout.h b/sfm_amd/csrc/ba_host_layout.h
--- a/sfm_amd/csrc/ba_host_layout.h
+++ b/sfm_amd/csrc/ba_host_layout.h
@@ -92,6 +92,10 @@
   for (int p = 0; p < P; ++p)
     if (n_obs_of_pt[p] > kSmallSetupMaxPtObs) return false;
   return true;
+}
+
+inline bool wave_major_fits(int64_t slots, int64_t N, int P) {
+  return 128 * slots <= 3 * N + 128 * ((int64_t(P) + 63) / 64);
 }
 
 struct SchurShape {
diff --git a/sfm_amd/csrc/ba_kernels.hip b/sfm_amd/csrc/ba_kernels.hip
--- a/sfm_amd/csrc/ba_kernels.hip
+++ b/sfm_amd/csrc/ba_kernels.hip
@@ -340,9 +340,17 @@
   double* part_bad;
 };
 
-__device__ __forceinline__ void point_eval_body(int p, const int32_t* __restrict__ pt_off,
-                                                const int32_t* __restrict__ cam_pm,
-                                                const double* __restrict__ uv_pm, const CamView cv,
+struct PmStream {
+  const int32_t* pt_off; const int32_t* cam; const double* uv; const int32_t* woff;
+};
+__device__ __forceinline__ void pm_lane(const PmStream& ps, int p, size_t& q0, int& stride, int& cnt) {
+  const int a = ps.pt_off[p];
+  cnt = ps.pt_off[p + 1] - a;
+  q0 = ps.woff ? size_t(ps.woff[p >> 6]) * 64 + size_t(p & 63) : size_t(a);
+  stride = ps.woff ? 64 : 1;
+}
+
+__device__ __forceinline__ void point_eval_body(int p, const PmStream& ps, const CamView cv,
                                                 const double* __restrict__ X, double* __restrict__ scale_p,
                                                 double* __restrict__ diag_p, double* __restrict__ ptV,
                                                 double min_diag, double max_diag, int mode, int reuse, double& g,
@@ -352,15 +360,18 @@
   double sp[3] = {1.0, 1.0, 1.0};
   if (mode == 1)
     for (int k = 0; k < 3; ++k) sp[k] = scale_p[3 * size_t(p) + k];
-  const int q0 = pt_off[p], q1 = pt_off[p + 1];
-  int c_n = q0 < q1 ? cam_pm[q0] : 0;
-  double2 uv_n = q0 < q1 ? ld2(uv_pm + 2 * size_t(q0)) : make_double2(0.0, 0.0);
-  for (int q = q0; q < q1; ++q) {
+  size_t q;
+  int qs, cnt;
+  pm_lane(ps, p, q, qs, cnt);
+  int c_n = cnt > 0 ? ps.cam[q] : 0;
+  double2 uv_n = cnt > 0 ? ld2(ps.uv + 2 * q) : make_double2(0.0, 0.0);
+  for (int k = 0; k < cnt; ++k) {
     const int c = c_n;
     const double2 uvo = uv_n;
-    if (q + 1 < q1) {
-      c_n = cam_pm[q + 1];
-      uv_n = ld2(uv_pm + 2 * size_t(q + 1));
+    if (k + 1 < cnt) {
+      q += size_t(qs);
+      c_n = ps.cam[q];
+      uv_n = ld2(ps.uv + 2 * q);
     }
     const double* cr = cv.R + size_t(cv.sR) * c;
     const double* k5 = cv.K + size_t(cv.sK) * c;
@@ -410,9 +421,7 @@
   }
 }
 
-__global__ __launch_bounds__(kThreads) void k_point_eval_rc(int P, const int32_t* __restrict__ pt_off,
-                                                            const int32_t* __restrict__ cam_pm,
-                                                            const double* __restrict__ uv_pm,
+__global__ __launch_bounds__(kThreads) void k_point_eval_rc(int P, const PmStream ps,
                                                             const double* __restrict__ camR,
                                                             const double* __restrict__ cam,
                                                             const double* __restrict__ Kc,
@@ -428,8 +437,7 @@
   double g = 0.0, xn = 0.0, bad = 0.0;
   const CamView cv{camR, cam + 3, Kc, kCamR, 6, 5};
   if (p < P)
-    point_eval_body(p, pt_off, cam_pm, uv_pm, cv, X, scale_p, diag_p, ptV, min_diag, max_diag, mode, reuse, g, xn, pf,
-                    bad);
+    point_eval_body(p, ps, cv, X, scale_p, diag_p, ptV, min_diag, max_diag, mode, reuse, g, xn, pf, bad);
   if (mode == 1) {
     const double rg = block_reduce(g, sh, true);
     if (threadIdx.x == 0) part_grad[blockIdx.x] = rg;
@@ -444,9 +452,7 @@
 
 constexpr int kCamE = 17;
 template <int kMaxC, int kGroups = 1>
-__global__ __launch_bounds__(kThreads * kGroups) void k_point_eval_lds(int P, int C, const int32_t* __restrict__ pt_off,
-                                                             const int32_t* __restrict__ cam_pm,
-                                                             const double* __restrict__ uv_pm,
+__global__ __launch_bounds__(kThreads * kGroups) void k_point_eval_lds(int P, int C, const PmStream ps,
                                                              const double* __restrict__ camR,
                                                              const double* __restrict__ cam,
                                                              const double* __restrict__ Kc,
@@ -477,8 +483,7 @@
   double g = 0.0, xn = 0.0, bad = 0.0;
   const CamView cv{cst, cst + 9, cst + 12, kCamE, kCamE, kCamE};
   if (p < P)
-    point_eval_body(p, pt_off, cam_pm, uv_pm, cv, X, scale_p, diag_p, ptV, min_diag, max_diag, mode, reuse, g, xn, pf,
-                    bad);
+    point_eval_body(p, ps, cv, X, scale_p, diag_p, ptV, min_diag, max_diag, mode, reuse, g, xn, pf, bad);
   if (mode == 1) {
     const int w = int(threadIdx.x) >> 6, l = int(threadIdx.x) & 63;
     __shared__ double shb[4 * kGroups];
@@ -1619,8 +1624,7 @@
 
 template <int kGroups>
 __global__ __launch_bounds__(kThreads * kGroups) void k_backsub_pm(
-    int P, int C, const int32_t* __restrict__ pt_off, const int32_t* __restrict__ cam_pm,
-    const double* __restrict__ uv_pm, const double* __restrict__ ptL,
+    int P, int C, const PmStream ps, const double* __restrict__ ptL,
     const double* __restrict__ ptV, const double* __restrict__ scale_p, const double* __restrict__ X,
     double* __restrict__ X_new, double* __restrict__ ypt, double* __restrict__ part_model,
     double* __restrict__ part_model_pt, double* __restrict__ part_step, double* __restrict__ part_bad,
@@ -1663,16 +1667,20 @@
   if (p < P) {
     const double Xp[3] = {X[3 * size_t(p)], X[3 * size_t(p) + 1], X[3 * size_t(p) + 2]};
     const double sp[3] = {scale_p[3 * size_t(p)], scale_p[3 * size_t(p) + 1], scale_p[3 * size_t(p) + 2]};
-    const int q0 = pt_off[p], q1 = pt_off[p + 1];
-    int c_n = q0 < q1 ? cam_pm[q0] : 0;
-    double2 uv_n = q0 < q1 ? ld2(uv_pm + 2 * size_t(q0)) : make_double2(0.0, 0.0);
+    size_t q0, q;
+    int qs, cnt;
+    pm_lane(ps, p, q0, qs, cnt);
+    q = q0;
+    int c_n = cnt > 0 ? ps.cam[q] : 0;
+    double2 uv_n = cnt > 0 ? ld2(ps.uv + 2 * q) : make_double2(0.0, 0.0);
     double h0 = 0.0, h1 = 0.0, h2 = 0.0;
-    for (int q = q0; q < q1; ++q) {
+    for (int i = 0; i < cnt; ++i) {
       const double* k = cst + kCamPM * c_n;
       const double2 uvo = uv_n;
-      if (q + 1 < q1) {
-        c_n = cam_pm[q + 1];
-        uv_n = ld2(uv_pm + 2 * size_t(q + 1));
+      if (i + 1 < cnt) {
+        q += size_t(qs);
+        c_n = ps.cam[q];
+        uv_n = ld2(ps.uv + 2 * q);
       }
       const double y0 = k[0] * Xp[0] + k[1] * Xp[1] + k[2] * Xp[2];
       const double y1 = k[3] * Xp[0] + k[4] * Xp[1] + k[5] * Xp[2];
@@ -1719,14 +1727,16 @@
       X_new[3 * size_t(p) + j] = Xn[j];
       ypt[3 * size_t(p) + j] = ys[j];
     }
-    c_n = q0 < q1 ? cam_pm[q0] : 0;
-    uv_n = q0 < q1 ? ld2(uv_pm + 2 * size_t(q0)) : make_double2(0.0, 0.0);
-    for (int q = q0; q < q1; ++q) {
+    q = q0;
+    c_n = cnt > 0 ? ps.cam[q] : 0;
+    uv_n = cnt > 0 ? ld2(ps.uv + 2 * q) : make_double2(0.0, 0.0);
+    for (int i = 0; i < cnt; ++i) {
       const double* k = cst + kCamPM * c_n;
       const double2 uvo = uv_n;
-      if (q + 1 < q1) {
-        c_n = cam_pm[q + 1];
-        uv_n = ld2(uv_pm + 2 * size_t(q + 1));
+      if (i + 1 < cnt) {
+        q += size_t(qs);
+        c_n = ps.cam[q];
+        uv_n = ld2(ps.uv + 2 * q);
       }
       const double* Rn = k + 23;
       double pc[3];
@@ -1809,6 +1819,9 @@
 void launch_cam_reduce(const DevProblem& d, hipStream_t s) {
   if (d.C) k_cam_sum<<<d.C, 64, 0, s>>>(d.cam_rng, d.jpart, d.Ucam, d.gate);
 }
+static PmStream pm_stream(const DevProblem& d) {
+  return d.uv_wm ? PmStream{d.pt_off, d.cam_wm, d.uv_wm, d.woff} : PmStream{d.pt_off, d.cam_pm, d.uv_pm, nullptr};
+}
 static CamFold cam_fold(const DevProblem& d, int mode, bool count_grad) {
   return CamFold{d.cam_rng, d.jpart, d.Ucam, d.scale_c, d.diag_c, d.min_diag, d.max_diag, mode, d.C,
                  count_grad ? slot(d, kPGradCam) : nullptr};
@@ -1819,7 +1832,7 @@
 bool launch_point_eval_with_cams(const DevProblem& d, int mode, bool count_grad, hipStream_t s) {
   if (d.P == 0 || d.C == 0 || d.C > 64) return false;
   const int nb = blocks_for(d.P, kThreads) + (d.C + kThreads / 64 - 1) / (kThreads / 64);
-  k_point_eval_lds<64><<<nb, kThreads, 0, s>>>(d.P, d.C, d.pt_off, d.cam_pm, d.uv_pm, d.camR, d.cam, d.Kc, d.X,
+  k_point_eval_lds<64><<<nb, kThreads, 0, s>>>(d.P, d.C, pm_stream(d), d.camR, d.cam, d.Kc, d.X,
                                                d.scale_p, d.diag_p, d.ptV, d.min_diag, d.max_diag, mode, 0,
                                                slot(d, kPGradPt), slot(d, kPXNormPt), d.gate,
                                                cam_fold(d, mode, count_grad), PointFold{});
@@ -1840,18 +1853,18 @@
   const PointFold pf = factor && mode == 1 ? PointFold{radius, d.radius_dev, d.ptL, d.ptS, d.ptG, slot(d, kPBad)}
                                            : PointFold{};
 #define SFM_PE_LDS(M_)                                                                                              \
-  k_point_eval_lds<M_><<<nb, kThreads, 0, s>>>(d.P, d.C, d.pt_off, d.cam_pm, d.uv_pm, d.camR, d.cam, d.Kc, d.X,      \
+  k_point_eval_lds<M_><<<nb, kThreads, 0, s>>>(d.P, d.C, pm_stream(d), d.camR, d.cam, d.Kc, d.X,      \
                                                d.scale_p, d.diag_p, d.ptV, d.min_diag, d.max_diag, mode,           \
                                                reuse_diag ? 1 : 0, slot(d, kPGradPt), slot(d, kPXNormPt), d.gate,    \
                                                CamFold{}, pf)
   if (d.C <= 64) SFM_PE_LDS(64);
   else if (d.C <= 512 && !env_flag_k("SFM_PE_GROUPS1"))
     k_point_eval_lds<512, 2><<<blocks_for(d.P, 2 * kThreads), 2 * kThreads, 0, s>>>(
-        d.P, d.C, d.pt_off, d.cam_pm, d.uv_pm, d.camR, d.cam, d.Kc, d.X, d.scale_p, d.diag_p, d.ptV, d.min_diag,
+        d.P, d.C, pm_stream(d), d.camR, d.cam, d.Kc, d.X, d.scale_p, d.diag_p, d.ptV, d.min_diag,
         d.max_diag, mode, reuse_diag ? 1 : 0, slot(d, kPGradPt), slot(d, kPXNormPt), d.gate, CamFold{}, pf);
   else if (d.C <= 512) SFM_PE_LDS(512);
   else
-    k_point_eval_rc<<<nb, kThreads, 0, s>>>(d.P, d.pt_off, d.cam_pm, d.uv_pm, d.camR, d.cam, d.Kc, d.X, d.scale_p,
+    k_point_eval_rc<<<nb, kThreads, 0, s>>>(d.P, pm_stream(d), d.camR, d.cam, d.Kc, d.X, d.scale_p,
                                             d.diag_p, d.ptV, d.min_diag, d.max_diag, mode, reuse_diag ? 1 : 0,
                                             slot(d, kPGradPt), slot(d, kPXNormPt), d.gate, pf);
 #undef SFM_PE_LDS
@@ -1969,7 +1982,7 @@
   if (backsub_pm(d, cams_var, pts_var)) {
     constexpr int kG = 4;
     k_backsub_pm<kG><<<blocks_for(d.P, kG * kThreads), kG * kThreads, 0, s>>>(
-        d.P, d.C, d.pt_off, d.cam_pm, d.uv_pm, d.ptL, d.ptV, d.scale_p, d.X, d.X_new, d.ypt,
+        d.P, d.C, pm_stream(d), d.ptL, d.ptV, d.scale_p, d.X, d.X_new, d.ypt,
         slot(d, kPModel), slot(d, kPModelPt), slot(d, kPStepPt), slot(d, kPBadBack), slot(d, kPNewCost), d.gate,
         CamStepFold{d.cam, d.ysol, d.scale_c, d.camR, d.Kc, d.cam_new, d.camRn,
                     count_norm ? slot(d, kPStepCam) : nullptr, slot(d, kPBadCam)});
diff --git a/sfm_amd/csrc/ba_problem.hip b/sfm_amd/csrc/ba_problem.hip
--- a/sfm_amd/csrc/ba_problem.hip
+++ b/sfm_amd/csrc/ba_problem.hip
@@ -57,6 +57,9 @@
   const int32_t* pair_order = nullptr;
   int64_t n_pairs = 0;
   int bperm_per = 0;
+  bool wm = false;
+  int64_t wm_slots = 0;
+  int32_t* wm_cnt = nullptr;
   int64_t* grp_host = nullptr;
   int32_t* uv_err_host = nullptr;
 
@@ -81,6 +84,8 @@
   template <typename T>
   bool tmp(T*& p, size_t count) { return (rc = dalloc_tmp(h, &p, count)) == 0; }
 };
+
+size_t wm_waves(int P) { return (size_t(P) + 63) / 64; }
 
 struct ProblemGuard {
   Setup& c;
@@ -262,6 +267,8 @@
   c.small = c.plan.host_counts && !(ss && ss[0] == '0') &&
             hostlayout::small_setup_fits(c.N, c.C, c.P, c.cam_cnt.data() + 4,
                                          reinterpret_cast<const int32_t*>(c.h->stage + c.plan.o_pc));
+  const char* wm = std::getenv("SFM_PM_WAVE_MAJOR");
+  c.wm = c.N > 0 && c.P > 0 && !c.small && !(wm && wm[0] == '0');
   c.timer.mark("camera runs (host)");
 }
 
@@ -279,7 +286,8 @@
                   c.alloc(d.jgrp, size_t(9)) && c.alloc(d.uv_cm, 2 * npad) && c.alloc(d.pos, N) &&
                   c.tmp(c.k64a, N) && c.tmp(c.k64b, N) && c.tmp(c.k32a, size_t(nmax)) && c.tmp(c.k32b, size_t(nmax)) &&
                   c.tmp(c.iota, size_t(nmax)) && c.tmp(c.pt_s, N) && c.tmp(c.cm_order, N) &&
-                  c.tmp(c.perm, size_t(std::max<int64_t>(1, nch))) && c.tmp(tb, c.sort_bytes);
+                  c.tmp(c.perm, size_t(std::max<int64_t>(1, nch))) && c.tmp(tb, c.sort_bytes) &&
+                  (!c.wm || (c.alloc(d.woff, wm_waves(c.P) + 1) && c.tmp(c.wm_cnt, wm_waves(c.P) + 1)));
   c.sort_tmp = tb;
   return ok ? 0 : c.rc;
 }
@@ -374,6 +382,7 @@
                    c.iota, s);
   if (deferred_uv) launch_pt_off(P, c.k64b, N, C, d.pt_off, s);
   else HIPCHK(exclusive_sum32(c.sort_tmp, c.sort_bytes, c.cnt_p, d.pt_off, int64_t(P) + 1, s));
+  if (c.wm) HIPCHK(launch_wm_off(P, d.pt_off, c.wm_cnt, d.woff, c.sort_tmp, c.sort_bytes, s));
   HIPCHK(sort_pairs32(c.sort_tmp, c.sort_bytes, c.k32a, c.k32b, c.iota, c.cm_order, N, uint64_t(std::max(1, C)) - 1,
                       s));
   launch_fill_cm(d.N_pad, d.wcam, d.cam_rng, c.d_cam_off, c.cm_order, c.pt_s, deferred_uv ? nullptr : d.uv_pm, d.cm_p,
@@ -394,6 +403,8 @@
   if (!c.plan.deferred_uv) {
     HIPCHK(hipMemcpyAsync(stg, c.poff + c.N, sizeof(int64_t), hipMemcpyDeviceToHost, c.s));
     HIPCHK(hipMemcpyAsync(stg + 8, c.d.jgrp, 9 * sizeof(int32_t), hipMemcpyDeviceToHost, c.s));
+    if (c.wm)
+      HIPCHK(hipMemcpyAsync(stg + 48, c.d.woff + wm_waves(c.P), sizeof(int32_t), hipMemcpyDeviceToHost, c.s));
     c.timer.mark("layout launches");
     return 0;
   }
@@ -404,6 +415,7 @@
   HostCopySet cs;
   cs.add(sd, c.poff + c.N, sizeof(int64_t));
   cs.add(sd + 8, c.d.jgrp, 9 * sizeof(int32_t));
+  if (c.wm) cs.add(sd + 48, c.d.woff + wm_waves(c.P), sizeof(int32_t));
   launch_copy_to_host(cs, c.s);
   return 0;
 }
@@ -415,6 +427,13 @@
   std::memcpy(g, stg + 8, sizeof(g));
   c.d.xcd_slice_max = 0;
   for (int i = 0; i < 8; ++i) c.d.xcd_slice_max = std::max(c.d.xcd_slice_max, g[i + 1] - g[i]);
+  if (c.wm) {
+    int32_t slots = 0;
+    std::memcpy(&slots, stg + 48, sizeof(slots));
+    c.wm_slots = slots;
+    c.wm = hostlayout::wave_major_fits(c.wm_slots, c.N, c.P);
+    if (!c.wm) c.d.woff = nullptr;
+  }
   c.timer.mark("layouts (device)");
   return 0;
 }
@@ -436,7 +455,8 @@
   c.uv_err_host = reinterpret_cast<int32_t*>(c.grp_host + 16);
   const bool ok = c.alloc(d.blk, std::max<size_t>(1, size_t(d.n_blk))) &&
                   (c.small || c.alloc(d.seg, size_t(d.n_blk) + 1)) &&
-                  c.alloc(d.bpts, std::max<size_t>(1, size_t(c.n_pairs)));
+                  c.alloc(d.bpts, std::max<size_t>(1, size_t(c.n_pairs))) &&
+                  (!c.wm || (c.alloc(d.uv_wm, 2 * 64 * size_t(c.wm_slots)) && c.alloc(d.cam_wm, 64 * size_t(c.wm_slots))));
   return ok ? 0 : c.rc;
 }
 
@@ -540,6 +560,11 @@
   return ok ? 0 : c.rc;
 }
 
+void layout_wave_major(Setup& c, hipStream_t st) {
+  DevProblem& d = c.d;
+  if (c.wm) launch_wm_fill(c.P, d.pt_off, d.woff, d.cam_pm, d.uv_pm, d.cam_wm, d.uv_wm, st);
+}
+
 int layout_deferred_uv(Setup& c) {
   sfm_ba_handle* h = c.h;
   DevProblem& d = c.d;
@@ -549,6 +574,7 @@
   hipStream_t u = h->ustream;
   launch_uv_layout(c.N, d.N_pad, d.order, d.wcam, d.cam_rng, c.d_cam_off, c.cm_order, c.in_uv, d.uv_pm, d.uv_cm, c.err,
                    u);
+  layout_wave_major(c, u);
   void* ue_d = nullptr;
   HIPCHK(hipHostGetDevicePointer(&ue_d, c.uv_err_host, 0));
   HostCopySet cs;
@@ -643,6 +669,7 @@
   if ((rc = alloc_solver_arrays(c))) return rc;
   release_pool(c.h);
   if (plan.deferred_uv && (rc = layout_deferred_uv(c))) return rc;
+  if (!plan.deferred_uv) layout_wave_major(c, c.s);
   if (side && c.small && (rc = enqueue_side_params(c))) return rc;
   if ((rc = finish_params(c))) return rc;
   return finish(c);
diff --git a/sfm_amd/csrc/ba_setup.h b/sfm_amd/csrc/ba_setup.h
--- a/sfm_amd/csrc/ba_setup.h
+++ b/sfm_amd/csrc/ba_setup.h
@@ -49,6 +49,10 @@
                       const int32_t* cam_off, const int32_t* cm_order, const double* uv, double* uv_pm, double* uv_cm,
                       int32_t* err, hipStream_t s);
 void launch_pt_off(int P, const uint64_t* sorted_keys, int64_t N, int C, int32_t* pt_off, hipStream_t s);
+hipError_t launch_wm_off(int P, const int32_t* pt_off, int32_t* m, int32_t* woff, void* tmp, size_t bytes,
+                         hipStream_t s);
+void launch_wm_fill(int P, const int32_t* pt_off, const int32_t* woff, const int32_t* cam_pm, const double* uv_pm,
+                    int32_t* cam_wm, double* uv_wm, hipStream_t s);
 void launch_chunk_keys(int n, const int4* ch, const int32_t* cm_order, const int32_t* pt_s, int P, uint32_t* key,
                        int32_t* iota, hipStream_t s);
 void launch_chunk_gather(int n, const int32_t* perm, const int4* ch, const uint32_t* key, int4* out, int32_t* grp,
diff --git a/sfm_amd/csrc/ba_setup.hip b/sfm_amd/csrc/ba_setup.hip
--- a/sfm_amd/csrc/ba_setup.hip
+++ b/sfm_amd/csrc/ba_setup.hip
@@ -185,6 +185,36 @@
     if (key[mid] < t) lo = mid + 1; else hi = mid;
   }
   pt_off[p] = int32_t(lo);
+}
+
+__global__ __launch_bounds__(kT) void k_wm_count(int P, int n_w, const int32_t* __restrict__ pt_off,
+                                                 int32_t* __restrict__ m) {
+  const int64_t p = int64_t(blockIdx.x) * kT + threadIdx.x;
+  int32_t n = p < P ? pt_off[p + 1] - pt_off[p] : 0;
+  for (int o = 32; o; o >>= 1) n = max(n, __shfl_xor(n, o));
+  if ((threadIdx.x & 63) == 0 && (p >> 6) <= n_w) m[p >> 6] = n;
+}
+__global__ __launch_bounds__(kT) void k_wm_fill(int P, int n_w, const int32_t* __restrict__ pt_off,
+                                                const int32_t* __restrict__ woff,
+                                                const int32_t* __restrict__ cam_pm, const double* __restrict__ uv_pm,
+                                                int32_t* __restrict__ cam_wm, double* __restrict__ uv_wm) {
+  const int64_t p = int64_t(blockIdx.x) * kT + threadIdx.x;
+  const int64_t w = p >> 6;
+  if (w >= n_w) return;
+  const int32_t q0 = p < P ? pt_off[p] : 0;
+  const int32_t n = p < P ? pt_off[p + 1] - q0 : 0;
+  const int32_t m = woff[w + 1] - woff[w];
+  size_t dst = size_t(woff[w]) * 64 + size_t(p & 63);
+  int32_t c = 0;
+  double2 u = make_double2(0.0, 0.0);
+  for (int32_t k = 0; k < m; ++k, dst += 64) {
+    if (k < n) {
+      c = cam_pm[q0 + k];
+      u = reinterpret_cast<const double2*>(uv_pm)[q0 + k];
+    }
+    cam_wm[dst] = c;
+    reinterpret_cast<double2*>(uv_wm)[dst] = u;
+  }
 }
 
 __global__ __launch_bounds__(kT) void k_seg(int64_t n_blk, const uint32_t* __restrict__ key, int64_t n_pairs,
@@ -586,6 +616,17 @@
 void launch_pt_off(int P, const uint64_t* sorted_keys, int64_t N, int C, int32_t* pt_off, hipStream_t s) {
   k_pt_off<<<nblocks(int64_t(P) + 1), kT, 0, s>>>(P, sorted_keys, N, C, pt_off);
 }
+hipError_t launch_wm_off(int P, const int32_t* pt_off, int32_t* m, int32_t* woff, void* tmp, size_t bytes,
+                         hipStream_t s) {
+  const int n_w = int((int64_t(P) + 63) / 64);
+  k_wm_count<<<nblocks(64 * int64_t(n_w) + 1), kT, 0, s>>>(P, n_w, pt_off, m);
+  return exclusive_sum32(tmp, bytes, m, woff, int64_t(n_w) + 1, s);
+}
+void launch_wm_fill(int P, const int32_t* pt_off, const int32_t* woff, const int32_t* cam_pm, const double* uv_pm,
+                    int32_t* cam_wm, double* uv_wm, hipStream_t s) {
+  const int n_w = int((int64_t(P) + 63) / 64);
+  if (n_w > 0) k_wm_fill<<<nblocks(64 * int64_t(n_w)), kT, 0, s>>>(P, n_w, pt_off, woff, cam_pm, uv_pm, cam_wm, uv_wm);
+}
 void launch_seg(int64_t n_blk, const uint32_t* key, int64_t n_pairs, int32_t* seg, hipStream_t s) {
   k_seg<<<nblocks(n_blk + 1), kT, 0, s>>>(n_blk, key, n_pairs, seg);
 }
```

After: 1.906 billion residual-evals/s (obs x evaluations), median of 6. +1.4%, better.
